# polimi-ispl/deep_prior_interpolation

Measured on AMD Instinct MI355X. Metric: Adam iters/sec on 3D MultiRes-UNet (whole job over n_gpus; per_gpu beside it); recon SNR(dB) vs ref under config.snr_vs_reference, higher is better.
Workload: dtype f32

## Files before the change

### deep_prior_interpolation_amd/_lib.py

```python
import ctypes as C
import os

_HERE = os.path.dirname(os.path.abspath(__file__))
LIB_PATH = os.path.join(_HERE, "libdpi_hip.so")


class DpiError(RuntimeError):
    pass


ABI_VERSION = 406

IO_X_BF16, IO_Y_BF16, IO_DY_BF16, IO_DX_BF16 = 1, 2, 4, 8
STORE_FWD_BF16, STORE_GRAD_BF16 = 1, 2


class ConvDesc(C.Structure):
    _fields_ = [("size", C.c_int), ("Cin", C.c_int), ("Cout", C.c_int), ("D", C.c_int), ("H", C.c_int), ("W", C.c_int),
                ("k", C.c_int), ("kd", C.c_int), ("stride", C.c_int), ("precision", C.c_int), ("io", C.c_int)]

    def __init__(self, Cin=0, Cout=0, D=1, H=1, W=1, k=1, kd=1, stride=1, precision=0, io=0):
        super().__init__(C.sizeof(ConvDesc), int(Cin), int(Cout), int(D), int(H), int(W), int(k), int(kd), int(stride), int(precision), int(io))


# ... 32 lines not shown
    "dpi_bn_bwd_reduce": (_I, [_P, _P, _P, _P, _P, _P, _F, _F, _I, _Z, _P, _P]),
    "dpi_bn_bwd_apply": (_I, [_P, _P, _P, _P, _P, _P, _F, _F, _P, _I, _I, _Z, _P, _P, _P, _P]),
    "dpi_bn_bwd_apply_fork": (_I, [_P, _P, _P, _P, _P, _P, _F, _F, _P, _I, _I, _Z, _P, _P, _P,
                                   _P, _P, _P, _P, _P, _F, _P, _P, _P, _P, _P, _P, _F, _P, _P]),
    "dpi_bn_bwd_apply_dual": (_I, [_P, _I, _I, _Z] + [_P, _P, _P, _P, _P, _F, _P, _P, _P, _P] * 2 + [_I, _I, _P, _P, _P, _F, _P, _P]),
    "dpi_chain_add_stats": (_I, [_P, _P, _P, _P, _I, _Z, _F, _P, _P, _P]),
    "dpi_lrelu_bwd": (_I, [_P, _P, _F, _Z, _P, _P]),
    "dpi_act_fwd": (_I, [_P, _Z, _I, _P, _P]),
    "dpi_act_bwd": (_I, [_P, _P, _Z, _I, _P, _P]),
    "dpi_add": (_I, [_P, _P, _Z, _P, _P]),
    "dpi_channel_sum": (_I, [_P, _I, _Z, _P, _P, _P]),
    "dpi_upsample2x_fwd": (_I, [_P, _P, _I, _I, _I, _I, _I, _I, _I, _I, _P, _P]),
    "dpi_upsample2x_bwd_ws_floats": (_Z, [_I, _I, _I, _I, _I, _I, _I, _I]),
    "dpi_upsample2x_bwd": (_I, [_P, _I, _I, _I, _I, _I, _I, _I, _I, _P, _P, _P]),
    "dpi_crop_copy": (_I, [_P, _I, _I, _I, _I, _I, _I, _I, _I, _I, _I, _P, _P]),
    "dpi_crop_copy_bwd": (_I, [_P, _I, _I, _I, _I, _I, _I, _I, _I, _I, _I, _P, _P]),
    "dpi_attn_gate_fwd": (_I, [_P, _P, _I, _I, _I, _I, _I, _P, _P, _P]),
    "dpi_attn_gate_bwd_ws_floats": (_Z, [_I, _I, _I, _I, _I]),
    "dpi_attn_gate_bwd": (_I, [_P, _P, _P, _I, _I, _I, _I, _I, _P, _P, _P, _P]),
    "dpi_pconv_mask_fwd": (_I, [_P, _P, _I, _I, _Z, _P, _P, _P]),
    "dpi_pconv_norm_fwd": (_I, [_P, _P, _P, _I, _I, _I, _I, _P, _P, _P, _P]),
    "dpi_pconv_norm_bwd_ws_floats": (_Z, [_I, _Z]),
    "dpi_pconv_norm_bwd": (_I, [_P, _P, _I, _Z, _P, _P, _P, _P]),
    "dpi_pconv_mask_bwd": (_I, [_P, _P, _P, _I, _I, _Z, _P, _P, _P]),
    "dpi_maxpool2x2_fwd": (_I, [_P, _I, _I, _I, _P, _P]),
    "dpi_maxpool2x2_bwd": (_I, [_P, _P, _I, _I, _I, _P, _P]),
    "dpi_deconv4x4s2_fwd": (_I, [_P, _P, _P, _I, _I, _I, _I, _P, _P]),
    "dpi_deconv4x4s2_bwd_data": (_I, [_P, _P, _I, _I, _I, _I, _P, _P]),
    "dpi_deconv4x4s2_bwd_weight": (_I, [_P, _P, _I, _I, _I, _I, _P, _P]),
    "dpi_loss_ws_doubles": (_Z, [_Z]),
    "dpi_masked_loss": (_I, [_P, _P, _P, _Z, _I, _F, _P, _P, _P, _P]),
    "dpi_adam_multi": (_I, [_P, _P, _I, _P, C.c_double, C.c_double, C.c_double, _P, _P]),
    "dpi_langevin_multi": (_I, [_P, _P, _I, _P, _I, C.c_double, C.c_double, C.c_double, C.c_double, C.c_double, _U64, _P, _P, _P]),
    "dpi_moments_update": (_I, [_P, _P, _P, _Z, _P, _I, _I, _P, _P]),
    "dpi_loop_control": (_I, [_P, _P, _P, _I, _P, _P, _P, _I, C.c_double, C.c_double, _I, C.c_double, C.c_double, _I, C.c_double, _P]),
    "dpi_copy_if": (_I, [_P, _P, _P, _Z, _P]),
    "dpi_masked_loss_holdout": (_I, [_P, _P, _P, _P, _I, _I, _Z, _I, _F, _P, _P, _P, _P]),
    "dpi_loop_control_holdout": (_I, [_P, _P, _P, _I, _P, _P, _P, _I, C.c_double, C.c_double, _I, C.c_double, C.c_double, _I, C.c_double, _P]),
    "dpi_ema_loss": (_I, [_P, _P, _P, _P, _P, _I, _I, _Z, _I, _F, _P, _P, _P, _P, _P]),
    "dpi_loop_control_ema": (_I, [_P, _P, _I, _P, _P, _I, _P, _P, _P, _I, C.c_double, C.c_double, _I, C.c_double, C.c_double, _I, C.c_double, _P]),
    "dpi_noise_add": (_I, [_P, _Z, _F, _U64, _P, _P, _P]),
    "dpi_fill_normal": (_I, [_P, _Z, _F, _F, _U64, _U64, _P]),
    "dpi_fir_axis0": (_I, [_P, _P, _I, _I, _I, _Z, _P, _P]),
    "dpi_axpy": (_I, [_F, _P, _Z, _P, _P]),
    "dpi_diff_axis": (_I, [_P, _Z, _I, _Z, _I, _F, _I, _P, _P]),
    "dpi_hale2d": (_I, [_P, _P, _P, _P, _Z, _I, _I, _I, _P, _P]),
    "dpi_structure_tensor": (_I, [_P, _Z, _I, _I, _F, _F, _P, _P, _P, _P]),
    "dpi_dips": (_I, [_P, _P, _P, _Z, _P, _P, _P]),
    "dpi_hale_sections": (_I, [_P, _P, _I, _I, _I, _I, _I, _P, _P]),
    "dpi_structure_tensor_sections": (_I, [_P, _I, _I, _I, _I, _F, _F, _F, _P, _P, _P, _P, _P, _P]),
    "dpi_avo_fwd": (_I, [_P, _P, _I, _I, _Z, _P, _P]),
    "dpi_avo_adj": (_I, [_P, _P, _I, _I, _Z, _P, _P]),
    "dpi_trace_sample_fwd": (_I, [_P, _P, _I, _I, _I, _I, _P, _P]),
    "dpi_trace_sample_adj": (_I, [_P, _P, _I, _I, _I, _I, _P, _P]),
    "dpi_max_ws_floats": (_Z, [_Z]),
    "dpi_scaled_max": (_I, [_P, _Z, _F, _P, _P, _P]),
    "dpi_threshold": (_I, [_P, _Z, _P, _P, _P]),
    "dpi_pocs_project": (_I, [_P, _P, _P, _Z, _P, _P]),
    "dpi_overlap_add": (_I, [_P, _I, _I, _I, _I, _I, _I, _P, _I, _I, _I, _P]),
    "dpi_overlap_normalize": (_I, [_P, _I, _I, _I, _I, _I, _I, _I, _I, _I, _F, _P]),
    "dpi_overlap_add_weighted": (_I, [_P, _P, _I, _I, _I, _I, _I, _I, _P, _I, _P, _I, _P, _I, _U, _P, _I, _I, _I, _I, _P]),
    "dpi_overlap_finalize_weighted": (_I, [_P, _I, _I, _I, _I, _F, _P, _P, _P]),
    "dpi_channel_stats_io": (_I, [_P, _P, _I, _Z, _P, _U, _P]),
    "dpi_chain_apply_io": (_I, [_P, _P, _I, _Z, _P, _U, _P]),
    "dpi_chain_add_stats_io": (_I, [_P, _P, _P, _P, _I, _Z, _F, _P, _P, _U, _P]),
    "dpi_bn_bwd_reduce_io": (_I, [_P, _P, _P, _P, _P, _P, _F, _F, _I, _Z, _P, _U, _P]),
    "dpi_bn_bwd_apply_io": (_I, [_P, _P, _P, _P, _P, _P, _F, _F, _P, _I, _I, _Z, _P, _P, _P, _U, _P]),
    "dpi_bn_bwd_apply_fork_io": (_I, [_P, _P, _P, _P, _P, _P, _F, _F, _P, _I, _I, _Z, _P, _P, _P,
                                      _P, _P, _P, _P, _P, _F, _P, _P, _P, _P, _P, _P, _F, _P, _U, _P]),
    "dpi_bn_bwd_apply_dual_io": (_I, [_P, _I, _I, _Z] + [_P, _P, _P, _P, _P, _F, _P, _P, _P, _P] * 2 + [_I, _I, _P, _P, _P, _F, _P, _U, _P]),
    "dpi_upsample2x_fwd_io": (_I, [_P, _P, _I, _I, _I, _I, _I, _I, _I, _I, _P, _U, _P]),
    "dpi_upsample2x_bwd_io": (_I, [_P, _I, _I, _I, _I, _I, _I, _I, _I, _P, _P, _U, _P]),
    "dpi_noise_add_io": (_I, [_P, _Z, _F, _U64, _P, _P, _U, _P]),
    "dpi_noise_add_regen_io": (_I, [_Z, _F, _U64, _U64, _F, _U64, _P, _P, _U, _P]),
    "dpi_set_option": (_I, [C.c_char_p, _I]),
    "dpi_pack_scratch_bytes": (_Z, []),
    "dpi_pack_release": (_I, []),
    "dpi_pack_forget": (_I, [_P]),
    "dpi_pack_slot_count": (_Z, []),
    "dpi_join_bwd_ws_doubles": (_Z, [_I, _Z]),
    "dpi_join_bwd": (_I, [_P, _P, _P, _P, _P, _F, _I, _Z,  _P, _P, _P, _P, _P, _F,  _P, _P, _P, _P, _P, _F,  _P, _P,  _I, _I, _P, _P, _P, _F,
                          _P, _P, _P, _P, _P, _P, _P, _U, _P]),
    "dpi_chain_add_apply": (_I, [_P, _P, _P, _P, _P, _I, _Z, _P, _U, _P]),
}

_lib = None


def load():
    global _lib
    if _lib is not None:
        return _lib
    if not os.path.exists(LIB_PATH):
        raise DpiError("libdpi_hip.so not found at %s — run `python -c 'import __graft_entry__ as g; g.build()'` "
                       "(hipcc --offload-arch=gfx950); there is no CPU fallback" % LIB_PATH)
    import torch
    lib = C.CDLL(LIB_PATH)
    for name, (res, args) in SIGNATURES.items():
        try:
            fn = getattr(lib, name)
        except AttributeError as e:
            raise DpiError("libdpi_hip.so does not export %s (stale build?)" % name) from e
        fn.restype = res
        fn.argtypes = args
    if lib.dpi_version() < ABI_VERSION or lib.dpi_conv_desc_size() != C.sizeof(ConvDesc):
        raise DpiError("libdpi_hip.so is ABI version %d with a %d-byte dpi_conv_desc; this binding needs >= %d and %d bytes (stale build? "
                       "re-run __graft_entry__.build())" % (lib.dpi_version(), lib.dpi_conv_desc_size(), ABI_VERSION, C.sizeof(ConvDesc)))
    lib.set_option = lambda key, value: check(lib.dpi_set_option(key.encode(), int(value)), "dpi_set_option(%s)" % key)
    _lib = lib
    return lib


def check(code, what=""):
    if code != 0:
        msg = load().dpi_last_error()
        raise DpiError("%s failed (%d): %s" % (what, code, msg.decode() if msg else "?"))


def ptr(t):
    return None if t is None else t.data_ptr()


def stream():
    import torch
    return torch.cuda.current_stream().cuda_stream
```

### deep_prior_interpolation_amd/csrc/api.cpp

```cpp
#include <stdarg.h>
#include <string.h>
#include "common.h"

static thread_local char g_err[512] = "";

void dpi_set_error(const char* fmt, ...) {
  va_list ap;
  va_start(ap, fmt);
  vsnprintf(g_err, sizeof(g_err), fmt, ap);
  va_end(ap);
}

int dpi_check_launch(const char* what) {
  const hipError_t e = hipGetLastError();
  if (e != hipSuccess) {
    dpi_set_error("%s: %s", what, hipGetErrorString(e));
    return DPI_E_LAUNCH;
  }
  return DPI_OK;
}

extern "C" const char* dpi_last_error(void) { return g_err; }
extern "C" int dpi_version(void) { return 406; }
extern "C" int dpi_conv_desc_size(void) { return (int)sizeof(dpi_conv_desc); }

extern "C" int dpi_device_info(int device, int* cus, int* lds_bytes, size_t* hbm_bytes, char* name, int name_len) {
  hipDeviceProp_t p;
  const hipError_t e = hipGetDeviceProperties(&p, device);
  if (e != hipSuccess) {
    dpi_set_error("device_info: %s", hipGetErrorString(e));
    return DPI_E_LAUNCH;
  }
  if (cus) *cus = p.multiProcessorCount;
  if (lds_bytes) *lds_bytes = (int)p.sharedMemPerBlock;
  if (hbm_bytes) *hbm_bytes = p.totalGlobalMem;
  if (name && name_len > 0) {
    strncpy(name, p.gcnArchName, name_len - 1);
    name[name_len - 1] = 0;
  }
  return DPI_OK;
}

__global__ void dpi_marker_kernel() {}

extern "C" int dpi_profile_marker(int id, void* stream) {
  DPI_REQUIRE(id >= 1 && id < 65536, "profile_marker: id %d out of range", id);
  dpi_marker_kernel<<<(unsigned)id, 64, 0, (hipStream_t)stream>>>();
  return dpi_check_launch("profile_marker");
}

extern "C" int dpi_set_option(const char* key, int value) {
  DPI_REQUIRE(key != nullptr, "set_option: key is NULL");
  struct Entry { const char* key; int lo, hi; void (*set)(int); };
  static const Entry table[] = {
      {"splitk", 0, 1, dpi_set_splitk},
      {"dual_bwd_data", 0, 1, dpi_set_dual_bwd_data},
      {"bw_pair", 0, 2, dpi_set_bw_pair},
      {"bw_workgroups", 1, 1 << 24, [](int v) { dpi_set_bw_tuning(v, -1); }},
      {"bw_xcd_order", 0, 1, [](int v) { dpi_set_bw_tuning(0, v); }},
      {"mfma_min_cout", 0, 1 << 20, dpi_set_mfma_min_cout},
      {"bwd_weight_mfma_min_cout", 0, 1 << 20, dpi_set_bwd_weight_mfma_min_cout},
      {"fewco_mfma", 0, 1, dpi_set_fewco_mfma},
      {"q4", 0, 2, [](int v) { dpi_set_q4(v, -1); }},
      {"q4_ck", 0, 4, [](int v) { dpi_set_q4(-1, v); }},
      {"q4_debug", 0, 0xFFFF, dpi_set_q4_debug},
      {"bf16_debug", 0, 0x7F, dpi_set_bf16_debug},
  };
  for (const Entry& e : table)
    if (strcmp(key, e.key) == 0) {
      DPI_REQUIRE(value >= e.lo && value <= e.hi && !(strcmp(key, "q4_ck") == 0 && value != 0 && value != 2 && value != 4),
                  "set_option: %s = %d out of range [%d, %d]", key, value, e.lo, e.hi);
      e.set(value);
      return DPI_OK;
    }
  dpi_set_error("set_option: unknown key '%s'", key);
  return DPI_E_ARG;
}
```

### deep_prior_interpolation_amd/csrc/conv_direct.hip

```cpp
#include "conv_kernels.h"

namespace {

struct ConvArgs {
  const float* __restrict__ x;
  const float* __restrict__ chain;
  const float* __restrict__ w;
  const float* __restrict__ bias;
  float* __restrict__ y;
  double* __restrict__ partials;
  int Cin, Cout;
  int D, H, W;
  int Do, Ho, Wo;
  int ntd, nth, ntw;
  long w_out_stride, w_in_stride;
  int accumulate;
  int xb, yb;
};

template <int KD, int S, int CO_B, int OW, int TZ, int TY, int TX, int CI_B, bool FLIP>
__global__ __launch_bounds__(TZ* TY* TX) void conv_direct_kernel(ConvArgs a) {
  constexpr int KS = 3;
  constexpr int NT = TZ * TY * TX;
  constexpr int SD = (KD > 1) ? S : 1;
// ... 447 lines not shown

extern "C" size_t dpi_conv_bwd_data_ws_floats(const dpi_conv_desc* d) {
  return dpi_check_conv_desc(d) == DPI_OK && d->stride == 1 ? conv_plan(d, true, 0).ws_floats : 0;
}

static int conv_run(const dpi_conv_desc* d, const float* x, const float* chain, const float* w, const float* bias,
                    float* y, double* partials, bool flip, int accumulate, float* ws, size_t ws_floats, hipStream_t st) {
  switch (conv_plan(d, flip, accumulate).kernel) {
    case ConvKernel::Bf16S2: return dpi_conv_bf16_s2_run(d, x, chain, w, bias, y, partials, st);
    case ConvKernel::Bf16: return dpi_conv_bf16_run(d, x, chain, w, bias, y, partials, flip, accumulate, st);
    case ConvKernel::Q4: return dpi_conv_q4_run(d, x, chain, w, bias, y, partials, flip, accumulate, st);
    case ConvKernel::Mfma: return dpi_conv_mfma_run(d, x, chain, w, bias, y, partials, flip, accumulate, ws, ws_floats, st);
    case ConvKernel::PwMfma: return dpi_conv_pw_mfma_run(d, x, chain, w, bias, y, partials, flip, accumulate, st);
    case ConvKernel::Fewco: return dpi_conv_fewco_mfma_run(d, x, chain, w, bias, y, partials, st);
    case ConvKernel::Pw: case ConvKernel::Direct: break;
  }
  const int taps = d->kd * d->k * d->k;
  const int cin = flip ? d->Cout : d->Cin, cout = flip ? d->Cin : d->Cout;
  const long w_out = flip ? taps : (long)d->Cin * taps, w_in = flip ? (long)d->Cin * taps : taps;
  const int xb = dpi_io_in(d, flip), yb = dpi_io_out(d, flip);
  const int co_b = pick_co_b(cout);
  if (d->k == 1) {
    PwArgs a{x, chain, w, bias, y, partials, cin, cout, (size_t)d->D * d->H * d->W, w_out, w_in, accumulate, xb, yb};
    dim3 grid((unsigned)cdivz(a.V, kPwVoxPerBlock), cdiv(cout, co_b));
    launch_pw_co(a, co_b, grid, st);
    return dpi_check_launch("conv_pw");
  }
  ConvArgs a{x, chain, w, bias, y, partials, cin, cout, d->D, d->H, d->W, 0, 0, 0, 0, 0, 0, w_out, w_in, accumulate, xb, yb};
  dpi_conv_out_dims(d, &a.Do, &a.Ho, &a.Wo);
  dim3 grid(direct_tiles(d, &a.ntd, &a.nth, &a.ntw), cdiv(cout, co_b));
  if (d->kd == 3) {
    if (d->stride == 1) { if (flip) launch_co<3, 1, true>(a, co_b, grid, st); else launch_co<3, 1, false>(a, co_b, grid, st); }
    else launch_co<3, 2, false>(a, co_b, grid, st);
  } else {
    if (d->stride == 1) { if (flip) launch_co<1, 1, true>(a, co_b, grid, st); else launch_co<1, 1, false>(a, co_b, grid, st); }
    else launch_co<1, 2, false>(a, co_b, grid, st);
  }
  return dpi_check_launch("conv_direct");
}

extern "C" int dpi_conv_fwd_ws(const dpi_conv_desc* d, const float* x, const float* x_chain, const float* w, const float* bias, float* y,
                               double* stat_partials, float* ws, size_t ws_floats, void* stream) {
  if (int e = dpi_check_conv_desc(d)) return e;
  DPI_REQUIRE(x && w && y, "conv_fwd: null tensor");
  DPI_REQUIRE(ws || ws_floats == 0, "conv_fwd: workspace size without a workspace");
  return conv_run(d, x, x_chain, w, bias, y, stat_partials, false, 0, ws, ws_floats, (hipStream_t)stream);
}

extern "C" int dpi_conv_fwd(const dpi_conv_desc* d, const float* x, const float* x_chain, const float* w,
                            const float* bias, float* y, double* stat_partials, void* stream) {
  return dpi_conv_fwd_ws(d, x, x_chain, w, bias, y, stat_partials, nullptr, 0, stream);
}

extern "C" int dpi_conv_bwd_data(const dpi_conv_desc* d, const float* dy, const float* w, float* dx,
                                 int accumulate, void* stream) {
  return dpi_conv_bwd_data_ws(d, dy, w, dx, accumulate, nullptr, 0, stream);
}

static int g_dual = getenv("DPI_NO_DUAL") ? 0 : 1;
extern "C" void dpi_set_dual_bwd_data(int on) { g_dual = on; }
extern "C" int dpi_conv_bwd_data_dual(const dpi_conv_desc* d3, const float* dy3, const float* w3, const dpi_conv_desc* d1, const float* dy1,
                                      const float* w1, float* dx, int accumulate, float* ws, size_t ws_floats, void* stream) {
  if (int e = dpi_check_conv_desc(d3)) return e;
  if (int e = dpi_check_conv_desc(d1)) return e;
  DPI_REQUIRE(dy3 && w3 && dy1 && w1 && dx, "conv_bwd_data_dual: null tensor");
  DPI_REQUIRE(ws || ws_floats == 0, "conv_bwd_data_dual: workspace size without a workspace");
  DPI_REQUIRE(d3->k == 3 && d1->k == 1 && d3->stride == 1 && d1->stride == 1, "conv_bwd_data_dual: needs a 3x3(x3) and a 1x1(x1) stride-1 layer");
  DPI_REQUIRE(d3->Cin == d1->Cin && d3->D == d1->D && d3->H == d1->H && d3->W == d1->W, "conv_bwd_data_dual: the two layers read different tensors");
  hipStream_t st = (hipStream_t)stream;
  DPI_REQUIRE((d3->io & (DPI_IO_DX_BF16 | DPI_IO_X_BF16)) == (d1->io & (DPI_IO_DX_BF16 | DPI_IO_X_BF16)), "conv_bwd_data_dual: the two layers disagree on the storage type of their input");
  const ConvKernel k3 = conv_plan(d3, true, accumulate).kernel;
  if (g_dual && k3 == ConvKernel::Bf16 && dpi_conv_bf16_second_ok(d3, true) && (d3->io & DPI_IO_DY_BF16) == (d1->io & DPI_IO_DY_BF16)) {
    const MfmaSecond sec{dy1, w1, d1->Cout, 1, (long)d1->Cin};
    return dpi_conv_bf16_run(d3, dy3, nullptr, w3, nullptr, dx, nullptr, true, accumulate, st, &sec);
  }
  if (g_dual && k3 == ConvKernel::Mfma && dpi_conv_mfma_second_ok(d3, true, d1->Cout, ws != nullptr)) {
    const MfmaSecond sec{dy1, w1, d1->Cout, 1, (long)d1->Cin};
    return dpi_conv_mfma_run(d3, dy3, nullptr, w3, nullptr, dx, nullptr, true, accumulate, nullptr, 0, st, &sec);
  }
  if (int e = conv_run(d1, dy1, nullptr, w1, nullptr, dx, nullptr, true, accumulate, nullptr, 0, st)) return e;
  return conv_run(d3, dy3, nullptr, w3, nullptr, dx, nullptr, true, 1, ws, ws_floats, st);
}

extern "C" int dpi_conv_bwd_data_ws(const dpi_conv_desc* d, const float* dy, const float* w, float* dx,
                                    int accumulate, float* ws, size_t ws_floats, void* stream) {
  if (int e = dpi_check_conv_desc(d)) return e;
  DPI_REQUIRE(dy && w && dx, "conv_bwd_data: null tensor");
  DPI_REQUIRE(ws || ws_floats == 0, "conv_bwd_data: workspace size without a workspace");
  hipStream_t st = (hipStream_t)stream;
  if (d->stride == 1) return conv_run(d, dy, nullptr, w, nullptr, dx, nullptr, true, accumulate, ws, ws_floats, st);
  if (dpi_conv_bf16_s2_bwd_usable(d) && ((uintptr_t)dy & 7) == 0 && ((uintptr_t)dx & 3) == 0) return dpi_conv_bf16_s2_bwd_run(d, dy, w, dx, accumulate, st);
  if (d->Cin >= g_mfma_min_cout) return dpi_conv_bwd_data_s2_mfma_run(d, dy, w, dx, accumulate, st);
  int Do, Ho, Wo;
  dpi_conv_out_dims(d, &Do, &Ho, &Wo);
  BwdS2Args a{dy, w, dx, d->Cin, d->Cout, d->D, d->H, d->W, Do, Ho, Wo, d->kd, accumulate, (d->io & DPI_IO_DY_BF16) != 0, (d->io & DPI_IO_DX_BF16) != 0};
  const size_t V = (size_t)d->D * d->H * d->W;
  dim3 grid((unsigned)cdivz(V, 256), cdiv(d->Cin, 8));
  conv_bwd_data_s2_kernel<8><<<grid, 256, 0, st>>>(a);
  return dpi_check_launch("conv_bwd_data_s2");
}
```

### deep_prior_interpolation_amd/csrc/conv_kernels.h

```cpp
#pragma once
#include "common.h"

struct MfmaSecond { const float* x2; const float* w2; int C2; long w2_co_stride, w2_c_stride; };
void dpi_conv_out_dims(const dpi_conv_desc* d, int* Do, int* Ho, int* Wo);
int dpi_conv_mfma_stat_blocks(const dpi_conv_desc* d, bool flip);
size_t dpi_conv_mfma_ws_floats(const dpi_conv_desc* d, bool flip);
bool dpi_conv_mfma_second_ok(const dpi_conv_desc* d, bool flip, int C2, bool have_ws);
int dpi_conv_mfma_run(const dpi_conv_desc* d, const float* x, const float* chain, const float* w, const float* bias, float* y,
                      double* partials, bool flip, int accumulate, float* ws, size_t ws_floats, hipStream_t st, const MfmaSecond* sec = nullptr);
int dpi_conv_bwd_data_s2_mfma_run(const dpi_conv_desc* d, const float* dy, const float* w, float* dx, int accumulate, hipStream_t st);
size_t dpi_conv_bwd_weight_mfma_ws_floats(const dpi_conv_desc* d);
bool dpi_conv_bwd_weight_mfma_swapped(const dpi_conv_desc* d, bool chained);
int dpi_conv_bwd_weight_mfma_run(const dpi_conv_desc* d, const float* x, const float* chain, const float* dy, float* dw, float* ws, hipStream_t st);
size_t dpi_conv_bwd_weight_smallco_ws_floats(const dpi_conv_desc* d);
int dpi_conv_bwd_weight_smallco_run(const dpi_conv_desc* d, const float* x, const float* chain, const float* dy, float* dw, float* ws, hipStream_t st);
int dpi_conv_pw_mfma_stat_blocks(const dpi_conv_desc* d);
int dpi_conv_pw_mfma_run(const dpi_conv_desc* d, const float* x, const float* chain, const float* w, const float* bias, float* y,
                         double* partials, bool flip, int accumulate, hipStream_t st);
size_t dpi_conv_pw_bwd_weight_mfma_ws_floats(const dpi_conv_desc* d);
int dpi_conv_pw_bwd_weight_mfma_run(const dpi_conv_desc* d, const float* x, const float* chain, const float* dy, float* dw, float* ws, hipStream_t st);
bool dpi_conv_fewco_usable(const dpi_conv_desc* d);
int dpi_conv_fewco_stat_blocks(const dpi_conv_desc* d);
int dpi_conv_fewco_mfma_run(const dpi_conv_desc* d, const float* x, const float* chain, const float* w, const float* bias, float* y,
                            double* partials, hipStream_t st);
bool dpi_conv_q4_usable(const dpi_conv_desc* d, bool flip);
int dpi_conv_q4_stat_blocks(const dpi_conv_desc* d);
int dpi_conv_q4_run(const dpi_conv_desc* d, const float* x, const float* chain, const float* w, const float* bias, float* y,
                    double* partials, bool flip, int accumulate, hipStream_t st);
bool dpi_bf16_force_all();
bool dpi_conv_bf16_usable(const dpi_conv_desc* d, bool flip);
int dpi_conv_bf16_stat_blocks(const dpi_conv_desc* d);
bool dpi_conv_bf16_second_ok(const dpi_conv_desc* d, bool flip);
int dpi_conv_bf16_run(const dpi_conv_desc* d, const float* x, const float* chain, const float* w, const float* bias, float* y,
                      double* partials, bool flip, int accumulate, hipStream_t st, const MfmaSecond* sec = nullptr);
bool dpi_conv_bf16_s2_usable(const dpi_conv_desc* d);
int dpi_conv_bf16_s2_stat_blocks(const dpi_conv_desc* d);
int dpi_conv_bf16_s2_run(const dpi_conv_desc* d, const float* x, const float* chain, const float* w, const float* bias, float* y, double* partials,
                         hipStream_t st);
bool dpi_conv_bf16_s2_bwd_usable(const dpi_conv_desc* d);
int dpi_conv_bf16_s2_bwd_run(const dpi_conv_desc* d, const float* dy, const float* w, float* dx, int accumulate, hipStream_t st);
bool dpi_conv_bf16_bww_usable(const dpi_conv_desc* d);
size_t dpi_conv_bf16_bww_ws_floats(const dpi_conv_desc* d);
int dpi_conv_bf16_bww_run(const dpi_conv_desc* d, const float* x, const float* chain, const float* dy, float* dw, float* ws, hipStream_t st);
bool dpi_conv_bf16_bww_s2_usable(const dpi_conv_desc* d);
size_t dpi_conv_bf16_bww_s2_ws_floats(const dpi_conv_desc* d);
int dpi_conv_bf16_bww_s2_run(const dpi_conv_desc* d, const float* x, const float* dy, float* dw, float* ws, hipStream_t st);
```

### deep_prior_interpolation_amd/csrc/conv_mfma.hip

```cpp
#include "conv_kernels.h"

namespace {

typedef float f32x4 __attribute__((ext_vector_type(4)));

struct MArgs {
  const float* __restrict__ x;
  const float* __restrict__ chain;
  const float* __restrict__ w;
  const float* __restrict__ bias;
  float* __restrict__ y;
  double* __restrict__ partials;
  int Cin, Cout;
  int D, H, W;
  int ntd, nth, ntw;
  long w_out_stride, w_in_stride;
  int accumulate;
  int split_cps;
  const float* __restrict__ x2;
  const float* __restrict__ w2;
  int C2;
  long w2_co_stride, w2_c_stride;
  int xb, yb;
  int ny;
};

template <int KD, int NR, int NH, int S = 1>
struct Geo {
  static constexpr bool SLICES = (KD == 3 && NR >= 4);
  static constexpr int SD = KD == 3 ? S : 1;
  static constexpr int TZ = SLICES ? 4 : 1;
  static constexpr int TY = SLICES ? NR : 4 * NR;
  static constexpr int TW = 16 * NH;
  static constexpr int ID = (TZ - 1) * SD + KD;
  static constexpr int IH = (TY - 1) * S + 3;
  static constexpr int IW = (TW - 1) * S + 3;
  static constexpr int RS = (IW + 3) & ~3;
  static constexpr int DS0 = IH * RS;
  static constexpr int DS = (S == 1 && (RS % 32) == 4) ? DS0 + ((12 - (DS0 % 32)) + 32) % 32 : DS0;
  static constexpr int CS0 = ID * DS;
  static constexpr int CSM = S == 1 ? 16 : 1;
  static constexpr int CS = CS0 + ((CSM - (CS0 % 32)) + 32) % 32;
  static constexpr int TILE = ID * IH * IW;
  static constexpr int E = (TILE + 255) / 256;
  static constexpr int NROW = (NR - 1) * S + 3;
  static constexpr int NSTEP = KD * NROW;
  static constexpr int NB = 3 * NH;
};

__device__ __forceinline__ int xcd_tile(int bid, int ntiles) {
  const int q = ntiles >> 3, r = ntiles & 7, xcd = bid & 7, i = bid >> 3;
  return (xcd < r ? xcd * (q + 1) : r * (q + 1) + (xcd - r) * q) + i;
}

template <class G>
__device__ __forceinline__ void tile_slots(int tid, int id0, int ih0, int iw0, int D, int H, int W, int (&goff)[G::E], int (&loff)[G::E]) {
#pragma unroll
  for (int e = 0; e < G::E; ++e) {
    const int idx = tid + e * 256;
    const int col = idx % G::IW, row = idx / G::IW;
    const int hy = row % G::IH, dz = row / G::IH;
    const int gd = id0 + dz, gh = ih0 + hy, gw = iw0 + col;
    const bool ok = idx < G::TILE && gd >= 0 && gd < D && gh >= 0 && gh < H && gw >= 0 && gw < W;
    goff[e] = ok ? (gd * H + gh) * W + gw : -1;
    loff[e] = idx < G::TILE ? dz * G::DS + hy * G::RS + col : -1;
  }
}

template <class G>
__device__ __forceinline__ void stage_load(float (&sr)[4][G::E], const float* __restrict__ x, int Cin, size_t V, int c0,
                                           const int (&goff)[G::E], bool xb = false) {
  if (xb) {
#pragma unroll
    for (int c = 0; c < 4; ++c) {
      const int ci = min(c0 + c, Cin - 1);
      const __amdgpu_buffer_rsrc_t r = dpi_buffer_t(dpi_at(x, (size_t)ci * V, true), V, true);
#pragma unroll
      for (int e = 0; e < G::E; ++e) sr[c][e] = dpi_buffer_load_bf16_raw(r, goff[e]);
    }
    return;
  }
#pragma unroll
  for (int c = 0; c < 4; ++c) {
    const int ci = min(c0 + c, Cin - 1);
    const __amdgpu_buffer_rsrc_t r = dpi_buffer(x + (size_t)ci * V, V * sizeof(float));
#pragma unroll
    for (int e = 0; e < G::E; ++e) sr[c][e] = dpi_buffer_load(r, goff[e] * 4);
  }
}

template <class G>
__device__ __forceinline__ void stage_store(float* lds, const float (&sr_in)[4][G::E], const float* __restrict__ chain, int Cin, int c0,
                                            const int (&goff)[G::E], const int (&loff)[G::E], bool xb = false) {
  float sr[4][G::E];
#pragma unroll
  for (int c = 0; c < 4; ++c)
#pragma unroll
    for (int e = 0; e < G::E; ++e) sr[c][e] = sr_in[c][e];
  if (xb) {
#pragma unroll
    for (int c = 0; c < 4; ++c)
#pragma unroll
      for (int e = 0; e < G::E; ++e) sr[c][e] = dpi_widen_raw(sr[c][e]);
  }
  if (chain == nullptr) {
#pragma unroll
    for (int c = 0; c < 4; ++c)
// ... 11 lines not shown
      const float v = goff[e] >= 0 ? apply_chain(t, sr[c][e]) : sr[c][e];
      if ((e + 1) * 256 <= G::TILE || loff[e] >= 0) lds[c * G::CS + loff[e]] = v;
    }
  }
}

template <int KD, int NR, int NH>
struct GeoV2 {
  static constexpr int TY = 4 * NR, TW = 16 * NH;
  static constexpr int ID = KD == 3 ? 3 : 1, IH = (TY - 1) * 2 + 3;
  static constexpr int NQ = TW / 2 + 1;
  static constexpr int PW = 2 * NQ;
  static constexpr int RS = 2 * PW;
  static constexpr int DS = IH * RS;
  static constexpr int CS0 = ID * DS;
  static constexpr int CS = CS0 + ((16 - (CS0 % 32)) + 32) % 32;
  static constexpr int NV4 = ID * IH * NQ;
  static constexpr int E = (NV4 + 255) / 256;
};
template <class GV>
__device__ __forceinline__ void tile_slots_v(int tid, int id0, int ih0, int iw0, int D, int H, int W, int (&goff)[GV::E], int (&loff)[GV::E]) {
#pragma unroll
  for (int e = 0; e < GV::E; ++e) {
    const int idx = tid + e * 256;
    const int q = idx % GV::NQ, row = idx / GV::NQ;
    const int hy = row % GV::IH, dz = row / GV::IH;
    const int gd = id0 + dz, gh = ih0 + hy, gw = iw0 + 4 * q;
    const bool ok = idx < GV::NV4 && gd >= 0 && gd < D && gh >= 0 && gh < H && gw >= 0 && gw + 4 <= W;
    goff[e] = ok ? (gd * H + gh) * W + gw : -4;
    loff[e] = idx < GV::NV4 ? dz * GV::DS + hy * GV::RS + 2 * q : -1;
  }
}
template <class GV>
__device__ __forceinline__ void stage_load_v(f32x4 (&sv)[4][GV::E], const float* __restrict__ x, int Cin, size_t V, int c0, const int (&goff)[GV::E]) {
#pragma unroll
  for (int c = 0; c < 4; ++c) {
    const int ci = min(c0 + c, Cin - 1);
    const __amdgpu_buffer_rsrc_t r = dpi_buffer(x + (size_t)ci * V, V * sizeof(float));
#pragma unroll
    for (int e = 0; e < GV::E; ++e) sv[c][e] = __builtin_bit_cast(f32x4, __builtin_amdgcn_raw_buffer_load_b128(r, goff[e] * 4, 0, 0));
  }
}
template <class GV>
__device__ __forceinline__ void stage_store_v(float* lds, const f32x4 (&sv)[4][GV::E], const float* __restrict__ chain, int Cin, int c0,
                                              const int (&goff)[GV::E], const int (&loff)[GV::E]) {
  typedef float f32x2 __attribute__((ext_vector_type(2)));
  if (chain == nullptr) {
#pragma unroll
    for (int c = 0; c < 4; ++c)
#pragma unroll
      for (int e = 0; e < GV::E; ++e)
        if ((e + 1) * 256 <= GV::NV4 || loff[e] >= 0) {
          float* const p = lds + c * GV::CS + loff[e];
          *reinterpret_cast<f32x2*>(p) = (f32x2){sv[c][e][0], sv[c][e][2]};
          *reinterpret_cast<f32x2*>(p + GV::PW) = (f32x2){sv[c][e][1], sv[c][e][3]};
        }
    return;
  }
#pragma unroll
  for (int c = 0; c < 4; ++c) {
    const Chain t = load_chain(chain, min(c0 + c, Cin - 1));
#pragma unroll
    for (int e = 0; e < GV::E; ++e) {
      const float m = goff[e] >= 0 ? 1.f : 0.f;
      if ((e + 1) * 256 <= GV::NV4 || loff[e] >= 0) {
        float* const p = lds + c * GV::CS + loff[e];
        *reinterpret_cast<f32x2*>(p) = (f32x2){m * apply_chain(t, sv[c][e][0]), m * apply_chain(t, sv[c][e][2])};
        *reinterpret_cast<f32x2*>(p + GV::PW) = (f32x2){m * apply_chain(t, sv[c][e][1]), m * apply_chain(t, sv[c][e][3])};
      }
    }
  }
}

#ifdef DPI_TRACE
__device__ long long g_blk[8192][4];
__device__ long long g_trace[4][64];
#define TR(i) do { if (trc >= 0 && tid == 0) g_trace[trc][i] = clock64(); } while (0)
#define TRC(i) do { if (trc >= 0 && tid == 0 && (i) < 38) g_trace[trc][i] = clock64(); } while (0)
#else
#define TR(i)
#define TRC(i)
#endif
template <int KD, int NR, int NH, bool FLIP, int S = 1, int WPE = 2, bool PERSIST = false, bool TAILPACK = false, bool IOB = false, bool YLOOP = false,
          bool S2V = false>
__global__ __launch_bounds__(256, WPE) void conv_mfma_kernel(MArgs a) {
  static_assert(!YLOOP || (!PERSIST && !TAILPACK), "the channel-tile loop is built for the one-tile-per-workgroup variants without a packed tail");
  static_assert(!S2V || (S == 2 && !FLIP && !PERSIST && !TAILPACK && !IOB && NR < 4), "vectorised stride-2 staging: forward, fp32 tensors, row-split tiles");
  using GV = GeoV2<KD, NR < 4 ? NR : 2, NH>;
  if constexpr (!IOB) { a.xb = 0; a.yb = 0; }
  using G = Geo<KD, NR, NH, S>;
  constexpr int TAPS = KD * 9;
  constexpr int PD = (KD - 1) / 2;
  constexpr int NT = NR * NH;
  __shared__ __attribute__((aligned(16))) float lds[4 * (S2V ? GV::CS : G::CS)];
  __shared__ double red[4][16][2];

  const int tid = threadIdx.x, lane = tid & 63, wid = tid >> 6;
  const int lk = lane >> 4, lj = lane & 15;
  const int ntiles = a.ntd * a.nth * a.ntw;
  int vt0 = blockIdx.x, ytile = blockIdx.y;
  if constexpr (!PERSIST) {
    if (a.ny > 0) {
      const int q8 = ntiles >> 3, r8 = ntiles & 7, xcd = blockIdx.x & 7, j = blockIdx.x >> 3;
      const int i = YLOOP ? j : j / a.ny;
      ytile = YLOOP ? 0 : j - i * a.ny;
      if (i >= q8 + (xcd < r8 ? 1 : 0)) return;
      vt0 = i * 8 + xcd;
    }
  }
  int n0 = ytile * 16;
  const size_t V = (size_t)a.D * a.H * a.W;
  const int Do = (a.D + 2 * PD - KD) / G::SD + 1, Ho = (a.H - 1) / S + 1, Wo = (a.W - 1) / S + 1;
  const size_t Vo = (size_t)Do * Ho * Wo;
#ifdef DPI_TRACE
  const int trc = blockIdx.y != 0 ? -1 : blockIdx.x == 0 ? 0 : blockIdx.x == 1 ? 1 : blockIdx.x == 30 ? 2 : blockIdx.x == 50 ? 3 : -1;
  TR(0);
  if (tid == 0 && blockIdx.y == 0 && blockIdx.x < 8192) {
    g_blk[blockIdx.x][0] = wall_clock64();
    g_blk[blockIdx.x][2] = __builtin_amdgcn_s_getreg(63492);
    g_blk[blockIdx.x][3] = __builtin_amdgcn_s_getreg(63508);
  }
#endif
  auto tile_origin = [&](int vt, int& tile_id, int& od0, int& oh0, int& ow0) {
    tile_id = xcd_tile(vt, ntiles);
    int bt = tile_id;
    const int tw_i = bt % a.ntw; bt /= a.ntw;
    const int th_i = bt % a.nth; bt /= a.nth;
    od0 = bt * G::TZ; oh0 = th_i * G::TY; ow0 = tw_i * G::TW;
  };

  const int wz = G::SLICES ? wid : 0, wh = G::SLICES ? 0 : wid * NR;
  const int lbase = S2V ? lk * GV::CS + wh * 2 * GV::RS + lj : lk * G::CS + wz * G::SD * G::DS + wh * S * G::RS + lj * S;

  int co_w = n0 + lj;
  auto w_ptr = [&](int c0, bool& ok) {
    const int ci = c0 + lk;
    ok = co_w < a.Cout && ci < a.Cin;
    return a.w + (ok ? co_w : 0) * a.w_out_stride + (ok ? ci : 0) * a.w_in_stride;
  };
  auto load_w_raw = [&](float (&wn)[9], int c0, int kd) {
    bool ok;
    const float* __restrict__ wp = w_ptr(c0, ok);
#pragma unroll
    for (int t = 0; t < 9; ++t) wn[t] = wp[FLIP ? (TAPS - 1 - (kd * 9 + t)) : kd * 9 + t];
  };
  auto commit_w = [&](float (&wr)[TAPS], const float (&wn)[9], int c0, int kd) {
    const bool ok = co_w < a.Cout && c0 + lk < a.Cin;
#pragma unroll
    for (int t = 0; t < 9; ++t) wr[kd * 9 + t] = ok ? wn[t] : 0.f;
  };

  const int c_lo = a.split_cps ? (int)blockIdx.z * a.split_cps : 0;
  float* __restrict__ const ybase = a.y + (size_t)blockIdx.z * a.Cout * Vo;
  constexpr int EE = S2V ? GV::E : G::E;
  int goff[EE], loff[EE];
  float wr[TAPS], wn[9], sr[S2V ? 1 : 4][S2V ? 1 : G::E];
  f32x4 sv[S2V ? 4 : 1][S2V ? GV::E : 1];
  auto slots = [&](int od, int oh, int ow) {
    if constexpr (S2V) tile_slots_v<GV>(tid, od * G::SD - PD, oh * 2 - 1, ow * 2 - 4, a.D, a.H, a.W, goff, loff);
    else tile_slots<G>(tid, od * G::SD - PD, oh * S - 1, ow * S - 1, a.D, a.H, a.W, goff, loff);
  };
  auto sload = [&](int c0) {
    if constexpr (S2V) stage_load_v<GV>(sv, a.x, a.Cin, V, c0, goff);
    else stage_load<G>(sr, a.x, a.Cin, V, c0, goff, a.xb);
  };
  auto sstore = [&](int c0) {
    if constexpr (S2V) stage_store_v<GV>(lds, sv, a.chain, a.Cin, c0, goff, loff);
    else stage_store<G>(lds, sr, a.chain, a.Cin, c0, goff, loff, a.xb);
// ... 128 lines not shown
        for (int i = 0; i < G::NB; ++i) bc[i] = bn[i];
        if constexpr (!YLOOP) { if (ir == G::NROW - 1) commit_w(wr, wn, cn, kd); }
      }
      if (tail_next) commit_tail_w();
      TRC(5 + (c0 / 4) * 4);
    }
    if constexpr (TAILPACK) {
      if (tail && cin_main == 0) { load_tail_w(); commit_tail_w(); }
      if (tail) {
        __syncthreads();
        sstore(cin_main);
        __syncthreads();
        if (has_next) {
          slots(od_n, oh_n, ow_n);
          sload(0);
        }
#pragma unroll
        for (int hr = 0; hr < NR; ++hr) {
          float tb[NH][NTG];
#pragma unroll
          for (int h = 0; h < NH; ++h)
#pragma unroll
            for (int g = 0; g < NTG; ++g) tb[h][g] = lds[lbase + ttoff[g] + hr * G::RS + h * 16];
#pragma unroll
          for (int g = 0; g < NTG; ++g)
#pragma unroll
            for (int h = 0; h < NH; ++h)
              acc[hr * NH + h] = __builtin_amdgcn_mfma_f32_16x16x4f32(wt[g], tb[h][g], acc[hr * NH + h], 0, 0, 0);
        }
      }
    }
    if constexpr (YLOOP) {
      if (yt + 1 < nyt) {
        const int con = (yt + 1) * 16 + lj, ci = c_lo + lk;
        const bool okn = con < a.Cout && ci < a.Cin;
        const float* __restrict__ wp = a.w + (okn ? con : 0) * a.w_out_stride + (okn ? ci : 0) * a.w_in_stride;
#pragma unroll
        for (int t = 0; t < TAPS; ++t) wr[t] = wp[FLIP ? (TAPS - 1 - t) : t];
      }
    }
    if constexpr (FLIP && !PERSIST) if (a.x2 != nullptr) {
      const __amdgpu_buffer_rsrc_t r2 = dpi_buffer_t(a.x2, (size_t)a.C2 * Vo, a.xb);
      int voff[NT];
#pragma unroll
      for (int t = 0; t < NT; ++t) {
        const int od = od0 + wz, oh = oh0 + wh + t / NH, ow = ow0 + (t % NH) * 16 + lj;
        voff[t] = (od < Do && oh < Ho && ow < Wo) ? (od * Ho + oh) * Wo + ow : -1;
      }
      const int nk2 = (a.C2 + 3) >> 2;
      auto load2 = [&](float (&b)[NT], float& wv, int kc) {
        const int c = kc * 4 + lk;
        const bool ok = c < a.C2 && co_w < a.Cout;
        const float wraw = a.w2[(ok ? co_w : 0) * a.w2_co_stride + (ok ? c : 0) * a.w2_c_stride];
        wv = ok ? wraw : 0.f;
        const int cbase = c * (int)Vo;
#pragma unroll
        for (int t = 0; t < NT; ++t)
          b[t] = a.xb ? dpi_buffer_load_bf16(r2, voff[t] >= 0 ? cbase + voff[t] : -1) : dpi_buffer_load(r2, voff[t] >= 0 ? (cbase + voff[t]) * 4 : -4);
      };
      float b0[NT], b1[NT], w0v, w1v;
      load2(b0, w0v, 0);
      for (int kc = 0; kc < nk2; kc += 2) {
        if (kc + 1 < nk2) load2(b1, w1v, kc + 1);
#pragma unroll
        for (int t = 0; t < NT; ++t) acc[t] = __builtin_amdgcn_mfma_f32_16x16x4f32(w0v, b0[t], acc[t], 0, 0, 0);
        if (kc + 1 < nk2) {
          if (kc + 2 < nk2) load2(b0, w0v, kc + 2);
#pragma unroll
          for (int t = 0; t < NT; ++t) acc[t] = __builtin_amdgcn_mfma_f32_16x16x4f32(w1v, b1[t], acc[t], 0, 0, 0);
        }
      }
    }
    TR(40);

    const bool interior = od0 + G::TZ <= Do && oh0 + G::TY <= Ho && ow0 + G::TW <= Wo && n0 + 16 <= a.Cout;
    const int vbase = ((od0 + wz) * Ho + oh0 + wh) * Wo + ow0 + lj;
#pragma unroll
    for (int r = 0; r < 4; ++r) {
      const int co = n0 + 4 * lk + r;
      const bool cok = co < a.Cout;
      const float bv = (a.bias && cok) ? a.bias[co] : 0.f;
      float* __restrict__ yc = dpi_at(ybase, (size_t)(cok ? co : 0) * Vo + vbase, a.yb);
      double s = 0.0, q = 0.0;
      if (a.yb) {
        const bool pairs = !(Wo & 1) && !(Vo & 1) && !((uintptr_t)ybase & 3);
#pragma unroll
        for (int t = 0; t < NT; ++t) {
          const int od = od0 + wz, oh = oh0 + wh + t / NH, ow = ow0 + (t % NH) * 16 + lj;
          const bool ok = interior || (cok && od < Do && oh < Ho && ow < Wo);
          const float v = dpi_round_bf16(acc[t][r] + bv);
          dpi_st_bf16_row(yc, (t / NH) * Wo + (t % NH) * 16, v, ok, pairs, lj);
          if (ok) { s += v; q += (double)v * v; }
        }
      } else if (interior) {
#pragma unroll
        for (int t = 0; t < NT; ++t) {
          const float v = acc[t][r] + bv;
          yc[(t / NH) * Wo + (t % NH) * 16] = v;
          if (a.partials) { s += v; q += (double)v * v; }
        }
      } else {
#pragma unroll
        for (int t = 0; t < NT; ++t) {
          const int od = od0 + wz, oh = oh0 + wh + t / NH, ow = ow0 + (t % NH) * 16 + lj;
          if (cok && od < Do && oh < Ho && ow < Wo) {
            const float v = acc[t][r] + bv;
            yc[(t / NH) * Wo + (t % NH) * 16] = v;
            s += v;
            q += (double)v * v;
          }
        }
      }
      if (a.partials) {
#pragma unroll
        for (int o = 8; o > 0; o >>= 1) { s += __shfl_xor(s, o, 64); q += __shfl_xor(q, o, 64); }
        if (lj == 0) { red[wid][4 * lk + r][0] = s; red[wid][4 * lk + r][1] = q; }
      }
    }
    if (a.partials) {
      __syncthreads();
      if (tid < 32) {
        const int c = tid >> 1, which = tid & 1;
        const double rsum = red[0][c][which] + red[1][c][which] + red[2][c][which] + red[3][c][which];
        if (n0 + c < a.Cout) a.partials[((size_t)tile_id * a.Cout + n0 + c) * 2 + which] = rsum;
      }
    }
    }
    TR(41);
    if (!has_next) break;
    vt = vt_next; tile_id = tile_n; od0 = od_n; oh0 = oh_n; ow0 = ow_n;
  }
#ifdef DPI_TRACE
  if (tid == 0 && blockIdx.y == 0 && blockIdx.x < 8192) g_blk[blockIdx.x][1] = wall_clock64();
#endif
}

struct BwMArgs {
  const float* __restrict__ x;
  const float* __restrict__ chain;
  const float* __restrict__ dy;
  float* __restrict__ ws;
  int Cin, Cout;
  int D, H, W;
  int ntd, nth, ntw, ntiles, tiles_per_chunk;
  int swap;
  int y0;
  int ngroups, nchunks;
  int xb, dyb;
};

template <int KD, int S, int NR, int NH, int NG = 1>
struct BwLds {
  using G = Geo<KD, NR, NH, S>;
  static constexpr int NTQ0 = (4 * KD * 9 + 15) / 16;
  static constexpr int LDSF = NG * (4 * G::CS > 4 * NTQ0 * 256 ? 4 * G::CS : 4 * NTQ0 * 256);
  static constexpr int DYRS = 4 * (4 * NH) + 4;
};

template <int KD, int S, int NR, int NH, int TC, int NG = 1, bool IOB = false>
__device__ __forceinline__ void conv_bwd_weight_mfma_body(const BwMArgs& a_in, float* __restrict__ lds, float* __restrict__ dyl_all, int first_group = -1) {
  BwMArgs a = a_in;
  if constexpr (!IOB) { a.xb = 0; a.dyb = 0; }
  static_assert(NG == 1 || TC == 0, "the column-trimmed tail is a single group");
#ifdef DPI_TRACE
  const int trc = (blockIdx.y == 0 && blockIdx.z == 0 && blockIdx.x < 4) ? (int)blockIdx.x : -1;
  int trn = 0;
#define TRW() do { if (trc >= 0 && threadIdx.x == 0 && trn < 64) g_trace[trc][trn++] = clock64(); } while (0)
// ... 447 lines not shown
      for (int t = 0; t < TAPS; ++t) wr[t] = ok ? wn[t] : 0.f;
    }
    __syncthreads();
#pragma unroll
    for (int c = 0; c < 4; ++c)
#pragma unroll
      for (int e = 0; e < E; ++e)
        if ((e + 1) * 256 <= TILE || loff[e] >= 0) lds[c * CS + loff[e]] = a.dyb ? dpi_widen_raw(sr[c][e]) : sr[c][e];
    __syncthreads();
    if (c0 + 4 < a.Cout) fetch(c0 + 4);
#pragma unroll
    for (int sd = 0; sd < ID; ++sd)
#pragma unroll
      for (int ir = 0; ir < 3; ++ir)
#pragma unroll
        for (int sw = 0; sw < 2; ++sw) {
          const float b = lds[lbase + (sd * IH + ir) * RS + sw];
#pragma unroll
          for (int sh = 0; sh < 2; ++sh) {
            const int row = ir - sh;
            if (row < 0 || row > 1) continue;
#pragma unroll
            for (int cls = 0; cls < NCLS; ++cls) {
              const int pw = cls & 1, ph = (cls >> 1) & 1, pd = KD == 3 ? (cls >> 2) & 1 : 0;
              if ((sw && !pw) || (sh && !ph) || (sd && !pd)) continue;
              const int kw = pw ? (sw ? 0 : 2) : 1, kh = ph ? (sh ? 0 : 2) : 1, kd = KD == 3 ? (pd ? (sd ? 0 : 2) : 1) : 0;
              acc[cls][row] = __builtin_amdgcn_mfma_f32_16x16x4f32(wr[(kd * 3 + kh) * 3 + kw], b, acc[cls][row], 0, 0, 0);
            }
          }
        }
  }
  typedef float f32x2 __attribute__((ext_vector_type(2)));
  const bool vec2 = !a.dxb && ((a.W | (int)(V & 1)) & 1) == 0 && (((uintptr_t)a.dx) & 7) == 0;
  if (vec2) {
#pragma unroll
    for (int cp = 0; cp < NCLS / 2; ++cp) {
      const int ph = cp & 1, pd = KD == 3 ? (cp >> 1) & 1 : 0;
#pragma unroll
      for (int row = 0; row < 2; ++row) {
        const int id = KD == 3 ? 2 * md0 + pd : md0, ih = 2 * (mh0 + wid * 2 + row) + ph, iw = 2 * (mw0 + lj);
        if (id < a.D && ih < a.H && iw < a.W) {
          f32x2 old[4];
#pragma unroll
          for (int r = 0; r < 4; ++r) {
            const int ci = n0 + 4 * lk + r;
            const size_t o = (size_t)min(ci, a.Cin - 1) * V + ((size_t)id * a.H + ih) * a.W + iw;
            old[r] = a.accumulate ? *reinterpret_cast<const f32x2*>(a.dx + o) : (f32x2){0.f, 0.f};
          }
#pragma unroll
          for (int r = 0; r < 4; ++r) {
            const int ci = n0 + 4 * lk + r;
            if (ci < a.Cin) {
              const size_t o = (size_t)ci * V + ((size_t)id * a.H + ih) * a.W + iw;
              const f32x2 v = a.accumulate ? (f32x2){old[r][0] + acc[2 * cp][row][r], old[r][1] + acc[2 * cp + 1][row][r]}
                                           : (f32x2){acc[2 * cp][row][r], acc[2 * cp + 1][row][r]};
              *reinterpret_cast<f32x2*>(a.dx + o) = v;
            }
          }
        }
      }
    }
    return;
  }
#pragma unroll
  for (int cls = 0; cls < NCLS; ++cls) {
    const int pw = cls & 1, ph = (cls >> 1) & 1, pd = KD == 3 ? (cls >> 2) & 1 : 0;
#pragma unroll
    for (int row = 0; row < 2; ++row) {
      const int id = KD == 3 ? 2 * md0 + pd : md0, ih = 2 * (mh0 + wid * 2 + row) + ph, iw = 2 * (mw0 + lj) + pw;
      if (id < a.D && ih < a.H && iw < a.W) {
#pragma unroll
        for (int r = 0; r < 4; ++r) {
          const int ci = n0 + 4 * lk + r;
          if (ci < a.Cin) {
            const size_t o = (size_t)ci * V + ((size_t)id * a.H + ih) * a.W + iw;
            dpi_st(a.dx, o, a.accumulate ? dpi_ld(a.dx, o, a.dxb) + acc[cls][row][r] : acc[cls][row][r], a.dxb);
          }
        }
      }
    }
  }
}

__global__ __launch_bounds__(256) void splitk_reduce_kernel(const float* __restrict__ ws, int nsplit, const float* __restrict__ bias,
                                                            float* __restrict__ y, int accumulate, double* __restrict__ partials,
                                                            int Cout, size_t Vo, size_t per, bool yb) {
  const int lane = threadIdx.x & 63, co = blockIdx.y * 4 + (threadIdx.x >> 6);
  if (co >= Cout) return;
  const size_t lo = (size_t)blockIdx.x * per, hi = lo + per < Vo ? lo + per : Vo;
  const float bv = bias ? bias[co] : 0.f;
  double sum = 0.0, sq = 0.0;
  for (size_t v = lo + lane; v < hi; v += 64) {
    float t = ws[(size_t)co * Vo + v];
    for (int sp = 1; sp < nsplit; ++sp) t += ws[((size_t)sp * Cout + co) * Vo + v];
    t += bv;
    if (accumulate) t += dpi_ld(y, (size_t)co * Vo + v, yb);
    t = dpi_stored(t, yb);
    dpi_st(y, (size_t)co * Vo + v, t, yb);
    sum += t; sq += (double)t * t;
  }
  if (partials) {
#pragma unroll
    for (int o = 32; o > 0; o >>= 1) { sum += __shfl_xor(sum, o, 64); sq += __shfl_xor(sq, o, 64); }
    if (lane == 0) { partials[((size_t)blockIdx.x * Cout + co) * 2] = sum; partials[((size_t)blockIdx.x * Cout + co) * 2 + 1] = sq; }
  }
}

}

static void dpi_mfma_variant(const dpi_conv_desc* d, int cout, int* nr, int* nh) {
  int Do, Ho, Wo;
  dpi_conv_out_dims(d, &Do, &Ho, &Wo);
  const int tz = d->kd == 3 ? 4 : 1, ty = d->kd == 3 ? 8 : 32;
  const long nb = (long)cdiv(Do, tz) * cdiv(Ho, ty) * cdiv(Wo, 32) * cdiv(cout, 16);
  if (nb >= 512 && d->stride == 1) { *nr = 8; *nh = 2; }
  else { *nr = 2; *nh = Wo > 16 ? 2 : 1; }
}

static bool dpi_mfma_half_tile(const dpi_conv_desc* d, bool flip) {
  const int cin = flip ? d->Cout : d->Cin, cout = flip ? d->Cin : d->Cout;
  int nr, nh;
  dpi_mfma_variant(d, cout, &nr, &nh);
  if (nr != 8 || d->kd != 3) return false;
  if (cin == 1) return true;
  if (cin <= 8) return false;
  return flip || ((cin & 3) == 1);
}

static int dpi_mfma_tiles(const dpi_conv_desc* d, int nr, int nh, int* ntd, int* nth, int* ntw) {
  int Do, Ho, Wo;
  dpi_conv_out_dims(d, &Do, &Ho, &Wo);
  const bool slices = d->kd == 3 && nr >= 4;
  const int tz = slices ? 4 : 1, ty = slices ? nr : 4 * nr;
  *ntd = cdiv(Do, tz); *nth = cdiv(Ho, ty); *ntw = cdiv(Wo, 16 * nh);
  return *ntd * *nth * *ntw;
}

struct MfmaTiling { int nr, nh, ntd, nth, ntw, ntiles; };
static MfmaTiling mfma_tiling(const dpi_conv_desc* d, bool flip) {
  MfmaTiling t{};
  dpi_mfma_variant(d, flip ? d->Cin : d->Cout, &t.nr, &t.nh);
  if (dpi_mfma_half_tile(d, flip)) t.nr = 4;
  t.ntiles = dpi_mfma_tiles(d, t.nr, t.nh, &t.ntd, &t.nth, &t.ntw);
  return t;
}
int dpi_conv_mfma_stat_blocks(const dpi_conv_desc* d, bool flip) { return mfma_tiling(d, flip).ntiles; }

template <int KD, bool FLIP, bool IOB = false>
static void launch_variant(const MArgs& a_in, int nr, int nh, int stride, dim3 grid_in, hipStream_t st) {
  if constexpr (!IOB) {
    if (a_in.xb || a_in.yb) { launch_variant<KD, FLIP, true>(a_in, nr, nh, stride, grid_in, st); return; }
  }
  const bool persistent = stride == 1 && nr == 8 && a_in.Cin > 8;
  MArgs a = a_in;
  dim3 grid = grid_in;
  if (!persistent && grid_in.y > 1) {
    a.ny = (int)grid_in.y;
    grid = dim3(8 * ((grid_in.x + 7) / 8) * grid_in.y, 1, grid_in.z);
  }
  if (stride == 2) {
    if constexpr (!FLIP) {
      if constexpr (!IOB) {
        static const bool s2v = getenv("DPI_NO_S2V") == nullptr;
        if (s2v && a.W % 4 == 0 && (((size_t)a.D * a.H * a.W) & 3) == 0 && ((uintptr_t)a.x & 15) == 0) {
          if (nh == 2) conv_mfma_kernel<KD, 2, 2, false, 2, 2, false, false, false, false, true><<<grid, 256, 0, st>>>(a);
          else conv_mfma_kernel<KD, 2, 1, false, 2, 2, false, false, false, false, true><<<grid, 256, 0, st>>>(a);
          return;
        }
      }
      if (nh == 2) conv_mfma_kernel<KD, 2, 2, false, 2, 2, false, false, IOB><<<grid, 256, 0, st>>>(a);
      else conv_mfma_kernel<KD, 2, 1, false, 2, 2, false, false, IOB><<<grid, 256, 0, st>>>(a);
    }
    return;
  }
  const bool tailpack = (a.Cin & 3) == 1 && (a.Cin > 4 || a.Cin == 1);
  if (nr == 4) {
    if constexpr (KD == 3) {
      if (tailpack) conv_mfma_kernel<KD, 4, 2, FLIP, 1, 3, false, true, IOB><<<grid, 256, 0, st>>>(a);
      else conv_mfma_kernel<KD, 4, 2, FLIP, 1, 3, false, false, IOB><<<grid, 256, 0, st>>>(a);
    }
    return;
  }
  if (nr == 8) {
    static const bool persist = getenv("DPI_NO_PERSIST") == nullptr;
    dim3 pg = grid;
    static const bool yloop = getenv("DPI_YLOOP") != nullptr && getenv("DPI_YLOOP")[0] == '1';
    if constexpr (KD == 3 && FLIP && !IOB) {
      if (yloop && a.Cin <= 4 && a.ny > 1 && a.split_cps == 0 && grid_in.z == 1) {
        conv_mfma_kernel<KD, 8, 2, FLIP, 1, 2, false, false, IOB, true><<<dim3(8 * ((grid_in.x + 7) / 8), 1, 1), 256, 0, st>>>(a);
        return;
      }
    }
    if (a.Cin <= 8) conv_mfma_kernel<KD, 8, 2, FLIP, 1, 3, false, false, IOB><<<grid, 256, 0, st>>>(a);
    else {
      if (persist && grid.x > 512) pg.x = 512;
      if (tailpack) conv_mfma_kernel<KD, 8, 2, FLIP, 1, 2, true, true, IOB><<<pg, 256, 0, st>>>(a);
      else conv_mfma_kernel<KD, 8, 2, FLIP, 1, 2, true, false, IOB><<<pg, 256, 0, st>>>(a);
    }
  }
  else if (nh == 2) conv_mfma_kernel<KD, 2, 2, FLIP, 1, 2, false, false, IOB><<<grid, 256, 0, st>>>(a);
  else conv_mfma_kernel<KD, 2, 1, FLIP, 1, 2, false, false, IOB><<<grid, 256, 0, st>>>(a);
}

#ifdef DPI_TRACE
extern "C" int dpi_debug_read_blocks(long long* out) { return (int)hipMemcpyFromSymbol(out, HIP_SYMBOL(g_blk), sizeof(long long) * 8192 * 4); }
extern "C" int dpi_debug_read_trace(long long* out) { return (int)hipMemcpyFromSymbol(out, HIP_SYMBOL(g_trace), sizeof(long long) * 4 * 64); }
#endif
static int g_splitk = getenv("DPI_SPLITK") ? atoi(getenv("DPI_SPLITK")) : 1;
extern "C" void dpi_set_splitk(int on) { g_splitk = on; }
static int dpi_mfma_splitk(const dpi_conv_desc* d, bool flip) {
  if (!g_splitk || d->k != 3) return 1;
  const int cin = flip ? d->Cout : d->Cin, cout = flip ? d->Cin : d->Cout;
  int nr, nh, a, b, c;
  dpi_mfma_variant(d, cout, &nr, &nh);
  if (nr != 2 || dpi_mfma_half_tile(d, flip)) return 1;
  const long wgs = (long)dpi_mfma_tiles(d, nr, nh, &a, &b, &c) * cdiv(cout, 16);
  const int chunks = cdiv(cin, 4);
  if (wgs > 512 || (wgs > 256 && chunks < 24)) return 1;
  long ns = 1536 / wgs;
  if (ns > chunks / 8) ns = chunks / 8;
  if (ns > 8) ns = 8;
  return ns < 2 ? 1 : (int)ns;
}
size_t dpi_conv_mfma_ws_floats(const dpi_conv_desc* d, bool flip) {
  const int ns = dpi_mfma_splitk(d, flip);
  if (ns < 2) return 0;
  int Do, Ho, Wo;
  dpi_conv_out_dims(d, &Do, &Ho, &Wo);
  return (size_t)ns * (flip ? d->Cin : d->Cout) * Do * Ho * Wo;
}

bool dpi_conv_mfma_second_ok(const dpi_conv_desc* d, bool flip, int C2, bool have_ws) {
  int Do, Ho, Wo;
  dpi_conv_out_dims(d, &Do, &Ho, &Wo);
  if (!flip || d->stride != 1 || C2 < 1 || ((size_t)C2 + 4) * Do * Ho * Wo * sizeof(float) >= ((size_t)1 << 31)) return false;
  int nr, nh;
  dpi_mfma_variant(d, d->Cin, &nr, &nh);
  if (nr == 8 && !dpi_mfma_half_tile(d, flip) && d->Cout > 8) return false;
  return !(have_ws && dpi_mfma_splitk(d, flip) > 1);
}

int dpi_conv_mfma_run(const dpi_conv_desc* d, const float* x, const float* chain, const float* w, const float* bias, float* y,
                      double* partials, bool flip, int accumulate, float* ws, size_t ws_floats, hipStream_t st, const MfmaSecond* sec) {
  const int taps = d->kd * 9;
  const int cin = flip ? d->Cout : d->Cin, cout = flip ? d->Cin : d->Cout;
  const long w_out = flip ? taps : (long)d->Cin * taps, w_in = flip ? (long)d->Cin * taps : taps;
  MArgs a{x, chain, w, bias, y, partials, cin, cout, d->D, d->H, d->W, 0, 0, 0, w_out, w_in, accumulate, 0, nullptr, nullptr, 0, 0, 0,
          dpi_io_in(d, flip), dpi_io_out(d, flip)};
  const MfmaTiling t = mfma_tiling(d, flip);
  const int nr = t.nr, nh = t.nh, ntiles = t.ntiles;
  a.ntd = t.ntd; a.nth = t.nth; a.ntw = t.ntw;
  dim3 grid(ntiles, cdiv(cout, 16));
  if (sec) { a.x2 = sec->x2; a.w2 = sec->w2; a.C2 = sec->C2; a.w2_co_stride = sec->w2_co_stride; a.w2_c_stride = sec->w2_c_stride; }
  const int nsplit = (ws && !sec) ? dpi_mfma_splitk(d, flip) : 1;
  if (nsplit > 1) {
    int Do, Ho, Wo;
    dpi_conv_out_dims(d, &Do, &Ho, &Wo);
    const size_t Vo = (size_t)Do * Ho * Wo;
    DPI_REQUIRE(ws_floats >= (size_t)nsplit * cout * Vo, "conv (split): workspace of %zu floats, need %zu", ws_floats, (size_t)nsplit * cout * Vo);
    a.split_cps = 4 * cdiv(cdiv(cin, 4), nsplit);
    a.y = ws; a.bias = nullptr; a.partials = nullptr; a.accumulate = 0; a.yb = 0;
    grid.z = cdiv(cin, a.split_cps);
    const int nz = (int)grid.z;
    if (d->kd == 3) { if (flip) launch_variant<3, true>(a, nr, nh, d->stride, grid, st); else launch_variant<3, false>(a, nr, nh, d->stride, grid, st); }
    else { if (flip) launch_variant<1, true>(a, nr, nh, d->stride, grid, st); else launch_variant<1, false>(a, nr, nh, d->stride, grid, st); }
    if (int e = dpi_check_launch("conv_mfma (split)")) return e;
    splitk_reduce_kernel<<<dim3(ntiles, cdiv(cout, 4)), 256, 0, st>>>(ws, nz, bias, y, accumulate, partials, cout, Vo, cdivz(Vo, (size_t)ntiles),
                                                                      dpi_io_out(d, flip));
    return dpi_check_launch("splitk_reduce");
  }
  if (d->kd == 3) { if (flip) launch_variant<3, true>(a, nr, nh, d->stride, grid, st); else launch_variant<3, false>(a, nr, nh, d->stride, grid, st); }
  else { if (flip) launch_variant<1, true>(a, nr, nh, d->stride, grid, st); else launch_variant<1, false>(a, nr, nh, d->stride, grid, st); }
  return dpi_check_launch("conv_mfma");
}

static bool mfma_bw_swap_better(const dpi_conv_desc* d) {
  if (d->stride != 1) return false;
  auto util = [](int rows, int staged) { return (double)rows / (16.0 * cdiv(rows, 16)) * staged / (4.0 * cdiv(staged, 4)); };
  return util(d->Cin, d->Cout) > 1.15 * util(d->Cout, d->Cin);
}

static int g_bw_want = getenv("DPI_BW_WANT") ? atoi(getenv("DPI_BW_WANT")) : 2304;
static int g_bw_xcd_order = getenv("DPI_BW_XCD_ORDER") ? atoi(getenv("DPI_BW_XCD_ORDER")) : 0;
extern "C" void dpi_set_bw_tuning(int want_workgroups, int xcd_order) {
  if (want_workgroups > 0) g_bw_want = want_workgroups;
  if (xcd_order >= 0) g_bw_xcd_order = xcd_order;
}
static size_t bw_extra_lds() { static const size_t v = getenv("DPI_BW_EXTRA_LDS") ? (size_t)atoi(getenv("DPI_BW_EXTRA_LDS")) * 1024 : 0; return v; }
struct MfmaBwPlan { int nchunks, tiles_per_chunk, ntiles, ntd, nth, ntw, nr, nh, npairs, nfull, ny; };
static int g_bw_pair = getenv("DPI_BW_PAIR") ? atoi(getenv("DPI_BW_PAIR")) : 2;
extern "C" void dpi_set_bw_pair(int mode) { if (mode >= 0 && mode <= 2) g_bw_pair = mode; }
static MfmaBwPlan mfma_bw_plan(const dpi_conv_desc* d, bool swap = false) {
  MfmaBwPlan p{};
  {
    const int staged = swap ? d->Cout : d->Cin, groups = cdiv(staged, 4);
    const bool s1k3 = d->stride == 1 && d->kd == 3;
    const int tailg = (s1k3 && (staged & 3) == 1) ? 1 : 0;
    p.nfull = groups - tailg;
    p.npairs = (g_bw_pair && s1k3 && !g_bw_xcd_order && p.nfull >= 2 && d->io == 0) ? p.nfull / 2 : 0;
    if (g_bw_pair == 2) {
      int a_, b_, c_;
      if (p.nfull < 4 || dpi_mfma_tiles(d, 8, 2, &a_, &b_, &c_) < 1024) p.npairs = 0;
    }
    p.ny = p.npairs ? p.npairs + (p.nfull & 1) + tailg : groups;
  }
  if (d->stride == 1) { p.nr = 8; p.nh = 2; }
  else { int Do, Ho, Wo; dpi_conv_out_dims(d, &Do, &Ho, &Wo); p.nr = 2; p.nh = Wo > 16 ? 2 : 1; }
  p.ntiles = dpi_mfma_tiles(d, p.nr, p.nh, &p.ntd, &p.nth, &p.ntw);
  const size_t per = (size_t)d->Cout * d->Cin * d->kd * 9;
  const size_t max_chunks_mem = per ? ((size_t)32 << 20) / per : 1;
  const size_t blocks_other = (size_t)p.ny * (swap ? cdiv(d->Cin, 16) : cdiv(d->Cout, 16));
  size_t want = (size_t)g_bw_want / blocks_other;
  if (want < 1) want = 1;
  if (want > (size_t)p.ntiles) want = p.ntiles;
  if (want > max_chunks_mem) want = max_chunks_mem;
  if (want < 1) want = 1;
  if (g_bw_xcd_order && want > 8) want = want / 8 * 8;
  p.tiles_per_chunk = (int)cdivz(p.ntiles, want);
  p.nchunks = cdiv(p.ntiles, p.tiles_per_chunk);
  return p;
}

size_t dpi_conv_bwd_weight_mfma_ws_floats(const dpi_conv_desc* d) {
  const int n0 = mfma_bw_plan(d, false).nchunks, n1 = mfma_bw_swap_better(d) ? mfma_bw_plan(d, true).nchunks : 0;
  return (size_t)(n0 > n1 ? n0 : n1) * d->Cout * d->Cin * d->kd * 9;
}
bool dpi_conv_bwd_weight_mfma_swapped(const dpi_conv_desc* d, bool chained) { return !chained && mfma_bw_swap_better(d); }

static int bf16_row_class(const void* base, int row_len, size_t channel_elems) {
  return ((row_len & 1) == 0 && (channel_elems & 1) == 0 && ((uintptr_t)base & 3) == 0) ? 1 : 2;
}

int dpi_conv_bwd_weight_mfma_run(const dpi_conv_desc* d, const float* x, const float* chain, const float* dy, float* dw, float* ws,
                                 hipStream_t st) {
  const bool swap = dpi_conv_bwd_weight_mfma_swapped(d, chain != nullptr);
  const MfmaBwPlan p = mfma_bw_plan(d, swap);
  BwMArgs a{x, chain, dy, ws, d->Cin, d->Cout, d->D, d->H, d->W, p.ntd, p.nth, p.ntw, p.ntiles, p.tiles_per_chunk, 0, 0, 0, p.nchunks,
            (d->io & DPI_IO_X_BF16) != 0, (d->io & DPI_IO_DY_BF16) != 0};
  dim3 grid(p.nchunks, cdiv(d->Cin, 4), cdiv(d->Cout, 16));
  if (swap) {
    a.x = dy; a.chain = nullptr; a.dy = x; a.Cin = d->Cout; a.Cout = d->Cin; a.swap = 1;
    a.xb = (d->io & DPI_IO_DY_BF16) != 0; a.dyb = (d->io & DPI_IO_X_BF16) != 0;
    grid = dim3(p.nchunks, cdiv(d->Cout, 4), cdiv(d->Cin, 16));
  }
  if (a.dyb) {
    int Do_, Ho_, Wo_;
    dpi_conv_out_dims(d, &Do_, &Ho_, &Wo_);
    a.dyb = swap ? bf16_row_class(a.dy, d->W, (size_t)d->D * d->H * d->W) : bf16_row_class(a.dy, Wo_, (size_t)Do_ * Ho_ * Wo_);
  }
  auto xcd_grid = [&](dim3 g) {
    if (!g_bw_xcd_order) { a.ngroups = 0; return g; }
    a.ngroups = (int)g.y;
// ... 97 lines not shown
```

### deep_prior_interpolation_amd/csrc/conv_q4_mfma.hip

```cpp
#include "conv_kernels.h"

namespace {

typedef float f32x4 __attribute__((ext_vector_type(4)));

struct QArgs {
  const float* __restrict__ x;
  const float* __restrict__ chain;
  const float* __restrict__ w;
  const float* __restrict__ bias;
  float* __restrict__ y;
  double* __restrict__ partials;
  int Cin, Cout;
  int D, H, W;
  int ntd, nth, ntw;
  long w_out_stride, w_in_stride;
  int accumulate;
  int dbg;
};

template <int R>
struct QGeo {
  static constexpr int TZ = 4, TY = R, TW = 64;
  static constexpr int ID = TZ + 2, IH = R + 2;
  static constexpr int RS = 72;
  static constexpr int DS = IH * RS, CS = ID * DS;
  static constexpr int NV4 = ID * IH * 18;
  static constexpr int E = (NV4 + 255) / 256;
};

__device__ __forceinline__ int q4_xcd_tile(int bid, int ntiles) {
  const int q = ntiles >> 3, r = ntiles & 7, xcd = bid & 7, i = bid >> 3;
  return (xcd < r ? xcd * (q + 1) : r * (q + 1) + (xcd - r) * q) + i;
}

template <int R, int NB, int CK, bool FLIP, bool AL>
__global__ __launch_bounds__(256, 2) void conv_q4_mfma_kernel(QArgs a) {
  using G = QGeo<R>;
  constexpr int TAPS = 27;
  constexpr int NWT = CK * TAPS * NB * 4;
  constexpr int WE = (NWT + 255) / 256;
  __shared__ __attribute__((aligned(16))) float lds[CK * G::CS];
  __shared__ float wl[NWT];
  __shared__ double red[4][4 * NB][2];

  const int tid = threadIdx.x, lane = tid & 63, wid = tid >> 6;
  const int ntiles = a.ntd * a.nth * a.ntw;
  const int tile_id = q4_xcd_tile(blockIdx.x, ntiles);
  int bt = tile_id;
  const int tw_i = bt % a.ntw; bt /= a.ntw;
  const int th_i = bt % a.nth; bt /= a.nth;
  const int od0 = bt * G::TZ, oh0 = th_i * G::TY, ow0 = tw_i * G::TW;
  const size_t V = (size_t)a.D * a.H * a.W;

  int goff[G::E], loff[G::E];
#pragma unroll
  for (int e = 0; e < G::E; ++e) {
    const int idx = tid + e * 256;
    const int q = idx % 18, row = idx / 18;
    const int hy = row % G::IH, dz = row / G::IH;
    const int gd = od0 - 1 + dz, gh = oh0 - 1 + hy, gw = ow0 - 4 + 4 * q;
    const bool ok = idx < G::NV4 && gd >= 0 && gd < a.D && gh >= 0 && gh < a.H && gw >= 0 && gw + 4 <= a.W;
    goff[e] = ok ? (gd * a.H + gh) * a.W + gw : -4;
    loff[e] = idx < G::NV4 ? dz * G::DS + hy * G::RS + 4 * q : -1;
  }
  auto stage_load = [&](f32x4 (&sr)[CK][G::E], int c0) {
#pragma unroll
    for (int c = 0; c < CK; ++c) {
      const int ci = min(c0 + c, a.Cin - 1);
      const __amdgpu_buffer_rsrc_t r = dpi_buffer(a.x + (size_t)ci * V, V * sizeof(float));
#pragma unroll
      for (int e = 0; e < G::E; ++e) {
        if constexpr (AL) sr[c][e] = __builtin_bit_cast(f32x4, __builtin_amdgcn_raw_buffer_load_b128(r, goff[e] * 4, 0, 0));
        else {
#pragma unroll
          for (int k = 0; k < 4; ++k) sr[c][e][k] = dpi_buffer_load(r, goff[e] < 0 ? -4 : (goff[e] + k) * 4);
        }
      }
    }
  };
  auto stage_store = [&](const f32x4 (&sr)[CK][G::E], int c0) {
    if (a.chain == nullptr) {
#pragma unroll
      for (int c = 0; c < CK; ++c)
#pragma unroll
        for (int e = 0; e < G::E; ++e)
          if ((e + 1) * 256 <= G::NV4 || loff[e] >= 0) *reinterpret_cast<f32x4*>(lds + c * G::CS + loff[e]) = sr[c][e];
      return;
    }
#pragma unroll
    for (int c = 0; c < CK; ++c) {
      const Chain t = load_chain(a.chain, min(c0 + c, a.Cin - 1));
#pragma unroll
      for (int e = 0; e < G::E; ++e) {
        const float m = goff[e] >= 0 ? 1.f : 0.f;
        f32x4 v;
#pragma unroll
        for (int k = 0; k < 4; ++k) v[k] = m * apply_chain(t, sr[c][e][k]);
        if ((e + 1) * 256 <= G::NV4 || loff[e] >= 0) *reinterpret_cast<f32x4*>(lds + c * G::CS + loff[e]) = v;
      }
    }
  };
  auto wt_index = [&](int t, int c0, bool& ok) {
    const int i = t & 3, s = (t >> 2) % NB, ct = (t >> 2) / NB, tap = ct % TAPS, c = ct / TAPS;
    const int co = 4 * s + i, ci = c0 + c;
    ok = t < NWT && co < a.Cout && ci < a.Cin;
    return (ok ? co : 0) * a.w_out_stride + (ok ? ci : 0) * a.w_in_stride + (FLIP ? TAPS - 1 - tap : tap);
  };
  auto load_wt = [&](float (&wreg)[WE], int c0) {
#pragma unroll
    for (int k = 0; k < WE; ++k) {
      bool ok;
      wreg[k] = a.w[wt_index(tid + k * 256, c0, ok)];
    }
  };
  auto store_wt = [&](const float (&wreg)[WE], int c0) {
#pragma unroll
    for (int k = 0; k < WE; ++k) {
      bool ok;
      wt_index(tid + k * 256, c0, ok);
// ... 1 lines not shown
    }
  };

  const int Do = a.D, Ho = a.H, Wo = a.W;
  const int od = od0 + wid, ow = ow0 + lane;
  f32x4 acc[R][NB];
#pragma unroll
  for (int hr = 0; hr < R; ++hr)
#pragma unroll
    for (int s = 0; s < NB; ++s) acc[hr][s] = (f32x4){0.f, 0.f, 0.f, 0.f};

  f32x4 sr[CK][G::E];
  float wreg[WE];
  load_wt(wreg, 0);
  stage_load(sr, 0);

  const int xbase = wid * G::DS + 4 + lane;
  constexpr int NSTEP = CK * 3 * G::IH;

  for (int c0 = 0; c0 < a.Cin; c0 += CK) {
    if (!(a.dbg & 32)) __syncthreads();
    if (!(a.dbg & 2) || c0 == 0) stage_store(sr, c0);
    store_wt(wreg, c0);
    if (!(a.dbg & 32)) __syncthreads();
    if (a.dbg & 4) {
      if (c0 + CK < a.Cin) { load_wt(wreg, c0 + CK); stage_load(sr, c0 + CK); }
      continue;
    }
    float wr[CK][TAPS][NB];
#pragma unroll
    for (int c = 0; c < CK; ++c)
#pragma unroll
      for (int t = 0; t < TAPS; ++t)
#pragma unroll
        for (int s = 0; s < NB; ++s) wr[c][t][s] = wl[((c * TAPS + t) * NB + s) * 4 + (lane & 3)];

    auto load_x = [&](float (&xv)[3], int step) {
      const int c = step / (3 * G::IH), kd = (step / G::IH) % 3, ir = step % G::IH;
      const int o = xbase + c * G::CS + kd * G::DS + ir * G::RS;
#pragma unroll
      for (int kw = 0; kw < 3; ++kw) xv[kw] = lds[o + kw - 1];
    };
    float xv[3], xn[3];
    load_x(xv, 0);
    __builtin_amdgcn_sched_barrier(0);
    if (c0 + CK < a.Cin) {
      load_wt(wreg, c0 + CK);
      if (!(a.dbg & 1)) stage_load(sr, c0 + CK);
    }
    __builtin_amdgcn_sched_barrier(0);
#pragma unroll
    for (int step = 0; step < NSTEP; ++step) {
      const int c = step / (3 * G::IH), kd = (step / G::IH) % 3, ir = step % G::IH;
      if (step + 1 < NSTEP) load_x(xn, step + 1);
      __builtin_amdgcn_sched_barrier(0);
#pragma unroll
      for (int kw = 0; kw < 3; ++kw) {
#pragma unroll
        for (int kh = 0; kh < 3; ++kh) {
          const int hr = ir - kh;
          if (hr >= 0 && hr < R) {
#pragma unroll
            for (int s = 0; s < NB; ++s)
              acc[hr][s] = __builtin_amdgcn_mfma_f32_4x4x1f32(wr[c][(kd * 3 + kh) * 3 + kw][s], xv[kw], acc[hr][s], 0, 0, 0);
          }
        }
      }
      __builtin_amdgcn_sched_barrier(0);
#pragma unroll
      for (int kw = 0; kw < 3; ++kw) xv[kw] = xn[kw];
    }
  }

  const bool col_ok = od < Do && ow < Wo;
#pragma unroll
  for (int s = 0; s < NB; ++s)
#pragma unroll
    for (int i = 0; i < 4; ++i) {
      const int co = 4 * s + i;
      const bool cok = co < a.Cout;
      const float bv = (a.bias && cok) ? a.bias[co] : 0.f;
      float* __restrict__ yc = a.y + (size_t)(cok ? co : 0) * V + ((size_t)(od < Do ? od : 0) * Ho + oh0) * Wo + ow;
      double sm = 0.0, sq = 0.0;
      float old[R];
      if (a.accumulate) {
#pragma unroll
        for (int hr = 0; hr < R; ++hr) old[hr] = (cok && col_ok && oh0 + hr < Ho) ? yc[hr * Wo] : 0.f;
      } else {
#pragma unroll
        for (int hr = 0; hr < R; ++hr) old[hr] = 0.f;
      }
#pragma unroll
      for (int hr = 0; hr < R; ++hr) {
        if (cok && col_ok && oh0 + hr < Ho) {
          const float v = acc[hr][s][i] + bv + old[hr];
          if (!(a.dbg & 8)) yc[hr * Wo] = v;
          sm += v;
          sq += (double)v * v;
        }
      }
      if (a.partials && cok) {
        sm = wave_sum(sm);
        sq = wave_sum(sq);
        if (lane == 0) { red[wid][co][0] = sm; red[wid][co][1] = sq; }
      }
    }
  if (a.partials) {
    __syncthreads();
    if (tid < 2 * a.Cout) {
      const int c = tid >> 1, which = tid & 1;
      a.partials[((size_t)tile_id * a.Cout + c) * 2 + which] = red[0][c][which] + red[1][c][which] + red[2][c][which] + red[3][c][which];
    }
  }
}

template <int R>
struct QiGeo {
  static constexpr int TZ = 4, TY = R, TW = 64;
  static constexpr int ID = TZ + 2, IH = R + 2;
  static constexpr int NP = 72;
  static constexpr int RS = NP * 4, DS = IH * RS, TILE = ID * DS;
  static constexpr int NSLOT = ID * IH * 18;
  static constexpr int E = (NSLOT + 255) / 256;
};
__device__ __forceinline__ int qi_pos(int col) {
  const int g = col >> 2, j = col & 3;
  return (4 * g + (j ^ ((g >> 1) & 3))) * 4;
}

template <int R, int NB, bool FLIP, bool AL, bool KHP = false>
__global__ __launch_bounds__(256, 2) void conv_q4i_mfma_kernel(QArgs a) {
  static_assert(!KHP || (NB == 1 && !FLIP), "kh-packed rows: one output channel, forward only");
  using G = QiGeo<R>;
  constexpr int TAPS = 27;
  constexpr int NWT = KHP ? 9 * 16 : TAPS * NB * 16;
  constexpr int WE = (NWT + 255) / 256;
  __shared__ __attribute__((aligned(16))) float lds[G::TILE];
  __shared__ __attribute__((aligned(16))) float wl[NWT];
  __shared__ double red[4][4 * NB][2];

  const int tid = threadIdx.x, lane = tid & 63, wid = tid >> 6;
  const int ntiles = a.ntd * a.nth * a.ntw;
  const int tile_id = q4_xcd_tile(blockIdx.x, ntiles);
  int bt = tile_id;
  const int tw_i = bt % a.ntw; bt /= a.ntw;
  const int th_i = bt % a.nth; bt /= a.nth;
  const int od0 = bt * G::TZ, oh0 = th_i * G::TY, ow0 = tw_i * G::TW;
  const size_t V = (size_t)a.D * a.H * a.W;

  int goff[G::E], loff[G::E];
#pragma unroll
  for (int e = 0; e < G::E; ++e) {
    const int idx = tid + e * 256;
    const int q = idx % 18, row = idx / 18;
    const int hy = row % G::IH, dz = row / G::IH;
    const int gd = od0 - 1 + dz, gh = oh0 - 1 + hy, gw = ow0 - 4 + 4 * q;
    const bool ok = idx < G::NSLOT && gd >= 0 && gd < a.D && gh >= 0 && gh < a.H && gw >= 0 && gw + 4 <= a.W;
    goff[e] = ok ? (gd * a.H + gh) * a.W + gw : -4;
    loff[e] = idx < G::NSLOT ? dz * G::DS + hy * G::RS + 16 * q : -1;
  }
  const int swz = ((tid % 18) >> 1) & 3;
  auto stage_load = [&](f32x4 (&sr)[G::E][4], int c0) {
#pragma unroll
    for (int c = 0; c < 4; ++c) {
      const int ci = min(c0 + c, a.Cin - 1);
      const __amdgpu_buffer_rsrc_t r = dpi_buffer(a.x + (size_t)ci * V, V * sizeof(float));
#pragma unroll
      for (int e = 0; e < G::E; ++e) {
        if constexpr (AL) sr[e][c] = __builtin_bit_cast(f32x4, __builtin_amdgcn_raw_buffer_load_b128(r, goff[e] * 4, 0, 0));
        else {
#pragma unroll
          for (int k = 0; k < 4; ++k) sr[e][c][k] = dpi_buffer_load(r, goff[e] < 0 ? -4 : (goff[e] + k) * 4);
        }
      }
    }
  };
  auto stage_store = [&](const f32x4 (&sr)[G::E][4], int c0) {
    if (a.chain == nullptr) {
#pragma unroll
      for (int e = 0; e < G::E; ++e) {
        const int x = (((tid + e * 256) % 18) >> 1) & 3;
// ... 153 lines not shown
      float old[R];
      if (a.accumulate) {
#pragma unroll
        for (int hr = 0; hr < R; ++hr) old[hr] = (cok && col_ok && oh0 + hr < Ho) ? yc[hr * Wo] : 0.f;
      } else {
#pragma unroll
        for (int hr = 0; hr < R; ++hr) old[hr] = 0.f;
      }
#pragma unroll
      for (int hr = 0; hr < R; ++hr) {
        if (cok && col_ok && oh0 + hr < Ho) {
          const float v = acc[hr][s][i] + bv + old[hr];
          if (!(a.dbg & 8)) yc[hr * Wo] = v;
          sm += v;
          sq += (double)v * v;
        }
      }
      if (a.partials && cok) {
        sm = wave_sum(sm);
        sq = wave_sum(sq);
        if (lane == 0) { red[wid][co][0] = sm; red[wid][co][1] = sq; }
      }
    }
  if (a.partials) {
    __syncthreads();
    if (tid < 2 * a.Cout) {
      const int c = tid >> 1, which = tid & 1;
      a.partials[((size_t)tile_id * a.Cout + c) * 2 + which] = red[0][c][which] + red[1][c][which] + red[2][c][which] + red[3][c][which];
    }
  }
}

static int g_q4 = 1;
static int g_q4_ck = 0;
static int g_q4_dbg = 0;
static int g_q4_khp = getenv("DPI_NO_KHP") ? 0 : 1;

}

extern "C" void dpi_set_q4_debug(int flags) { g_q4_dbg = flags; }
extern "C" void dpi_set_q4(int on, int ck) {
  if (on >= 0) g_q4 = on;
  if (ck == 0 || ck == 2 || ck == 4) g_q4_ck = ck;
}

bool dpi_conv_q4_usable(const dpi_conv_desc* d, bool flip) {
  if (!g_q4 || d->k != 3 || d->kd != 3 || d->stride != 1) return false;
  if (dpi_io_in(d, flip) || dpi_io_out(d, flip)) return false;
  const int cout = flip ? d->Cin : d->Cout;
  if (cout > 8 || (d->W & 3)) return false;
  if (g_q4 == 2) return true;
  if (d->W < 48) return false;
  const long tiles = (long)cdiv(d->D, 4) * cdiv(d->H, 8) * cdiv(d->W, 64);
  return tiles >= 192;
}

static int q4_tiles(const dpi_conv_desc* d, int* ntd, int* nth, int* ntw) {
  *ntd = cdiv(d->D, 4); *nth = cdiv(d->H, 8); *ntw = cdiv(d->W, 64);
  return *ntd * *nth * *ntw;
}
int dpi_conv_q4_stat_blocks(const dpi_conv_desc* d) { int a, b, c; return q4_tiles(d, &a, &b, &c); }

template <int NB, bool FLIP>
static void q4_launch(const QArgs& a, int ntiles, bool aligned, hipStream_t st) {
  const size_t extra = (size_t)((g_q4_dbg >> 8) & 255) * 1024;
  if constexpr (NB == 1) {
    if constexpr (!FLIP) {
      if (a.Cout == 1 && g_q4_khp && (g_q4_ck == 4 || g_q4_ck == 0)) {
        if (aligned) conv_q4i_mfma_kernel<8, 1, false, true, true><<<ntiles, 256, extra, st>>>(a);
        else conv_q4i_mfma_kernel<8, 1, false, false, true><<<ntiles, 256, extra, st>>>(a);
        return;
      }
    }
    if (g_q4_ck == 4 || (g_q4_ck == 0 && a.Cin >= 16)) {
      if (aligned) conv_q4i_mfma_kernel<8, NB, FLIP, true><<<ntiles, 256, extra, st>>>(a);
      else conv_q4i_mfma_kernel<8, NB, FLIP, false><<<ntiles, 256, extra, st>>>(a);
      return;
    }
  }
  if (aligned) conv_q4_mfma_kernel<8, NB, 2, FLIP, true><<<ntiles, 256, extra, st>>>(a);
  else conv_q4_mfma_kernel<8, NB, 2, FLIP, false><<<ntiles, 256, extra, st>>>(a);
}

int dpi_conv_q4_run(const dpi_conv_desc* d, const float* x, const float* chain, const float* w, const float* bias, float* y,
                    double* partials, bool flip, int accumulate, hipStream_t st) {
  const int cin = flip ? d->Cout : d->Cin, cout = flip ? d->Cin : d->Cout;
  const long w_out = flip ? 27 : (long)d->Cin * 27, w_in = flip ? (long)d->Cin * 27 : 27;
  QArgs a{x, chain, w, bias, y, partials, cin, cout, d->D, d->H, d->W, 0, 0, 0, w_out, w_in, accumulate, g_q4_dbg};
  const int ntiles = q4_tiles(d, &a.ntd, &a.nth, &a.ntw);
  const bool aligned = ((uintptr_t)x & 15) == 0;
  if (cout <= 4) { if (flip) q4_launch<1, true>(a, ntiles, aligned, st); else q4_launch<1, false>(a, ntiles, aligned, st); }
  else { if (flip) q4_launch<2, true>(a, ntiles, aligned, st); else q4_launch<2, false>(a, ntiles, aligned, st); }
  return dpi_check_launch("conv_q4_mfma");
}
```

### deep_prior_interpolation_amd/csrc/dpi_hip_internal.h

```cpp
#pragma once
#define DPI_INTERNAL __attribute__((visibility("hidden")))
extern "C" {
DPI_INTERNAL void dpi_set_bw_tuning(int want_workgroups, int xcd_order);
DPI_INTERNAL void dpi_set_bf16_debug(int flags);
DPI_INTERNAL void dpi_set_splitk(int on);
DPI_INTERNAL void dpi_set_dual_bwd_data(int on);
DPI_INTERNAL void dpi_set_bw_pair(int mode);
DPI_INTERNAL void dpi_set_mfma_min_cout(int n);
DPI_INTERNAL void dpi_set_bwd_weight_mfma_min_cout(int n);
DPI_INTERNAL void dpi_set_fewco_mfma(int on);
DPI_INTERNAL void dpi_set_q4(int on, int ck);
DPI_INTERNAL void dpi_set_q4_debug(int flags);
}
```

### deep_prior_interpolation_amd/csrc/elementwise.hip

```cpp
#include "common.h"
#include <stdlib.h>

namespace {

constexpr int kStatSpan = 16384;
constexpr int kMaxStatBlocks = 2048;

__host__ __device__ inline size_t stat_span(size_t V, int nblk) {
  size_t s = (V + nblk - 1) / nblk;
  return (s + 3) & ~(size_t)3;
}

typedef float ew_f32x4 __attribute__((ext_vector_type(4)));
constexpr size_t kNtMinFloats = (size_t)32 << 20;
__device__ __forceinline__ float4 ld4(const float* p, bool nt) {
  if (nt) { const ew_f32x4 v = __builtin_nontemporal_load(reinterpret_cast<const ew_f32x4*>(p)); return make_float4(v[0], v[1], v[2], v[3]); }
  return *reinterpret_cast<const float4*>(p);
}
__device__ __forceinline__ void st4(float* p, float4 v, bool nt) {
  if (nt) __builtin_nontemporal_store((ew_f32x4){v.x, v.y, v.z, v.w}, reinterpret_cast<ew_f32x4*>(p));
  else *reinterpret_cast<float4*>(p) = v;
}

template <bool xb = false>
__global__ __launch_bounds__(256) void channel_stats_kernel(const float* __restrict__ x, const float* __restrict__ chain,
                                                            int C, size_t V, int nblk, double* __restrict__ partials) {
  const bool nt = (size_t)gridDim.y * V >= kNtMinFloats;
  const int c = blockIdx.y, b = blockIdx.x;
  const size_t span = stat_span(V, nblk);
  const size_t beg = (size_t)b * span, end = beg + span < V ? beg + span : V;
  const float* __restrict__ xc = dpi_at(x, (size_t)c * V, xb);
  const Chain t = load_chain(chain, c);
  double s = 0.0, q = 0.0;
  const bool vec = (V & 3) == 0;
  for (size_t i = beg + (size_t)threadIdx.x * 4; i < end; i += 1024) {
    float v[4];
    if (vec) {
      const float4 f = dpi_ld4(xc, i, xb, nt);
      v[0] = f.x; v[1] = f.y; v[2] = f.z; v[3] = f.w;
    } else {
#pragma unroll
      for (int k = 0; k < 4; ++k) v[k] = i + k < end ? dpi_ld(xc, i + k, xb) : 0.f;
    }
    float ls = 0.f;
    double lq = 0.0;
#pragma unroll
    for (int k = 0; k < 4; ++k)
      if (i + k < end) {
        const float y = apply_chain(t, v[k]);
        ls += y;
        lq += (double)y * y;
      }
    s += ls; q += lq;
  }
  __shared__ double sh[8];
  const double S = block_sum(s, sh);
  const double Q = block_sum(q, sh + 4);
  if (threadIdx.x == 0) {
    partials[((size_t)b * C + c) * 2 + 0] = S;
    partials[((size_t)b * C + c) * 2 + 1] = Q;
  }
}

__global__ __launch_bounds__(256) void bn_finalize_kernel(const double* __restrict__ partials, int nblk, int C, double count,
                                                         const float* __restrict__ gamma, const float* __restrict__ beta,
                                                         float eps, float momentum, float slope, int act_first,
                                                         const float* __restrict__ in_chain, float* running_mean, float* running_var, int64_t* nbt,
                                                         float* __restrict__ mean_invstd, float* __restrict__ chain_out) {
  const int c = blockIdx.x, lane = threadIdx.x;
  double s = 0.0, q = 0.0;
  {
    double s1 = 0.0, q1 = 0.0;
    int b = lane;
    for (; b + 256 < nblk; b += 512) {
      const double2 u = *reinterpret_cast<const double2*>(partials + ((size_t)b * C + c) * 2);
      const double2 v = *reinterpret_cast<const double2*>(partials + ((size_t)(b + 256) * C + c) * 2);
      s += u.x; q += u.y; s1 += v.x; q1 += v.y;
    }
    if (b < nblk) {
      const double2 u = *reinterpret_cast<const double2*>(partials + ((size_t)b * C + c) * 2);
      s += u.x; q += u.y;
    }
    s += s1; q += q1;
  }
  __shared__ double sh[8];
  s = block_sum(s, sh);
  q = block_sum(q, sh + 4);
  if (lane == 0) {
    const double mean = s / count;
    double var = q / count - mean * mean;
    if (var < 0.0) var = 0.0;
    const float invstd = (float)(1.0 / sqrt(var + (double)eps));
    const float meanf = (float)mean;
    if (mean_invstd) { mean_invstd[c] = meanf; mean_invstd[C + c] = invstd; }
    if (running_mean) running_mean[c] = (1.f - momentum) * running_mean[c] + momentum * meanf;
    if (running_var) {
      const double unb = count > 1.0 ? var * (count / (count - 1.0)) : var;
      running_var[c] = (1.f - momentum) * running_var[c] + momentum * (float)unb;
    }
    if (nbt && c == 0) *nbt += 1;
    if (chain_out) {
      const float g = gamma ? gamma[c] : 1.f, bt = beta ? beta[c] : 0.f;
      const float a = g * invstd;
      float* o = chain_out + (size_t)c * DPI_CHAIN_STRIDE;
      if (in_chain) {
        const float* ic = in_chain + (size_t)c * DPI_CHAIN_STRIDE;
        o[0] = ic[0]; o[1] = ic[1]; o[2] = ic[2]; o[3] = a * ic[3]; o[4] = fmaf(a, ic[4], bt - meanf * a);
      } else if (act_first) { o[0] = 1.f; o[1] = 0.f; o[2] = slope; o[3] = a; o[4] = bt - meanf * a; }
      else { o[0] = a; o[1] = bt - meanf * a; o[2] = slope; o[3] = 1.f; o[4] = 0.f; }
    }
  }
}

template <bool xb = false, bool yb = false>
__global__ __launch_bounds__(256) void chain_apply_kernel(const float* __restrict__ x, const float* __restrict__ chain, size_t V,
                                                          float* __restrict__ y) {
  const bool nt = (size_t)gridDim.y * V >= kNtMinFloats;
  const int c = blockIdx.y;
  const Chain t = load_chain(chain, c);
  const float* __restrict__ xc = dpi_at(x, (size_t)c * V, xb);
  float* __restrict__ yc = dpi_at(y, (size_t)c * V, yb);
  const bool vec = (V & 3) == 0;
  for (size_t i = ((size_t)blockIdx.x * 256 + threadIdx.x) * 4; i < V; i += (size_t)gridDim.x * 1024) {
    if (vec) {
      float4 f = dpi_ld4(xc, i, xb, nt);
      f.x = apply_chain(t, f.x); f.y = apply_chain(t, f.y); f.z = apply_chain(t, f.z); f.w = apply_chain(t, f.w);
      dpi_st4(yc, i, f, yb, nt);
    } else {
      for (int k = 0; k < 4 && i + k < V; ++k) dpi_st(yc, i + k, apply_chain(t, dpi_ld(xc, i + k, xb)), yb);
    }
  }
}

struct BnBwd {
  float mean, invstd, a, pb, pre, post;
  bool chained;
  Chain in;
};
__device__ __forceinline__ BnBwd bn_bwd_consts(const float* __restrict__ mean_invstd, const float* __restrict__ gamma,
                                               const float* __restrict__ beta, const float* __restrict__ in_chain, float pre,
                                               float post, int C, int c) {
  BnBwd k;
  k.chained = in_chain != nullptr;
  k.in = load_chain(in_chain, c);
  k.mean = mean_invstd[c]; k.invstd = mean_invstd[C + c];
  k.a = (gamma ? gamma[c] : 1.f) * k.invstd;
  k.pb = (beta ? beta[c] : 0.f) - k.mean * k.a;
  k.pre = pre; k.post = post;
  return k;
}
__device__ __forceinline__ void bn_bwd_elem(const BnBwd& k, float x, float dy, float& xhat, float& g) {
  if (k.chained) x = apply_chain(k.in, x);
  const float u = x > 0.f ? x : x * k.pre;
  xhat = (u - k.mean) * k.invstd;
  const float yv = fmaf(k.a, u, k.pb);
  g = (k.post == 1.f || yv > 0.f) ? dy : dy * k.post;
}

template <bool fb = false, bool gb = false>
__global__ __launch_bounds__(256) void bn_bwd_reduce_kernel(const float* __restrict__ dy, const float* __restrict__ x,
                                                            const float* __restrict__ mean_invstd, const float* __restrict__ gamma,
                                                            const float* __restrict__ beta, const float* __restrict__ in_chain,
                                                            float pre, float post, int C, size_t V, int nblk,
                                                            double* __restrict__ partials) {
  const bool nt = (size_t)gridDim.y * V >= kNtMinFloats;
  const int c = blockIdx.y, b = blockIdx.x;
  const size_t span = stat_span(V, nblk);
  const size_t beg = (size_t)b * span, end = beg + span < V ? beg + span : V;
  const BnBwd k = bn_bwd_consts(mean_invstd, gamma, beta, in_chain, pre, post, C, c);
  const float* __restrict__ xc = dpi_at(x, (size_t)c * V, fb);
  const float* __restrict__ gc = dpi_at(dy, (size_t)c * V, gb);
  double s = 0.0, q = 0.0;
  const bool vec = (V & 3) == 0;
  for (size_t i = beg + (size_t)threadIdx.x * 4; i < end; i += 1024) {
    float xv[4], gv[4];
    if (vec) {
      const float4 f = dpi_ld4(xc, i, fb, nt);
      const float4 g = dpi_ld4(gc, i, gb, nt);
      xv[0] = f.x; xv[1] = f.y; xv[2] = f.z; xv[3] = f.w;
      gv[0] = g.x; gv[1] = g.y; gv[2] = g.z; gv[3] = g.w;
    } else {
#pragma unroll
      for (int j = 0; j < 4; ++j) { xv[j] = i + j < end ? dpi_ld(xc, i + j, fb) : 0.f; gv[j] = i + j < end ? dpi_ld(gc, i + j, gb) : 0.f; }
    }
    float ls = 0.f, lq = 0.f;
#pragma unroll
    for (int j = 0; j < 4; ++j)
      if (i + j < end) {
        float xh, g;
        bn_bwd_elem(k, xv[j], gv[j], xh, g);
        ls += g; lq = fmaf(g, xh, lq);
      }
    s += ls; q += lq;
  }
  __shared__ double sh[8];
  const double S = block_sum(s, sh);
  const double Q = block_sum(q, sh + 4);
  if (threadIdx.x == 0) {
    partials[((size_t)b * C + c) * 2 + 0] = S;
    partials[((size_t)b * C + c) * 2 + 1] = Q;
  }
}

template <bool fb = false, bool gb = false>
__global__ __launch_bounds__(256) void bn_bwd_apply_kernel(const float* __restrict__ dy, const float* __restrict__ x,
                                                           const float* __restrict__ mean_invstd, const float* __restrict__ gamma,
                                                           const float* __restrict__ beta, const float* __restrict__ in_chain,
                                                           float pre, float post, const double* __restrict__ partials, int nblk, int C, size_t V,
                                                           float* __restrict__ dx, float* __restrict__ dgamma,
                                                           float* __restrict__ dbeta) {
  const bool nt = (size_t)gridDim.y * V >= kNtMinFloats;
  const int c = blockIdx.y;
  __shared__ double tot[2];
  if (threadIdx.x < 64) {
    double s = 0.0, q = 0.0;
    for (int b = threadIdx.x; b < nblk; b += 64) {
      s += partials[((size_t)b * C + c) * 2 + 0];
      q += partials[((size_t)b * C + c) * 2 + 1];
    }
    s = wave_sum(s);
    q = wave_sum(q);
    if (threadIdx.x == 0) { tot[0] = s; tot[1] = q; }
  }
  __syncthreads();
  const BnBwd k = bn_bwd_consts(mean_invstd, gamma, beta, in_chain, pre, post, C, c);
  const float k1 = (float)(tot[0] / (double)V), k2 = (float)(tot[1] / (double)V);
  if (blockIdx.x == 0 && threadIdx.x == 0) {
    if (dgamma) dgamma[c] = (float)tot[1];
    if (dbeta) dbeta[c] = (float)tot[0];
  }
  const float* __restrict__ xc = dpi_at(x, (size_t)c * V, fb);
  const float* __restrict__ gc = dpi_at(dy, (size_t)c * V, gb);
  float* __restrict__ oc = dpi_at(dx, (size_t)c * V, gb);
  const bool vec = (V & 3) == 0;
  auto one = [&](float xv, float gv) {
    float xh, g;
    bn_bwd_elem(k, xv, gv, xh, g);
    const float du = k.a * (g - k1 - xh * k2);
    return (k.pre == 1.f || xv > 0.f) ? du : du * k.pre;
// ... 816 lines not shown

#define DPI_LAUNCH_FG(io, KERNEL, GRID, ST, ...)                                          \
  do {                                                                                    \
    if (DPI_FB(io)) {                                                                     \
      if (DPI_GB(io)) KERNEL<true, true><<<GRID, 256, 0, ST>>>(__VA_ARGS__);              \
      else KERNEL<true, false><<<GRID, 256, 0, ST>>>(__VA_ARGS__);                        \
    } else {                                                                              \
      if (DPI_GB(io)) KERNEL<false, true><<<GRID, 256, 0, ST>>>(__VA_ARGS__);             \
      else KERNEL<false, false><<<GRID, 256, 0, ST>>>(__VA_ARGS__);                       \
    }                                                                                     \
  } while (0)
#define DPI_FB(io) (((io) & DPI_STORE_FWD_BF16) != 0)
#define DPI_GB(io) (((io) & DPI_STORE_GRAD_BF16) != 0)
#define DPI_REQUIRE_IO(io, what) DPI_REQUIRE(((io) & ~3u) == 0, what ": unknown storage-type bits in io = %u", (unsigned)(io))

extern "C" int dpi_channel_stats_io(const float* x, const float* chain, int C, size_t V, double* partials, unsigned io, void* stream) {
  DPI_REQUIRE(x && partials && C > 0 && V > 0, "channel_stats: bad argument");
  DPI_REQUIRE_IO(io, "channel_stats");
  const int nblk = dpi_stat_blocks(C, V);
  if (DPI_FB(io)) channel_stats_kernel<true><<<dim3(nblk, C), 256, 0, (hipStream_t)stream>>>(x, chain, C, V, nblk, partials);
  else channel_stats_kernel<false><<<dim3(nblk, C), 256, 0, (hipStream_t)stream>>>(x, chain, C, V, nblk, partials);
  return dpi_check_launch("channel_stats");
}
extern "C" int dpi_channel_stats(const float* x, const float* chain, int C, size_t V, double* partials, void* stream) {
  return dpi_channel_stats_io(x, chain, C, V, partials, 0, stream);
}

extern "C" int dpi_bn_finalize(const double* partials, int nblk, int C, size_t count, const float* gamma, const float* beta,
                               float eps, float momentum, float slope, int act_first, const float* in_chain, float* running_mean,
                               float* running_var, int64_t* num_batches_tracked, float* mean_invstd, float* chain_out,
                               void* stream) {
  DPI_REQUIRE(partials && nblk > 0 && C > 0 && count > 0, "bn_finalize: bad argument");
  DPI_REQUIRE(!in_chain || (slope == 1.f && !act_first), "bn_finalize: a composed input chain excludes a fused activation");
  bn_finalize_kernel<<<C, 256, 0, (hipStream_t)stream>>>(partials, nblk, C, (double)count, gamma, beta, eps, momentum, slope, act_first,
                                                        in_chain, running_mean, running_var, num_batches_tracked, mean_invstd, chain_out);
  return dpi_check_launch("bn_finalize");
}

extern "C" int dpi_chain_apply_io(const float* x, const float* chain, int C, size_t V, float* y, unsigned io, void* stream) {
  DPI_REQUIRE(x && y && C > 0 && V > 0, "chain_apply: bad argument");
  DPI_REQUIRE_IO(io, "chain_apply");
  if (DPI_FB(io)) chain_apply_kernel<true, true><<<dim3(ew_blocks(cdivz(V, 4)), C), 256, 0, (hipStream_t)stream>>>(x, chain, V, y);
  else chain_apply_kernel<false, false><<<dim3(ew_blocks(cdivz(V, 4)), C), 256, 0, (hipStream_t)stream>>>(x, chain, V, y);
  return dpi_check_launch("chain_apply");
}
extern "C" int dpi_chain_apply(const float* x, const float* chain, int C, size_t V, float* y, void* stream) {
  return dpi_chain_apply_io(x, chain, C, V, y, 0, stream);
}

extern "C" int dpi_bn_bwd_reduce(const float* dy, const float* x, const float* mean_invstd, const float* gamma, const float* beta,
                                 const float* in_chain, float pre_slope, float post_slope, int C, size_t V, double* partials,
                                 void* stream) {
  return dpi_bn_bwd_reduce_io(dy, x, mean_invstd, gamma, beta, in_chain, pre_slope, post_slope, C, V, partials, 0, stream);
}
extern "C" int dpi_bn_bwd_reduce_io(const float* dy, const float* x, const float* mean_invstd, const float* gamma, const float* beta,
                                    const float* in_chain, float pre_slope, float post_slope, int C, size_t V, double* partials,
                                    unsigned io, void* stream) {
  DPI_REQUIRE(dy && x && mean_invstd && partials && C > 0 && V > 0, "bn_bwd_reduce: bad argument");
  DPI_REQUIRE_IO(io, "bn_bwd_reduce");
  DPI_REQUIRE(!in_chain || pre_slope == 1.f, "bn_bwd_reduce: in_chain excludes pre_slope");
  const int nblk = dpi_stat_blocks(C, V);
  DPI_LAUNCH_FG(io, bn_bwd_reduce_kernel, dim3(nblk, C), (hipStream_t)stream, dy, x, mean_invstd, gamma, beta, in_chain, pre_slope, post_slope, C, V,
                nblk, partials);
  return dpi_check_launch("bn_bwd_reduce");
}

extern "C" int dpi_bn_bwd_apply(const float* dy, const float* x, const float* mean_invstd, const float* gamma, const float* beta,
                                const float* in_chain, float pre_slope, float post_slope, const double* partials, int nblk, int C,
                                size_t V, float* dx, float* dgamma, float* dbeta, void* stream) {
  return dpi_bn_bwd_apply_io(dy, x, mean_invstd, gamma, beta, in_chain, pre_slope, post_slope, partials, nblk, C, V, dx, dgamma, dbeta, 0, stream);
}
extern "C" int dpi_bn_bwd_apply_io(const float* dy, const float* x, const float* mean_invstd, const float* gamma, const float* beta,
                                   const float* in_chain, float pre_slope, float post_slope, const double* partials, int nblk, int C,
                                   size_t V, float* dx, float* dgamma, float* dbeta, unsigned io, void* stream) {
  DPI_REQUIRE(dy && x && mean_invstd && partials && dx && C > 0 && V > 0 && nblk > 0, "bn_bwd_apply: bad argument");
  DPI_REQUIRE_IO(io, "bn_bwd_apply");
  DPI_REQUIRE(!in_chain || pre_slope == 1.f, "bn_bwd_apply: in_chain excludes pre_slope");
  unsigned gx = ew_blocks(cdivz(V, 4 * 8));
  DPI_LAUNCH_FG(io, bn_bwd_apply_kernel, dim3(gx, C), (hipStream_t)stream, dy, x, mean_invstd, gamma, beta, in_chain, pre_slope, post_slope, partials, nblk,
                C, V, dx, dgamma, dbeta);
  return dpi_check_launch("bn_bwd_apply");
}

extern "C" int dpi_bn_bwd_apply_fork(const float* dy, const float* x, const float* mean_invstd, const float* gamma, const float* beta,
                                     const float* in_chain, float pre_slope, float post_slope, const double* partials, int nblk, int C,
                                     size_t V, float* dx, float* dgamma, float* dbeta, const float* xa, const float* mi_a,
                                     const float* gamma_a, const float* beta_a, const float* chain_a, float post_a, double* partials_a,
                                     const float* xb, const float* mi_b, const float* gamma_b, const float* beta_b, const float* chain_b,
                                     float post_b, double* partials_b, void* stream) {
  return dpi_bn_bwd_apply_fork_io(dy, x, mean_invstd, gamma, beta, in_chain, pre_slope, post_slope, partials, nblk, C, V, dx, dgamma, dbeta,
                                  xa, mi_a, gamma_a, beta_a, chain_a, post_a, partials_a, xb, mi_b, gamma_b, beta_b, chain_b, post_b, partials_b, 0,
                                  stream);
}
extern "C" int dpi_bn_bwd_apply_fork_io(const float* dy, const float* x, const float* mean_invstd, const float* gamma, const float* beta,
                                        const float* in_chain, float pre_slope, float post_slope, const double* partials, int nblk, int C,
                                        size_t V, float* dx, float* dgamma, float* dbeta, const float* xa, const float* mi_a,
                                        const float* gamma_a, const float* beta_a, const float* chain_a, float post_a, double* partials_a,
                                        const float* xb, const float* mi_b, const float* gamma_b, const float* beta_b, const float* chain_b,
                                        float post_b, double* partials_b, unsigned io, void* stream) {
  DPI_REQUIRE(dy && x && mean_invstd && partials && dx && C > 0 && V > 0 && nblk > 0, "bn_bwd_apply_fork: bad argument");
  DPI_REQUIRE_IO(io, "bn_bwd_apply_fork");
  DPI_REQUIRE(!in_chain || pre_slope == 1.f, "bn_bwd_apply_fork: in_chain excludes pre_slope");
  DPI_REQUIRE((!xa || (mi_a && partials_a)) && (!xb || (mi_b && partials_b)), "bn_bwd_apply_fork: incomplete follow-up BatchNorm");
  const int nb = dpi_stat_blocks(C, V);
  const BnFork fa{xa, mi_a, gamma_a, beta_a, chain_a, post_a, partials_a}, fb{xb, mi_b, gamma_b, beta_b, chain_b, post_b, partials_b};
  DPI_LAUNCH_FG(io, bn_bwd_apply_fork_kernel, dim3(nb, C), (hipStream_t)stream, dy, x, mean_invstd, gamma, beta, in_chain, pre_slope, post_slope,
                partials, nblk, C, V, nb, dx, dgamma, dbeta, fa, fb);
  return dpi_check_launch("bn_bwd_apply_fork");
}

extern "C" int dpi_bn_bwd_apply_dual(const float* dy, int nblk, int C, size_t V, const float* xa, const float* mi_a, const float* gamma_a,
                                     const float* beta_a, const float* chain_a, float post_a, const double* partials_a, float* dxa,
                                     float* dgamma_a, float* dbeta_a, const float* xb, const float* mi_b, const float* gamma_b,
                                     const float* beta_b, const float* chain_b, float post_b, const double* partials_b, float* dxb,
                                     float* dgamma_b, float* dbeta_b, int f_lo, int f_hi, const float* f_mi, const float* f_gamma,
                                     const float* f_beta, float f_post, double* f_partials, void* stream) {
  return dpi_bn_bwd_apply_dual_io(dy, nblk, C, V, xa, mi_a, gamma_a, beta_a, chain_a, post_a, partials_a, dxa, dgamma_a, dbeta_a, xb, mi_b, gamma_b,
                                  beta_b, chain_b, post_b, partials_b, dxb, dgamma_b, dbeta_b, f_lo, f_hi, f_mi, f_gamma, f_beta, f_post, f_partials, 0,
                                  stream);
}
extern "C" int dpi_bn_bwd_apply_dual_io(const float* dy, int nblk, int C, size_t V, const float* xa, const float* mi_a, const float* gamma_a,
                                        const float* beta_a, const float* chain_a, float post_a, const double* partials_a, float* dxa,
                                        float* dgamma_a, float* dbeta_a, const float* xb, const float* mi_b, const float* gamma_b,
                                        const float* beta_b, const float* chain_b, float post_b, const double* partials_b, float* dxb,
                                        float* dgamma_b, float* dbeta_b, int f_lo, int f_hi, const float* f_mi, const float* f_gamma,
                                        const float* f_beta, float f_post, double* f_partials, unsigned io, void* stream) {
  DPI_REQUIRE(dy && xa && xb && mi_a && mi_b && partials_a && partials_b && dxa && dxb && C > 0 && V > 0 && nblk > 0,
              "bn_bwd_apply_dual: bad argument");
  DPI_REQUIRE_IO(io, "bn_bwd_apply_dual");
  DPI_REQUIRE(!f_partials || (f_mi && f_lo >= 0 && f_hi <= C && f_lo < f_hi), "bn_bwd_apply_dual: bad fork range");
  const int nb = dpi_stat_blocks(C, V);
  const BnSide A{xa, mi_a, gamma_a, beta_a, chain_a, post_a, partials_a, dxa, dgamma_a, dbeta_a};
  const BnSide B{xb, mi_b, gamma_b, beta_b, chain_b, post_b, partials_b, dxb, dgamma_b, dbeta_b};
  DPI_LAUNCH_FG(io, bn_bwd_apply_dual_kernel, dim3(nb, C), (hipStream_t)stream, dy, A, B, nblk, C, V, nb, f_lo, f_hi, f_mi, f_gamma, f_beta, f_post,
                f_partials);
  return dpi_check_launch("bn_bwd_apply_dual");
}

static int join_blocks(int C, size_t V) { return dpi_stat_blocks(C, V); }
extern "C" size_t dpi_join_bwd_ws_doubles(int C, size_t V) { return (size_t)join_blocks(C, V) * (size_t)C * kJoinSums; }
extern "C" int dpi_join_bwd(const float* dy, const float* t, const float* mi, const float* gamma, const float* beta, float pre, int C, size_t V,
                            const float* xa, const float* mi_a, const float* gamma_a, const float* beta_a, const float* chain_a, float post_a,
                            const float* xb, const float* mi_b, const float* gamma_b, const float* beta_b, const float* chain_b, float post_b,
                            const float* fwd_chain_a, const float* fwd_chain_b,
                            int f_lo, int f_hi, const float* f_mi, const float* f_gamma, const float* f_beta, float f_post,
                            double* ws, float* coef, float* dxa, float* dxb, float* dxf, float* dgb, float* dgb_f, unsigned io, void* stream) {
  DPI_REQUIRE(dy && mi && xa && xb && mi_a && mi_b && ws && coef && dxa && dxb && dgb && C > 0 && V > 0, "join_bwd: bad argument");
  DPI_REQUIRE_IO(io, "join_bwd");
  DPI_REQUIRE(t || (fwd_chain_a && fwd_chain_b), "join_bwd: without t the two forward chains that form it are needed");
  DPI_REQUIRE(f_lo >= 0 && f_hi <= C && f_lo <= f_hi, "join_bwd: bad fork range");
  DPI_REQUIRE(f_lo == f_hi || (f_mi && dxf && dgb_f), "join_bwd: the fork range needs its BatchNorm's statistics and outputs");
  const int nblk = join_blocks(C, V);
  const JoinSide A{xa, mi_a, gamma_a, beta_a, chain_a, post_a, fwd_chain_a}, B{xb, mi_b, gamma_b, beta_b, chain_b, post_b, fwd_chain_b};
  const JoinFork F{f_lo, f_hi, f_mi, f_gamma, f_beta, f_post};
  hipStream_t st = (hipStream_t)stream;
  DPI_LAUNCH_FG(io, join_bwd_sums_kernel, dim3(nblk, C), st, dy, t, mi, gamma, beta, pre, A, B, F, C, V, nblk, ws);
  join_bwd_coef_kernel<<<C, 64, 0, st>>>(ws, nblk, C, (double)V, mi_b, gamma_b, f_lo, f_hi, coef, dgb, dgb_f);
  DPI_LAUNCH_FG(io, join_bwd_apply_kernel, dim3(ew_blocks(cdivz(V, 4 * 8)), C), st, dy, t, mi, gamma, beta, pre, A, B, F, coef, C, V, dxa, dxb, dxf);
  return dpi_check_launch("join_bwd");
}

extern "C" int dpi_chain_add_stats(const float* a, const float* chain_a, const float* b, const float* chain_b, int C, size_t V,
                                   float slope, float* t, double* partials, void* stream) {
  return dpi_chain_add_stats_io(a, chain_a, b, chain_b, C, V, slope, t, partials, 0, stream);
}
extern "C" int dpi_chain_add_stats_io(const float* a, const float* chain_a, const float* b, const float* chain_b, int C, size_t V,
// ... 165 lines not shown
```

### deep_prior_interpolation_amd/ops.py

```python
import ctypes as C
import os
import threading

import torch

from . import _lib
from ._lib import ConvDesc, check, ptr, stream
from .schedule import Schedule

BN_EPS = 1e-5
BN_MOMENTUM = 0.1


def _req(t, name, act=False):
    if not t.is_cuda:
        raise _lib.DpiError("%s must live on the GPU: the HIP path has no CPU fallback" % name)
    if t.dtype != torch.float32 and not (act and t.dtype == torch.bfloat16):
        raise _lib.DpiError("%s must be float32%s (got %s)" % (name, " or bfloat16" if act else "", t.dtype))
    return t.contiguous()


STORAGE_BF16 = os.environ.get("DPI_STORAGE", "fp32") == "bf16"
_tls = threading.local()

# ... 88 lines not shown
        raise _lib.DpiError("conv: weight expects %d input channels, tensor has %d" % (w.shape[1], Cin))
    io = ((_lib.IO_X_BF16 | _lib.IO_DX_BF16) if _bf(x) else 0) | ((_lib.IO_Y_BF16 | _lib.IO_DY_BF16) if ydt == torch.bfloat16 else 0)
    return ConvDesc(Cin, w.shape[0], D, H, W, k, kd, int(stride), precision(), io)


def desc_out_dims(d):
    sd = d.stride if d.kd > 1 else 1
    return conv_out(d.D, d.kd, sd), conv_out(d.H, d.k, d.stride), conv_out(d.W, d.k, d.stride)


class KernelTimer:

    def __init__(self, match):
        self.match = match
        self.events = []

    def durations(self):
        return [a.elapsed_time(b) for _, a, b in self.events]

    def by_key(self):
        out = {}
        for key, a, b in self.events:
            out.setdefault(key, []).append(a.elapsed_time(b))
        return out


_timer = None


def set_timer(t):
    global _timer
    _timer = t


_PROFILE_TAGS = os.environ.get("DPI_PROFILE_TAGS")
_tag_ids = {}


def _tag_id(kind, d):
    key = "%s %d->%d k%d%s s%d @%dx%dx%d" % (kind, d.Cin, d.Cout, d.k, " (2-D)" if d.D == 1 else "", d.stride, d.D, d.H, d.W)
    i = _tag_ids.get(key)
    if i is None:
        i = len(_tag_ids) + 2
        _tag_ids[key] = i
    return i


if _PROFILE_TAGS:
    import atexit
    import json

    def _dump_tags():
        with open(_PROFILE_TAGS, "w") as fp:
            json.dump({str(i): k for k, i in _tag_ids.items()}, fp, indent=0)
    atexit.register(_dump_tags)


def _timed(kind, d, launch):
    if _PROFILE_TAGS:
        L = _lib.load()
        L.dpi_profile_marker(_tag_id(kind, d), stream())
        launch()
        L.dpi_profile_marker(1, stream())
        return
    key = _timer.match(kind, d) if _timer is not None else None
    if key:
        e0, e1 = torch.cuda.Event(enable_timing=True), torch.cuda.Event(enable_timing=True)
        e0.record()
        launch()
        e1.record()
        _timer.events.append((key, e0, e1))
    else:
        launch()


_ws_cache = {}


def _ws_floats(kind, d):
    key = (kind, d.Cin, d.Cout, d.D, d.H, d.W, d.k, d.kd, d.stride, d.precision, d.io)
    n = _ws_cache.get(key)
    if n is None:
        L = _lib.load()
        n = {"fwd": L.dpi_conv_fwd_ws_floats, "bwd_data": L.dpi_conv_bwd_data_ws_floats}[kind](C.byref(d))
        _ws_cache[key] = n
    return n


def reset_ws_cache():
    _ws_cache.clear()


def _conv_ws(n, like):
    return torch.empty(n, dtype=torch.float32, device=like.device) if n else None


def raw_conv_fwd(d, x, chain, w, bias, y, partials=None):
    L = _lib.load()
    n = _ws_floats("fwd", d)
    ws = _conv_ws(n, x)
    _timed("conv_fwd", d, lambda: check(L.dpi_conv_fwd_ws(C.byref(d), ptr(x), ptr(chain), ptr(w), ptr(bias), ptr(y),
                                                          ptr(partials), ptr(ws), n, stream()), "dpi_conv_fwd"))


def raw_conv_bwd_data(d, dy, w, dx, accumulate=False):
    L = _lib.load()
    n = _ws_floats("bwd_data", d)
    ws = _conv_ws(n, dy)
    _timed("conv_bwd_data", d, lambda: check(L.dpi_conv_bwd_data_ws(C.byref(d), ptr(dy), ptr(w), ptr(dx), int(accumulate),
                                                                    ptr(ws), n, stream()), "dpi_conv_bwd_data"))


def raw_conv_bwd_data_dual(d3, dy3, w3, d1, dy1, w1, dx, accumulate=False):
    L = _lib.load()
    n = _ws_floats("bwd_data", d3)
    ws = _conv_ws(n, dy3)

    def launch():
        check(L.dpi_conv_bwd_data_dual(C.byref(d3), ptr(dy3), ptr(w3), C.byref(d1), ptr(dy1), ptr(w1), ptr(dx), int(accumulate),
                                       ptr(ws), n, stream()), "dpi_conv_bwd_data_dual")
    _timed("conv_bwd_data", d3, launch)


sched = Schedule()
set_weight_grad_overlap = sched.set_overlap
begin_iteration = sched.begin
abort_iteration = sched.abort
finish_backward = sched.finish


def conv_bwd_weight_async(d, x, chain, dy, dw):
    if not sched.overlap or (torch.cuda.is_current_stream_capturing() and not sched.overlap_in_graph):
        return raw_conv_bwd_weight(d, x, chain, dy, dw)
    side = sched.side_stream()
    side.wait_stream(torch.cuda.current_stream())
    with torch.cuda.stream(side):
        raw_conv_bwd_weight(d, x, chain, dy, dw)
    sched.keep(x, chain, dy, dw)


def raw_conv_bwd_weight(d, x, chain, dy, dw):
    L = _lib.load()
    n = L.dpi_conv_bwd_weight_ws_floats(C.byref(d))
    ws = torch.empty(n, dtype=torch.float32, device=x.device)
    _timed("conv_bwd_weight", d, lambda: check(L.dpi_conv_bwd_weight(C.byref(d), ptr(x), ptr(chain), ptr(dy), ptr(dw),
                                                                     ptr(ws), n, stream()), "dpi_conv_bwd_weight"))


def raw_channel_sum(x, C_, V, out):
    L = _lib.load()
    nblk = L.dpi_stat_blocks(C_, V)
    ws = torch.empty(nblk * C_ * 2, dtype=torch.float64, device=x.device)
    check(L.dpi_channel_sum(ptr(x), C_, V, ptr(ws), ptr(out), stream()), "dpi_channel_sum")


def raw_bn_stats_finalize(x, chain_in, C_, V, gamma, beta, slope, running_mean, running_var, nbt, mean_invstd, chain_out,
                          eps=BN_EPS, momentum=BN_MOMENTUM, act_first=0, compose=False):
    L = _lib.load()
    nblk = L.dpi_stat_blocks(C_, V)
    part = torch.empty(nblk * C_ * 2, dtype=torch.float64, device=x.device)
    check(L.dpi_channel_stats_io(ptr(x), ptr(chain_in), C_, V, ptr(part), _io(x), stream()), "dpi_channel_stats")
    check(L.dpi_bn_finalize(ptr(part), nblk, C_, V, ptr(gamma), ptr(beta), eps, momentum, slope, act_first,
                            ptr(chain_in) if compose else None, ptr(running_mean), ptr(running_var), ptr(nbt), ptr(mean_invstd),
                            ptr(chain_out), stream()), "dpi_bn_finalize")


def raw_bn_finalize(part, nblk, C_, count, gamma, beta, slope, running_mean, running_var, nbt, mean_invstd, chain_out,
# ... 40 lines not shown
        Do, Ho, Wo = desc_out_dims(d)
        y = torch.empty(_like_spatial(x, d.Cout, Do, Ho, Wo), dtype=torch.float32, device=x.device)
        raw_conv_fwd(d, x, None, w, b, y)
        ctx.save_for_backward(x, w)
        ctx.d = d
        ctx.has_bias = b is not None
        return y

    @staticmethod
    def backward(ctx, dy):
        x, w = ctx.saved_tensors
        d = ctx.d
        dy = _req(dy, "conv grad")
        dx = dw = db = None
        if ctx.needs_input_grad[1]:
            dw = torch.empty_like(w)
            conv_bwd_weight_async(d, x, None, dy, dw)
        if ctx.needs_input_grad[0]:
            dx = torch.empty_like(x)
            raw_conv_bwd_data(d, dy, w, dx)
        if ctx.has_bias and ctx.needs_input_grad[2]:
            db = torch.empty(d.Cout, dtype=torch.float32, device=x.device)
            raw_channel_sum(dy, d.Cout, dy.numel() // d.Cout, db)
        sched.join_side()
        return dx, dw, db, None


def _bn_backward(dy, x, mi, gamma, beta, pre_slope, post_slope, in_chain=None, dx=None):
    L = _lib.load()
    C_ = x.shape[1]
    V = x.numel() // C_
    nblk = L.dpi_stat_blocks(C_, V)
    part = torch.empty(nblk * C_ * 2, dtype=torch.float64, device=x.device)
    io = _io(x, dy)
    check(L.dpi_bn_bwd_reduce_io(ptr(dy), ptr(x), ptr(mi), ptr(gamma), ptr(beta), ptr(in_chain), pre_slope, post_slope, C_, V,
                                 ptr(part), io, stream()), "dpi_bn_bwd_reduce")
    if dx is None:
        dx = torch.empty_like(dy)
    _same_type(dy, dx, "bn_backward")
    dgamma = torch.empty_like(gamma)
    dbeta = torch.empty_like(gamma)
    check(L.dpi_bn_bwd_apply_io(ptr(dy), ptr(x), ptr(mi), ptr(gamma), ptr(beta), ptr(in_chain), pre_slope, post_slope, ptr(part), nblk,
                                C_, V, ptr(dx), ptr(dgamma), ptr(dbeta), io, stream()), "dpi_bn_bwd_apply")
    return dx, dgamma, dbeta


def _bn_backward_fork(dy, x, mi, gamma, beta, pre_slope, post_slope, forks):
    L = _lib.load()
    C_ = x.shape[1]
    V = x.numel() // C_
    nblk = L.dpi_stat_blocks(C_, V)
    part = torch.empty(nblk * C_ * 2, dtype=torch.float64, device=x.device)
    io = _io(x, dy)
    check(L.dpi_bn_bwd_reduce_io(ptr(dy), ptr(x), ptr(mi), ptr(gamma), ptr(beta), None, pre_slope, post_slope, C_, V, ptr(part),
                                 io, stream()), "dpi_bn_bwd_reduce")
    dx = torch.empty_like(dy)
    dgamma, dbeta = torch.empty_like(gamma), torch.empty_like(gamma)
    fparts = [torch.empty(nblk * C_ * 2, dtype=torch.float64, device=x.device) for _ in forks]
    fa = []
    for k in range(2):
        if k < len(forks):
            xk, mik, gk, ek, chk, postk = forks[k]
            _same_type(x, xk, "bn_backward_fork")
            fa += [ptr(xk), ptr(mik), ptr(gk), ptr(ek), ptr(chk), postk, ptr(fparts[k])]
        else:
            fa += [None, None, None, None, None, 1.0, None]
    check(L.dpi_bn_bwd_apply_fork_io(ptr(dy), ptr(x), ptr(mi), ptr(gamma), ptr(beta), None, pre_slope, post_slope, ptr(part), nblk, C_, V,
                                     ptr(dx), ptr(dgamma), ptr(dbeta), *fa, io, stream()), "dpi_bn_bwd_apply_fork")
    return dx, dgamma, dbeta, [(nblk, fp) for fp in fparts]


def _bn_backward_apply(dy, x, mi, gamma, beta, pre_slope, post_slope, red, in_chain=None, dx=None):
    L = _lib.load()
    C_ = x.shape[1]
    V = x.numel() // C_
    nblk, part = red
    if dx is None:
        dx = torch.empty_like(dy)
    _same_type(dy, dx, "bn_backward_apply")
    dgamma, dbeta = torch.empty_like(gamma), torch.empty_like(gamma)
    check(L.dpi_bn_bwd_apply_io(ptr(dy), ptr(x), ptr(mi), ptr(gamma), ptr(beta), ptr(in_chain), pre_slope, post_slope, ptr(part), nblk,
                                C_, V, ptr(dx), ptr(dgamma), ptr(dbeta), _io(x, dy), stream()), "dpi_bn_bwd_apply")
    return dx, dgamma, dbeta


def _bn_backward_apply_dual(dy, side_a, side_b, fork=None):
    L = _lib.load()
    xa, mia, ga, ea, cha, posta, (nblk, parta) = side_a
    xb, mib, gb, eb, chb, postb, (nblk_b, partb) = side_b
    assert nblk == nblk_b
    C_ = xa.shape[1]
    V = xa.numel() // C_
    _same_type(xa, xb, "bn_backward_apply_dual")
    dxa, dxb = torch.empty_like(dy), torch.empty_like(dy)
    dga, dea, dgb, deb = (torch.empty_like(g) for g in (ga, ga, gb, gb))
    red_f = None
    fargs = [0, 0, None, None, None, 1.0, None]
    if fork is not None:
        lo, hi, mif, gf, ef, postf = fork
        nb = L.dpi_stat_blocks(C_, V)
        pf = torch.empty(nb * (hi - lo) * 2, dtype=torch.float64, device=xa.device)
        fargs = [lo, hi, ptr(mif), ptr(gf), ptr(ef), postf, ptr(pf)]
        red_f = (nb, pf)
    check(L.dpi_bn_bwd_apply_dual_io(ptr(dy), nblk, C_, V,
                                     ptr(xa), ptr(mia), ptr(ga), ptr(ea), ptr(cha), posta, ptr(parta), ptr(dxa), ptr(dga), ptr(dea),
                                     ptr(xb), ptr(mib), ptr(gb), ptr(eb), ptr(chb), postb, ptr(partb), ptr(dxb), ptr(dgb), ptr(deb),
                                     *fargs, _io(xa, dy), stream()), "dpi_bn_bwd_apply_dual")
    return (dxa, dga, dea), (dxb, dgb, deb), red_f


JOIN_BWD_FUSED = os.environ.get("DPI_JOIN_BWD", "1") == "1"


def _join_backward(dy, t, mi, gamma, beta, pre_slope, side_a, side_b, fork=None, fwd_chains=None):
    L = _lib.load()
    xa, mia, ga, ea, cha, posta = side_a
    xb, mib, gb, eb, chb, postb = side_b
    C_ = dy.shape[1]
    V = dy.numel() // C_
    dev = dy.device
    fwa, fwb = fwd_chains if fwd_chains is not None else (None, None)
    ws = torch.empty(L.dpi_join_bwd_ws_doubles(C_, V), dtype=torch.float64, device=dev)
    coef = torch.empty(C_ * 8, dtype=torch.float32, device=dev)
    dgb = torch.empty((6, C_), dtype=torch.float32, device=dev)
    dxa, dxb = torch.empty_like(dy), torch.empty_like(dy)
    if fork is not None:
        lo, hi, mif, gf, ef, postf, dxf = fork
        dgbf = torch.empty((2, hi - lo), dtype=torch.float32, device=dev)
        fa = [lo, hi, ptr(mif), ptr(gf), ptr(ef), postf]
    else:
        dxf = dgbf = None
        fa = [0, 0, None, None, None, 1.0]
    check(L.dpi_join_bwd(ptr(dy), ptr(t), ptr(mi), ptr(gamma), ptr(beta), pre_slope, C_, V,
                         ptr(xa), ptr(mia), ptr(ga), ptr(ea), ptr(cha), posta, ptr(xb), ptr(mib), ptr(gb), ptr(eb), ptr(chb), postb,
                         ptr(fwa), ptr(fwb), *fa, ptr(ws), ptr(coef), ptr(dxa), ptr(dxb), ptr(dxf), ptr(dgb), ptr(dgbf), _io(xa, dy), stream()),
          "dpi_join_bwd")
    f = None if dgbf is None else (dgbf[0], dgbf[1])
    return (dxa, dgb[2], dgb[3]), (dxb, dgb[4], dgb[5]), (dgb[0], dgb[1]), f


def _join_fused_ok(*tensors):
    return JOIN_BWD_FUSED and (all(x.dtype == torch.float32 for x in tensors) or all(x.dtype == torch.bfloat16 for x in tensors))


def _join_forward(a, ch_a, b, ch_b, C_, V, slope, bn, gamma, beta, mi_out, y, keep_t, t=None, ch_out=None):
    L = _lib.load()
    dev = a.device
    if keep_t and t is None:
        t = torch.empty_like(a)
    nblk = L.dpi_stat_blocks(C_, V)
    part = torch.empty(nblk * C_ * 2, dtype=torch.float64, device=dev)
    check(L.dpi_chain_add_stats_io(ptr(a), ptr(ch_a), ptr(b), ptr(ch_b), C_, V, slope, ptr(t), ptr(part), _io(a), stream()),
          "dpi_chain_add_stats")
    if ch_out is None:
        ch_out = torch.empty(C_ * 5, dtype=torch.float32, device=dev)
    raw_bn_finalize(part, nblk, C_, V, gamma, beta, slope, bn.running_mean, bn.running_var, bn.num_batches_tracked, mi_out, ch_out,
                    act_first=1)
    if keep_t:
        raw_chain_apply(t, ch_out, C_, V, y)
    else:
        check(L.dpi_chain_add_apply(ptr(a), ptr(ch_a), ptr(b), ptr(ch_b), ptr(ch_out), C_, V, ptr(y), _io(a), stream()), "dpi_chain_add_apply")
    return t


def _pre_chain(C_, pre_slope, device):
    return None if pre_slope == 1.0 else slope_chain(C_, pre_slope, device)
# ... 124 lines not shown

    @staticmethod
    def forward(ctx, x, blk, slope, *p):
        x = _req(x, "block input", act=True)
        (w1, b1, g1, e1, w2, b2, g2, e2, w3, b3, g3, e3, ws, bs, gs, es, gA, eA, gB, eB) = p
        L = _lib.load()
        dev = x.device
        f32 = dict(dtype=torch.float32, device=dev)
        adt = act_dtype()
        c1, c2, c3 = w1.shape[0], w2.shape[0], w3.shape[0]
        Ct = c1 + c2 + c3
        bn1_, bn2_, bn3_, bns_ = (m._parts()[1] for m in (blk.conv3x3, blk.conv5x5, blk.conv7x7, blk.shortcut))
        d1 = make_desc(x, w1, 1, adt)
        Do, Ho, Wo = desc_out_dims(d1)
        V = Do * Ho * Wo
        R = torch.empty(_like_spatial(x, Ct, Do, Ho, Wo), dtype=adt, device=dev)
        CH = torch.empty(Ct * 5, **f32)
        r1, r2, r3 = R[:, :c1], R[:, c1:c1 + c2], R[:, c1 + c2:]
        ch1, ch2, ch3 = CH[:c1 * 5], CH[c1 * 5:(c1 + c2) * 5], CH[(c1 + c2) * 5:]
        mi1, mi2, mi3 = (torch.empty(2 * c, **f32) for c in (c1, c2, c3))
        miA, miS, miB = (torch.empty(2 * Ct, **f32) for _ in range(3))
        dsc = make_desc(x, ws, 1, adt)
        S = torch.empty_like(R)
        chSA = torch.empty((2, Ct * 5), **f32)
        chS, chA = chSA[0], chSA[1]
        side_shortcut = sched.branch_shortcut if sched.branch_on() else 0

        def shortcut_on_branch():
            with sched.branch("short", x, S, miS, chS):
                _cba_raw(dsc, x, None, ws, bs, bns_, slope, S, miS, chS)
        if side_shortcut == 1:
            shortcut_on_branch()
        _cba_raw(d1, x, None, w1, b1, bn1_, slope, r1, mi1, ch1)
        if side_shortcut == 2:
            shortcut_on_branch()
        d2 = make_desc(r1, w2, 1, adt)
        _cba_raw(d2, r1, ch1, w2, b2, bn2_, slope, r2, mi2, ch2)
        d3 = make_desc(r2, w3, 1, adt)
        _cba_raw(d3, r2, ch2, w3, b3, bn3_, slope, r3, mi3, ch3)
        A = blk.bn1
        raw_bn_stats_finalize(R, CH, Ct, V, gA, eA, 1.0, A.running_mean, A.running_var, A.num_batches_tracked, miA, chA,
                              compose=True)
        if side_shortcut:
            sched.join_branch("short")
        else:
            _cba_raw(dsc, x, None, ws, bs, bns_, slope, S, miS, chS)
        y = torch.empty_like(R)
        tless = _join_fused_ok(R, S)
        t = _join_forward(S, chS, R, chA, Ct, V, slope, blk.bn2, gB, eB, miB, y, keep_t=not tless)
        if tless:
            t = chSA
        ctx.tless = tless
        _save_with_params(ctx, (x, R, S, t, CH, mi1, mi2, mi3, miA, miS, miB), p)
        ctx.descs = (d1, d2, d3, dsc)
        ctx.slope = float(slope)
        ctx.split = (c1, c2, c3)
        return y

    @staticmethod
    def backward(ctx, dy):
        dy = _req(dy, "block grad", act=True)
        (x, R, S, t, CH, mi1, mi2, mi3, miA, miS, miB), p = _saved_with_params(ctx, 11)
        (w1, b1, g1, e1, w2, b2, g2, e2, w3, b3, g3, e3, ws, bs, gs, es, gA, eA, gB, eB) = p
        d1, d2, d3, dsc = ctx.descs
        slope = ctx.slope
        c1, c2, c3 = ctx.split
        s1, s2, s3 = slice(0, c1), slice(c1, c1 + c2), slice(c1 + c2, c1 + c2 + c3)
        ch1, ch2 = CH[:c1 * 5], CH[c1 * 5:(c1 + c2) * 5]
        dR = torch.empty_like(R)
        if ctx.tless or _join_fused_ok(dy, t, S, R):
            (dS, dgs, des), (dcat, dgA, deA), (dgB, deB), (dg3, de3) = _join_backward(
                dy, None if ctx.tless else t, miB, gB, eB, slope, (S, miS, gs, es, None, slope), (R, miA, gA, eA, CH, 1.0),
                fork=(c1 + c2, c1 + c2 + c3, mi3, g3, e3, slope, dR[:, s3]), fwd_chains=(t[0], t[1]) if ctx.tless else None)
        else:
            dt, dgB, deB, (redS, redA) = _bn_backward_fork(dy, t, miB, gB, eB, slope, 1.0,
                                                           [(S, miS, gs, es, None, slope), (R, miA, gA, eA, CH, 1.0)])
            (dS, dgs, des), (dcat, dgA, deA), red3 = _bn_backward_apply_dual(
                dt, (S, miS, gs, es, None, slope, redS), (R, miA, gA, eA, CH, 1.0, redA), fork=(c1 + c2, c1 + c2 + c3, mi3, g3, e3, slope))
            del dt
            _, dg3, de3 = _bn_backward_apply(dcat[:, s3], R[:, s3], mi3, g3, e3, 1.0, slope, red3, dx=dR[:, s3])
        dws = torch.empty_like(ws)
        dw3 = torch.empty_like(w3)
        conv_bwd_weight_async(d3, R[:, s2], ch2, dR[:, s3], dw3)
        raw_conv_bwd_data(d3, dR[:, s3], w3, dcat[:, s2], accumulate=True)
        _, dg2, de2 = _bn_backward(dcat[:, s2], R[:, s2], mi2, g2, e2, 1.0, slope, dx=dR[:, s2])
        dw2 = torch.empty_like(w2)
        conv_bwd_weight_async(d2, R[:, s1], ch1, dR[:, s2], dw2)
        raw_conv_bwd_data(d2, dR[:, s2], w2, dcat[:, s1], accumulate=True)
        _, dg1, de1 = _bn_backward(dcat[:, s1], R[:, s1], mi1, g1, e1, 1.0, slope, dx=dR[:, s1])
        dw1 = torch.empty_like(w1)
        conv_bwd_weight_async(d1, x, None, dR[:, s1], dw1)
        conv_bwd_weight_async(dsc, x, None, dS, dws)
        dx = None
        if ctx.needs_input_grad[0]:
            dx = torch.empty_like(x)
            raw_conv_bwd_data_dual(d1, dR[:, s1], w1, dsc, dS, ws, dx)
        sched.join_side()
        z = _zeros_like_or_none
        return (dx, None, None, dw1, z(b1, dR[:, s1]), dg1, de1, dw2, z(b2, dR[:, s2]), dg2, de2, dw3, z(b3, dR[:, s3]), dg3, de3,
                dws, z(bs, dS), dgs, des, dgA, deA, dgB, deB)


def _respath_bn_backward(dy, t, miB, gB, eB, slope, r3, mi3, g3, e3, r1, mi1, g1, e1, tless=False):
    if tless or _join_fused_ok(dy, t, r3, r1):
        a, b, top, _ = _join_backward(dy, None if tless else t, miB, gB, eB, slope, (r3, mi3, g3, e3, None, slope), (r1, mi1, g1, e1, None, slope),
                                      fwd_chains=(t[1], t[0]) if tless else None)
        return a, b, top
    dt, dgB, deB, (red3, red1) = _bn_backward_fork(dy, t, miB, gB, eB, slope, 1.0,
                                                   [(r3, mi3, g3, e3, None, slope), (r1, mi1, g1, e1, None, slope)])
    a, b, _ = _bn_backward_apply_dual(dt, (r3, mi3, g3, e3, None, slope, red3), (r1, mi1, g1, e1, None, slope, red1))
    return a, b, (dgB, deB)


def _respath_alloc(x, p, y=None):
    w3, w1 = p[0], p[4]
    f32 = dict(dtype=torch.float32, device=x.device)
    adt = act_dtype()
    Cs = w3.shape[0]
    d3, d1 = make_desc(x, w3, 1, adt), make_desc(x, w1, 1, adt)
    dims = desc_out_dims(d3)
    T = dict(adt=adt, Cs=Cs, d3=d3, d1=d1, dims=dims)
    T["r3"] = torch.empty(_like_spatial(x, Cs, *dims), dtype=adt, device=x.device)
    T["r1"] = torch.empty_like(T["r3"])
    if y is not None and (y.shape != T["r3"].shape or y.dtype != adt):
        raise _lib.DpiError("respath: the output slice is %s %s, the node writes %s %s" % (tuple(y.shape), y.dtype, tuple(T["r3"].shape), adt))
    T["y"] = torch.empty_like(T["r3"]) if y is None else y
    T["tless"] = _join_fused_ok(T["r3"])
    T["mi3"], T["mi1"], T["miB"] = (torch.empty(2 * Cs, **f32) for _ in range(3))
    T["ch13"] = torch.empty((2, 5 * Cs), **f32)
    T["ch1"], T["ch3"], T["chB"] = T["ch13"][0], T["ch13"][1], torch.empty(5 * Cs, **f32)
    T["t"] = None if T["tless"] else torch.empty_like(T["r3"])
    T["keep"] = T["ch13"] if T["tless"] else T["t"]
    return T


def _respath_launch(x, rp, slope, p, T):
    (w3, b3, g3, e3, w1, b1, g1, e1, gB, eB) = p
    Do, Ho, Wo = T["dims"]
    bn3_, bn1_ = rp.conv3x3._parts()[1], rp.conv1x1._parts()[1]
    _cba_raw(T["d3"], x, None, w3, b3, bn3_, slope, T["r3"], T["mi3"], T["ch3"])
    _cba_raw(T["d1"], x, None, w1, b1, bn1_, slope, T["r1"], T["mi1"], T["ch1"])
    _join_forward(T["r1"], T["ch1"], T["r3"], T["ch3"], T["Cs"], Do * Ho * Wo, slope, rp.bn, gB, eB, T["miB"], T["y"], keep_t=not T["tless"],
                  t=T["t"], ch_out=T["chB"])


def _respath_save(ctx, x, T, p, slope):
    _save_with_params(ctx, (x, T["r3"], T["r1"], T["keep"], T["mi3"], T["mi1"], T["miB"]), p)
    ctx.descs = (T["d3"], T["d1"])
    ctx.slope = float(slope)
    ctx.tless = T["tless"]


def _respath_backward(ctx, dy):
    (x, r3, r1, t, mi3, mi1, miB), (w3, b3, g3, e3, w1, b1, g1, e1, gB, eB) = _saved_with_params(ctx, 7)
    d3, d1 = ctx.descs
    (dr3, dg3, de3), (dr1, dg1, de1), (dgB, deB) = _respath_bn_backward(dy, t, miB, gB, eB, ctx.slope, r3, mi3, g3, e3, r1, mi1, g1, e1, ctx.tless)
    dw3, dw1 = torch.empty_like(w3), torch.empty_like(w1)
    conv_bwd_weight_async(d3, x, None, dr3, dw3)
    conv_bwd_weight_async(d1, x, None, dr1, dw1)
    dx = None
    if ctx.needs_input_grad[0]:
        dx = torch.empty_like(x)
        raw_conv_bwd_data_dual(d3, dr3, w3, d1, dr1, w1, dx)
    z = _zeros_like_or_none
    return dx, (dw3, z(b3, dr3), dg3, de3, dw1, z(b1, dr1), dg1, de1, dgB, deB)


class ResPath3dFn(torch.autograd.Function):

    @staticmethod
    def forward(ctx, x, rp, slope, *p):
        x = _req(x, "respath input", act=True)
# ... 577 lines not shown
```

### include/dpi_hip.h

```cpp
#ifndef DPI_HIP_H
#define DPI_HIP_H

#include <stddef.h>
#include <stdint.h>

#ifdef __cplusplus
extern "C" {
#endif

#define DPI_OK 0
#define DPI_E_ARG (-1)
#define DPI_E_LAUNCH (-2)
#define DPI_E_WORKSPACE (-3)

#define DPI_CHAIN_STRIDE 5

const char* dpi_last_error(void);
int dpi_version(void);
int dpi_device_info(int device, int* cus, int* lds_bytes, size_t* hbm_bytes, char* name, int name_len);
int dpi_profile_marker(int id, void* stream);
int dpi_set_option(const char* key, int value);

typedef struct {
  int size;
  int Cin, Cout;
  int D, H, W;
  int k, kd;
  int stride;
  int precision;
  int io;
} dpi_conv_desc;
#define DPI_IO_X_BF16 1
#define DPI_IO_Y_BF16 2
#define DPI_IO_DY_BF16 4
#define DPI_IO_DX_BF16 8
int dpi_conv_desc_size(void);

int dpi_conv_fwd_stat_blocks(const dpi_conv_desc* d);
int dpi_conv_fwd(const dpi_conv_desc* d, const float* x, const float* x_chain, const float* w,
                 const float* bias, float* y, double* stat_partials, void* stream);
int dpi_conv_bwd_data(const dpi_conv_desc* d, const float* dy, const float* w, float* dx,
                      int accumulate, void* stream);
size_t dpi_conv_fwd_ws_floats(const dpi_conv_desc* d);
size_t dpi_conv_bwd_data_ws_floats(const dpi_conv_desc* d);
int dpi_conv_fwd_ws(const dpi_conv_desc* d, const float* x, const float* x_chain, const float* w,
                    const float* bias, float* y, double* stat_partials, float* ws, size_t ws_floats, void* stream);
int dpi_conv_bwd_data_ws(const dpi_conv_desc* d, const float* dy, const float* w, float* dx,
                         int accumulate, float* ws, size_t ws_floats, void* stream);
int dpi_conv_bwd_data_dual(const dpi_conv_desc* d3, const float* dy3, const float* w3,
                           const dpi_conv_desc* d1, const float* dy1, const float* w1,
                           float* dx, int accumulate, float* ws, size_t ws_floats, void* stream);
size_t dpi_conv_bwd_weight_ws_floats(const dpi_conv_desc* d);
int dpi_conv_bwd_weight(const dpi_conv_desc* d, const float* x, const float* x_chain, const float* dy,
                        float* dw, float* ws, size_t ws_floats, void* stream);


int dpi_stat_blocks(int C, size_t V);
int dpi_channel_stats(const float* x, const float* chain, int C, size_t V, double* partials, void* stream);
int dpi_bn_finalize(const double* partials, int nblk, int C, size_t count, const float* gamma,
                    const float* beta, float eps, float momentum, float slope, int act_first,
                    const float* in_chain, float* running_mean, float* running_var, int64_t* num_batches_tracked,
                    float* mean_invstd, float* chain_out, void* stream);
int dpi_chain_apply(const float* x, const float* chain, int C, size_t V, float* y, void* stream);
int dpi_bn_bwd_reduce(const float* dy, const float* x, const float* mean_invstd, const float* gamma,
                      const float* beta, const float* in_chain, float pre_slope, float post_slope, int C,
                      size_t V, double* partials, void* stream);
int dpi_bn_bwd_apply(const float* dy, const float* x, const float* mean_invstd, const float* gamma,
                     const float* beta, const float* in_chain, float pre_slope, float post_slope,
                     const double* partials, int nblk, int C, size_t V, float* dx, float* dgamma,
                     float* dbeta, void* stream);
int dpi_bn_bwd_apply_fork(const float* dy, const float* x, const float* mean_invstd, const float* gamma,
                          const float* beta, const float* in_chain, float pre_slope, float post_slope,
                          const double* partials, int nblk, int C, size_t V, float* dx, float* dgamma,
                          float* dbeta, const float* xa, const float* mi_a, const float* gamma_a,
                          const float* beta_a, const float* chain_a, float post_a, double* partials_a,
                          const float* xb, const float* mi_b, const float* gamma_b, const float* beta_b,
                          const float* chain_b, float post_b, double* partials_b, void* stream);
int dpi_bn_bwd_apply_dual(const float* dy, int nblk, int C, size_t V, const float* xa, const float* mi_a,
                          const float* gamma_a, const float* beta_a, const float* chain_a, float post_a,
                          const double* partials_a, float* dxa, float* dgamma_a, float* dbeta_a, const float* xb,
                          const float* mi_b, const float* gamma_b, const float* beta_b, const float* chain_b,
                          float post_b, const double* partials_b, float* dxb, float* dgamma_b, float* dbeta_b,
                          int f_lo, int f_hi, const float* f_mi, const float* f_gamma, const float* f_beta,
                          float f_post, double* f_partials, void* stream);
int dpi_chain_add_stats(const float* a, const float* chain_a, const float* b, const float* chain_b, int C,
                        size_t V, float slope, float* t, double* partials, void* stream);
int dpi_lrelu_bwd(const float* dy, const float* x, float slope, size_t n, float* dx, void* stream);
#define DPI_ACT_ELU 1
#define DPI_ACT_TANH 2
#define DPI_ACT_SIGMOID 3
int dpi_act_fwd(const float* x, size_t n, int kind, float* y, void* stream);
int dpi_act_bwd(const float* dy, const float* y, size_t n, int kind, float* dx, void* stream);
int dpi_add(const float* a, const float* b, size_t n, float* y, void* stream);
int dpi_channel_sum(const float* x, int C, size_t V, double* ws, float* out, void* stream);

#define DPI_STORE_FWD_BF16 1u
#define DPI_STORE_GRAD_BF16 2u
int dpi_channel_stats_io(const float* x , const float* chain, int C, size_t V, double* partials, unsigned io, void* stream);
int dpi_chain_apply_io(const float* x , const float* chain, int C, size_t V, float* y , unsigned io, void* stream);
int dpi_chain_add_stats_io(const float* a , const float* chain_a, const float* b , const float* chain_b, int C, size_t V,
                           float slope, float* t , double* partials, unsigned io, void* stream);
int dpi_bn_bwd_reduce_io(const float* dy , const float* x , const float* mean_invstd, const float* gamma, const float* beta,
                         const float* in_chain, float pre_slope, float post_slope, int C, size_t V, double* partials, unsigned io,
                         void* stream);
int dpi_bn_bwd_apply_io(const float* dy , const float* x , const float* mean_invstd, const float* gamma, const float* beta,
                        const float* in_chain, float pre_slope, float post_slope, const double* partials, int nblk, int C, size_t V,
                        float* dx , float* dgamma, float* dbeta, unsigned io, void* stream);
int dpi_bn_bwd_apply_fork_io(const float* dy , const float* x , const float* mean_invstd, const float* gamma, const float* beta,
                             const float* in_chain, float pre_slope, float post_slope, const double* partials, int nblk, int C,
                             size_t V, float* dx , float* dgamma, float* dbeta, const float* xa , const float* mi_a,
                             const float* gamma_a, const float* beta_a, const float* chain_a, float post_a, double* partials_a,
                             const float* xb , const float* mi_b, const float* gamma_b, const float* beta_b, const float* chain_b,
                             float post_b, double* partials_b, unsigned io, void* stream);
int dpi_bn_bwd_apply_dual_io(const float* dy , int nblk, int C, size_t V, const float* xa , const float* mi_a,
                             const float* gamma_a, const float* beta_a, const float* chain_a, float post_a,
                             const double* partials_a, float* dxa , float* dgamma_a, float* dbeta_a, const float* xb ,
                             const float* mi_b, const float* gamma_b, const float* beta_b, const float* chain_b,
                             float post_b, const double* partials_b, float* dxb , float* dgamma_b, float* dbeta_b,
                             int f_lo, int f_hi, const float* f_mi, const float* f_gamma, const float* f_beta,
                             float f_post, double* f_partials, unsigned io, void* stream);
int dpi_upsample2x_fwd_io(const float* x , const float* chain, int C, int D, int H, int W, int Do, int Ho, int Wo, int linear,
                          float* y , unsigned io, void* stream);
int dpi_upsample2x_bwd_io(const float* dy , int C, int D, int H, int W, int Do, int Ho, int Wo, int linear, float* dx ,
                          float* ws, unsigned io, void* stream);
int dpi_noise_add_io(const float* z, size_t n, float std, uint64_t seed, const uint64_t* step_ptr, float* out , unsigned io,
                     void* stream);

int dpi_upsample2x_fwd(const float* x, const float* chain, int C, int D, int H, int W, int Do, int Ho,
                       int Wo, int linear, float* y, void* stream);
size_t dpi_upsample2x_bwd_ws_floats(int C, int D, int H, int W, int Do, int Ho, int Wo, int linear);
int dpi_upsample2x_bwd(const float* dy, int C, int D, int H, int W, int Do, int Ho, int Wo, int linear,
                       float* dx, float* ws, void* stream);
int dpi_crop_copy(const float* x, int C, int D, int H, int W, int od, int oh, int ow, int Do, int Ho,
                  int Wo, float* y, void* stream);
int dpi_crop_copy_bwd(const float* dy, int C, int D, int H, int W, int od, int oh, int ow, int Do,
                      int Ho, int Wo, float* dx, void* stream);

int dpi_attn_gate_fwd(const float* x, const float* q, int C, int D, int H, int W, int scale_d, float* s_out, float* y, void* stream);
size_t dpi_attn_gate_bwd_ws_floats(int C, int D, int H, int W, int scale_d);
int dpi_attn_gate_bwd(const float* dy, const float* x, const float* s, int C, int D, int H, int W, int scale_d, float* dx, float* dq,
                      float* ws, void* stream);

int dpi_pconv_mask_fwd(const float* x, const float* m, int Cin, int Cm, size_t V, float* xm, float* msum, void* stream);
int dpi_pconv_norm_fwd(const float* c, const float* msum, const float* bias, int Cout, int D, int H, int W, float* y, float* new_mask,
                       float* S, void* stream);
size_t dpi_pconv_norm_bwd_ws_floats(int Cout, size_t V);
int dpi_pconv_norm_bwd(const float* dy, const float* S, int Cout, size_t V, float* dc, float* dbias, float* ws, void* stream);
int dpi_pconv_mask_bwd(const float* dxm, const float* x, const float* m, int Cin, int Cm, size_t V, float* dx, float* dm, void* stream);

int dpi_maxpool2x2_fwd(const float* x, int C, int H, int W, float* y, void* stream);
int dpi_maxpool2x2_bwd(const float* dy, const float* x, int C, int H, int W, float* dx, void* stream);
int dpi_deconv4x4s2_fwd(const float* x, const float* w, const float* bias, int Cin, int Cout, int H, int W,
                        float* y, void* stream);
// ... 99 lines not shown
```

Measured before the change: 34.08.

## Fuse BatchNorm-backward reduction into backward-data conv epilogue for MultiRes chain

The backward-data convolution epilogue (MFMA, Q4 and split-K reduce paths) now reads the saved BN input and computes the per-channel BatchNorm-backward partial sums while it stores dx. This replaces the separate reduction pass that re-read dcat and x. A small fold kernel shrinks the per-tile partials before the existing bn_bwd_apply runs. The cost is extra epilogue register pressure and x loads inside the conv kernels, plus more template variants and a new partials buffer allocation per call.

```diff
diff --git a/deep_prior_interpolation_amd/_lib.py b/deep_prior_interpolation_amd/_lib.py
--- a/deep_prior_interpolation_amd/_lib.py
+++ b/deep_prior_interpolation_amd/_lib.py
@@ -138,6 +138,11 @@
     "dpi_join_bwd": (_I, [_P, _P, _P, _P, _P, _F, _I, _Z,  _P, _P, _P, _P, _P, _F,  _P, _P, _P, _P, _P, _F,  _P, _P,  _I, _I, _P, _P, _P, _F,
                           _P, _P, _P, _P, _P, _P, _P, _U, _P]),
     "dpi_chain_add_apply": (_I, [_P, _P, _P, _P, _P, _I, _Z, _P, _U, _P]),
+    "dpi_conv_bwd_data_bnred_supported": (_I, [_DESC]),
+    "dpi_conv_bwd_data_bnred_blocks": (_I, [_DESC]),
+    "dpi_conv_bwd_data_bnred": (_I, [_DESC, _P, _P, _P, _I, _P, _Z, _P, _P, _P, _P, _P, _F, _F, _P, _P]),
+    "dpi_bn_bwd_fold_rows": (_I, [_I]),
+    "dpi_bn_bwd_fold": (_I, [_P, _I, _I, _P, _P]),
 }
 
 _lib = None
diff --git a/deep_prior_interpolation_amd/csrc/api.cpp b/deep_prior_interpolation_amd/csrc/api.cpp
--- a/deep_prior_interpolation_amd/csrc/api.cpp
+++ b/deep_prior_interpolation_amd/csrc/api.cpp
@@ -55,6 +55,7 @@
   static const Entry table[] = {
       {"splitk", 0, 1, dpi_set_splitk},
       {"dual_bwd_data", 0, 1, dpi_set_dual_bwd_data},
+      {"bwd_data_bnred", 0, 1, dpi_set_bwd_data_bnred},
       {"bw_pair", 0, 2, dpi_set_bw_pair},
       {"bw_workgroups", 1, 1 << 24, [](int v) { dpi_set_bw_tuning(v, -1); }},
       {"bw_xcd_order", 0, 1, [](int v) { dpi_set_bw_tuning(0, v); }},
diff --git a/deep_prior_interpolation_amd/csrc/bn_bwd.h b/deep_prior_interpolation_amd/csrc/bn_bwd.h
--- /dev/null
+++ b/deep_prior_interpolation_amd/csrc/bn_bwd.h
@@ -0,0 +1,36 @@
+#pragma once
+#include "common.h"
+
+struct BnBwd {
+  float mean, invstd, a, pb, pre, post;
+  bool chained;
+  Chain in;
+};
+__device__ __forceinline__ BnBwd bn_bwd_consts(const float* __restrict__ mean_invstd, const float* __restrict__ gamma,
+                                               const float* __restrict__ beta, const float* __restrict__ in_chain, float pre,
+                                               float post, int C, int c) {
+  BnBwd k;
+  k.chained = in_chain != nullptr;
+  k.in = load_chain(in_chain, c);
+  k.mean = mean_invstd[c]; k.invstd = mean_invstd[C + c];
+  k.a = (gamma ? gamma[c] : 1.f) * k.invstd;
+  k.pb = (beta ? beta[c] : 0.f) - k.mean * k.a;
+  k.pre = pre; k.post = post;
+  return k;
+}
+__device__ __forceinline__ void bn_bwd_elem(const BnBwd& k, float x, float dy, float& xhat, float& g) {
+  if (k.chained) x = apply_chain(k.in, x);
+  const float u = x > 0.f ? x : x * k.pre;
+  xhat = (u - k.mean) * k.invstd;
+  const float yv = fmaf(k.a, u, k.pb);
+  g = (k.post == 1.f || yv > 0.f) ? dy : dy * k.post;
+}
+
+struct BnRedArgs {
+  const float* __restrict__ x;
+  const float* __restrict__ mean_invstd;
+  const float* __restrict__ gamma;
+  const float* __restrict__ beta;
+  const float* __restrict__ in_chain;
+  float pre, post;
+};
diff --git a/deep_prior_interpolation_amd/csrc/conv_direct.hip b/deep_prior_interpolation_amd/csrc/conv_direct.hip
--- a/deep_prior_interpolation_amd/csrc/conv_direct.hip
+++ b/deep_prior_interpolation_amd/csrc/conv_direct.hip
@@ -553,6 +553,38 @@
   return conv_run(d3, dy3, nullptr, w3, nullptr, dx, nullptr, true, 1, ws, ws_floats, st);
 }
 
+static int g_bnred = getenv("DPI_NO_BNRED") ? 0 : 1;
+extern "C" void dpi_set_bwd_data_bnred(int on) { g_bnred = on; }
+static bool bnred_plan(const dpi_conv_desc* d, ConvPlan* plan) {
+  if (d->stride != 1) return false;
+  *plan = conv_plan(d, true, 0);
+  if (plan->kernel == ConvKernel::Q4) return dpi_conv_q4_bnred_ok(d);
+  if (plan->kernel == ConvKernel::Mfma) return dpi_conv_mfma_bnred_ok(d);
+  return false;
+}
+extern "C" int dpi_conv_bwd_data_bnred_supported(const dpi_conv_desc* d) {
+  ConvPlan plan;
+  return g_bnred && dpi_check_conv_desc(d) == DPI_OK && bnred_plan(d, &plan) ? 1 : 0;
+}
+extern "C" int dpi_conv_bwd_data_bnred_blocks(const dpi_conv_desc* d) {
+  ConvPlan plan;
+  return dpi_check_conv_desc(d) == DPI_OK && bnred_plan(d, &plan) ? plan.stat_blocks : 0;
+}
+extern "C" int dpi_conv_bwd_data_bnred(const dpi_conv_desc* d, const float* dy, const float* w, float* dx, int accumulate, float* ws,
+                                       size_t ws_floats, const float* x, const float* mean_invstd, const float* gamma, const float* beta,
+                                       const float* in_chain, float pre_slope, float post_slope, double* partials, void* stream) {
+  if (int e = dpi_check_conv_desc(d)) return e;
+  DPI_REQUIRE(dy && w && dx && x && mean_invstd && partials, "conv_bwd_data_bnred: null tensor");
+  DPI_REQUIRE(ws || ws_floats == 0, "conv_bwd_data_bnred: workspace size without a workspace");
+  DPI_REQUIRE(!in_chain || pre_slope == 1.f, "conv_bwd_data_bnred: in_chain excludes pre_slope");
+  ConvPlan plan;
+  DPI_REQUIRE(bnred_plan(d, &plan), "conv_bwd_data_bnred: not supported for this launch (dpi_conv_bwd_data_bnred_supported)");
+  const BnRedArgs bn{x, mean_invstd, gamma, beta, in_chain, pre_slope, post_slope};
+  hipStream_t st = (hipStream_t)stream;
+  if (plan.kernel == ConvKernel::Q4) return dpi_conv_q4_run(d, dy, nullptr, w, nullptr, dx, partials, true, accumulate, st, &bn);
+  return dpi_conv_mfma_run(d, dy, nullptr, w, nullptr, dx, partials, true, accumulate, ws, ws_floats, st, nullptr, &bn);
+}
+
 extern "C" int dpi_conv_bwd_data_ws(const dpi_conv_desc* d, const float* dy, const float* w, float* dx,
                                     int accumulate, float* ws, size_t ws_floats, void* stream) {
   if (int e = dpi_check_conv_desc(d)) return e;
diff --git a/deep_prior_interpolation_amd/csrc/conv_kernels.h b/deep_prior_interpolation_amd/csrc/conv_kernels.h
--- a/deep_prior_interpolation_amd/csrc/conv_kernels.h
+++ b/deep_prior_interpolation_amd/csrc/conv_kernels.h
@@ -1,5 +1,6 @@
 #pragma once
 #include "common.h"
+#include "bn_bwd.h"
 
 struct MfmaSecond { const float* x2; const float* w2; int C2; long w2_co_stride, w2_c_stride; };
 void dpi_conv_out_dims(const dpi_conv_desc* d, int* Do, int* Ho, int* Wo);
@@ -7,7 +8,9 @@
 size_t dpi_conv_mfma_ws_floats(const dpi_conv_desc* d, bool flip);
 bool dpi_conv_mfma_second_ok(const dpi_conv_desc* d, bool flip, int C2, bool have_ws);
 int dpi_conv_mfma_run(const dpi_conv_desc* d, const float* x, const float* chain, const float* w, const float* bias, float* y,
-                      double* partials, bool flip, int accumulate, float* ws, size_t ws_floats, hipStream_t st, const MfmaSecond* sec = nullptr);
+                      double* partials, bool flip, int accumulate, float* ws, size_t ws_floats, hipStream_t st, const MfmaSecond* sec = nullptr,
+                      const BnRedArgs* bn = nullptr);
+bool dpi_conv_mfma_bnred_ok(const dpi_conv_desc* d);
 int dpi_conv_bwd_data_s2_mfma_run(const dpi_conv_desc* d, const float* dy, const float* w, float* dx, int accumulate, hipStream_t st);
 size_t dpi_conv_bwd_weight_mfma_ws_floats(const dpi_conv_desc* d);
 bool dpi_conv_bwd_weight_mfma_swapped(const dpi_conv_desc* d, bool chained);
@@ -26,7 +29,8 @@
 bool dpi_conv_q4_usable(const dpi_conv_desc* d, bool flip);
 int dpi_conv_q4_stat_blocks(const dpi_conv_desc* d);
 int dpi_conv_q4_run(const dpi_conv_desc* d, const float* x, const float* chain, const float* w, const float* bias, float* y,
-                    double* partials, bool flip, int accumulate, hipStream_t st);
+                    double* partials, bool flip, int accumulate, hipStream_t st, const BnRedArgs* bn = nullptr);
+bool dpi_conv_q4_bnred_ok(const dpi_conv_desc* d);
 bool dpi_bf16_force_all();
 bool dpi_conv_bf16_usable(const dpi_conv_desc* d, bool flip);
 int dpi_conv_bf16_stat_blocks(const dpi_conv_desc* d);
diff --git a/deep_prior_interpolation_amd/csrc/conv_mfma.hip b/deep_prior_interpolation_amd/csrc/conv_mfma.hip
--- a/deep_prior_interpolation_amd/csrc/conv_mfma.hip
+++ b/deep_prior_interpolation_amd/csrc/conv_mfma.hip
@@ -23,6 +23,7 @@
   long w2_co_stride, w2_c_stride;
   int xb, yb;
   int ny;
+  BnRedArgs bn;
 };
 
 template <int KD, int NR, int NH, int S = 1>
@@ -200,8 +201,9 @@
 #define TRC(i)
 #endif
 template <int KD, int NR, int NH, bool FLIP, int S = 1, int WPE = 2, bool PERSIST = false, bool TAILPACK = false, bool IOB = false, bool YLOOP = false,
-          bool S2V = false>
+          bool S2V = false, bool BNR = false>
 __global__ __launch_bounds__(256, WPE) void conv_mfma_kernel(MArgs a) {
+  static_assert(!BNR || (FLIP && !IOB && !YLOOP && S == 1), "BatchNorm-backward partials: backward-data launches on fp32 tensors");
   static_assert(!YLOOP || (!PERSIST && !TAILPACK), "the channel-tile loop is built for the one-tile-per-workgroup variants without a packed tail");
   static_assert(!S2V || (S == 2 && !FLIP && !PERSIST && !TAILPACK && !IOB && NR < 4), "vectorised stride-2 staging: forward, fp32 tensors, row-split tiles");
   using GV = GeoV2<KD, NR < 4 ? NR : 2, NH>;
@@ -496,7 +498,29 @@
       const float bv = (a.bias && cok) ? a.bias[co] : 0.f;
       float* __restrict__ yc = dpi_at(ybase, (size_t)(cok ? co : 0) * Vo + vbase, a.yb);
       double s = 0.0, q = 0.0;
-      if (a.yb) {
+      if constexpr (BNR) {
+        const BnBwd k = bn_bwd_consts(a.bn.mean_invstd, a.bn.gamma, a.bn.beta, a.bn.in_chain, a.bn.pre, a.bn.post, a.Cout, cok ? co : 0);
+        const float* __restrict__ xc = a.bn.x + (size_t)(cok ? co : 0) * Vo + vbase;
+        float xr[NT];
+        bool okt[NT];
+#pragma unroll
+        for (int t = 0; t < NT; ++t) {
+          const int od = od0 + wz, oh = oh0 + wh + t / NH, ow = ow0 + (t % NH) * 16 + lj;
+          okt[t] = interior || (cok && od < Do && oh < Ho && ow < Wo);
+          xr[t] = okt[t] ? xc[(t / NH) * Wo + (t % NH) * 16] : 0.f;
+        }
+#pragma unroll
+        for (int t = 0; t < NT; ++t) {
+          if (okt[t]) {
+            const float v = acc[t][r] + bv;
+            yc[(t / NH) * Wo + (t % NH) * 16] = v;
+            float xh, g;
+            bn_bwd_elem(k, xr[t], v, xh, g);
+            s += (double)g;
+            q += (double)(g * xh);
+          }
+        }
+      } else if (a.yb) {
         const bool pairs = !(Wo & 1) && !(Vo & 1) && !((uintptr_t)ybase & 3);
 #pragma unroll
         for (int t = 0; t < NT; ++t) {
@@ -1110,14 +1134,17 @@
   }
 }
 
+template <bool BNR = false>
 __global__ __launch_bounds__(256) void splitk_reduce_kernel(const float* __restrict__ ws, int nsplit, const float* __restrict__ bias,
                                                             float* __restrict__ y, int accumulate, double* __restrict__ partials,
-                                                            int Cout, size_t Vo, size_t per, bool yb) {
+                                                            int Cout, size_t Vo, size_t per, bool yb, BnRedArgs bn) {
   const int lane = threadIdx.x & 63, co = blockIdx.y * 4 + (threadIdx.x >> 6);
   if (co >= Cout) return;
   const size_t lo = (size_t)blockIdx.x * per, hi = lo + per < Vo ? lo + per : Vo;
   const float bv = bias ? bias[co] : 0.f;
   double sum = 0.0, sq = 0.0;
+  BnBwd k;
+  if constexpr (BNR) k = bn_bwd_consts(bn.mean_invstd, bn.gamma, bn.beta, bn.in_chain, bn.pre, bn.post, Cout, co);
   for (size_t v = lo + lane; v < hi; v += 64) {
     float t = ws[(size_t)co * Vo + v];
     for (int sp = 1; sp < nsplit; ++sp) t += ws[((size_t)sp * Cout + co) * Vo + v];
@@ -1125,7 +1152,11 @@
     if (accumulate) t += dpi_ld(y, (size_t)co * Vo + v, yb);
     t = dpi_stored(t, yb);
     dpi_st(y, (size_t)co * Vo + v, t, yb);
-    sum += t; sq += (double)t * t;
+    if constexpr (BNR) {
+      float xh, g;
+      bn_bwd_elem(k, bn.x[(size_t)co * Vo + v], t, xh, g);
+      sum += (double)g; sq += (double)(g * xh);
+    } else { sum += t; sq += (double)t * t; }
   }
   if (partials) {
 #pragma unroll
@@ -1228,6 +1259,23 @@
   }
   else if (nh == 2) conv_mfma_kernel<KD, 2, 2, FLIP, 1, 2, false, false, IOB><<<grid, 256, 0, st>>>(a);
   else conv_mfma_kernel<KD, 2, 1, FLIP, 1, 2, false, false, IOB><<<grid, 256, 0, st>>>(a);
+}
+
+static void launch_variant_bnred(const MArgs& a_in, int nr, int nh, dim3 grid_in, hipStream_t st) {
+  MArgs a = a_in;
+  dim3 grid = grid_in;
+  if (grid_in.y > 1) {
+    a.ny = (int)grid_in.y;
+    grid = dim3(8 * ((grid_in.x + 7) / 8) * grid_in.y, 1, 1);
+  }
+  const bool tailpack = (a.Cin & 3) == 1 && (a.Cin > 4 || a.Cin == 1);
+  if (nr == 4) {
+    if (tailpack) conv_mfma_kernel<3, 4, 2, true, 1, 3, false, true, false, false, false, true><<<grid, 256, 0, st>>>(a);
+    else conv_mfma_kernel<3, 4, 2, true, 1, 3, false, false, false, false, false, true><<<grid, 256, 0, st>>>(a);
+  }
+  else if (nr == 8) conv_mfma_kernel<3, 8, 2, true, 1, 3, false, false, false, false, false, true><<<grid, 256, 0, st>>>(a);
+  else if (nh == 2) conv_mfma_kernel<3, 2, 2, true, 1, 2, false, false, false, false, false, true><<<grid, 256, 0, st>>>(a);
+  else conv_mfma_kernel<3, 2, 1, true, 1, 2, false, false, false, false, false, true><<<grid, 256, 0, st>>>(a);
 }
 
 #ifdef DPI_TRACE
@@ -1268,8 +1316,15 @@
   return !(have_ws && dpi_mfma_splitk(d, flip) > 1);
 }
 
+bool dpi_conv_mfma_bnred_ok(const dpi_conv_desc* d) {
+  if (d->k != 3 || d->kd != 3 || d->stride != 1 || dpi_io_in(d, true) || dpi_io_out(d, true)) return false;
+  const MfmaTiling t = mfma_tiling(d, true);
+  return !(t.nr == 8 && d->Cout > 8);
+}
+
 int dpi_conv_mfma_run(const dpi_conv_desc* d, const float* x, const float* chain, const float* w, const float* bias, float* y,
-                      double* partials, bool flip, int accumulate, float* ws, size_t ws_floats, hipStream_t st, const MfmaSecond* sec) {
+                      double* partials, bool flip, int accumulate, float* ws, size_t ws_floats, hipStream_t st, const MfmaSecond* sec,
+                      const BnRedArgs* bn) {
   const int taps = d->kd * 9;
   const int cin = flip ? d->Cout : d->Cin, cout = flip ? d->Cin : d->Cout;
   const long w_out = flip ? taps : (long)d->Cin * taps, w_in = flip ? (long)d->Cin * taps : taps;
@@ -1280,6 +1335,7 @@
   a.ntd = t.ntd; a.nth = t.nth; a.ntw = t.ntw;
   dim3 grid(ntiles, cdiv(cout, 16));
   if (sec) { a.x2 = sec->x2; a.w2 = sec->w2; a.C2 = sec->C2; a.w2_co_stride = sec->w2_co_stride; a.w2_c_stride = sec->w2_c_stride; }
+  if (bn) DPI_REQUIRE(flip && !sec && partials && dpi_conv_mfma_bnred_ok(d), "conv_mfma: this launch cannot take BatchNorm-backward partials");
   const int nsplit = (ws && !sec) ? dpi_mfma_splitk(d, flip) : 1;
   if (nsplit > 1) {
     int Do, Ho, Wo;
@@ -1293,9 +1349,16 @@
     if (d->kd == 3) { if (flip) launch_variant<3, true>(a, nr, nh, d->stride, grid, st); else launch_variant<3, false>(a, nr, nh, d->stride, grid, st); }
     else { if (flip) launch_variant<1, true>(a, nr, nh, d->stride, grid, st); else launch_variant<1, false>(a, nr, nh, d->stride, grid, st); }
     if (int e = dpi_check_launch("conv_mfma (split)")) return e;
-    splitk_reduce_kernel<<<dim3(ntiles, cdiv(cout, 4)), 256, 0, st>>>(ws, nz, bias, y, accumulate, partials, cout, Vo, cdivz(Vo, (size_t)ntiles),
-                                                                      dpi_io_out(d, flip));
-    return dpi_check_launch("splitk_reduce");
+    const dim3 rgrid(ntiles, cdiv(cout, 4));
+    const size_t per = cdivz(Vo, (size_t)ntiles);
+    if (bn) splitk_reduce_kernel<true><<<rgrid, 256, 0, st>>>(ws, nz, bias, y, accumulate, partials, cout, Vo, per, false, *bn);
+    else splitk_reduce_kernel<false><<<rgrid, 256, 0, st>>>(ws, nz, bias, y, accumulate, partials, cout, Vo, per, dpi_io_out(d, flip), BnRedArgs{});
+    return dpi_check_launch(bn ? "splitk_reduce (bn partials)" : "splitk_reduce");
+  }
+  if (bn) {
+    a.bn = *bn;
+    launch_variant_bnred(a, nr, nh, grid, st);
+    return dpi_check_launch("conv_mfma (bn partials)");
   }
   if (d->kd == 3) { if (flip) launch_variant<3, true>(a, nr, nh, d->stride, grid, st); else launch_variant<3, false>(a, nr, nh, d->stride, grid, st); }
   else { if (flip) launch_variant<1, true>(a, nr, nh, d->stride, grid, st); else launch_variant<1, false>(a, nr, nh, d->stride, grid, st); }
diff --git a/deep_prior_interpolation_amd/csrc/conv_q4_mfma.hip b/deep_prior_interpolation_amd/csrc/conv_q4_mfma.hip
--- a/deep_prior_interpolation_amd/csrc/conv_q4_mfma.hip
+++ b/deep_prior_interpolation_amd/csrc/conv_q4_mfma.hip
@@ -17,6 +17,7 @@
   long w_out_stride, w_in_stride;
   int accumulate;
   int dbg;
+  BnRedArgs bn;
 };
 
 template <int R>
@@ -34,8 +35,9 @@
   return (xcd < r ? xcd * (q + 1) : r * (q + 1) + (xcd - r) * q) + i;
 }
 
-template <int R, int NB, int CK, bool FLIP, bool AL>
+template <int R, int NB, int CK, bool FLIP, bool AL, bool BNR = false>
 __global__ __launch_bounds__(256, 2) void conv_q4_mfma_kernel(QArgs a) {
+  static_assert(!BNR || FLIP, "BatchNorm-backward partials: backward-data launches");
   using G = QGeo<R>;
   constexpr int TAPS = 27;
   constexpr int NWT = CK * TAPS * NB * 4;
@@ -203,6 +205,14 @@
       const float bv = (a.bias && cok) ? a.bias[co] : 0.f;
       float* __restrict__ yc = a.y + (size_t)(cok ? co : 0) * V + ((size_t)(od < Do ? od : 0) * Ho + oh0) * Wo + ow;
       double sm = 0.0, sq = 0.0;
+      float xf[BNR ? R : 1];
+      BnBwd bk;
+      if constexpr (BNR) {
+        bk = bn_bwd_consts(a.bn.mean_invstd, a.bn.gamma, a.bn.beta, a.bn.in_chain, a.bn.pre, a.bn.post, a.Cout, cok ? co : 0);
+        const float* __restrict__ xc = a.bn.x + (size_t)(cok ? co : 0) * V + ((size_t)(od < Do ? od : 0) * Ho + oh0) * Wo + ow;
+#pragma unroll
+        for (int hr = 0; hr < R; ++hr) xf[hr] = (cok && col_ok && oh0 + hr < Ho) ? xc[hr * Wo] : 0.f;
+      }
       float old[R];
       if (a.accumulate) {
 #pragma unroll
@@ -216,8 +226,15 @@
         if (cok && col_ok && oh0 + hr < Ho) {
           const float v = acc[hr][s][i] + bv + old[hr];
           if (!(a.dbg & 8)) yc[hr * Wo] = v;
-          sm += v;
-          sq += (double)v * v;
+          if constexpr (BNR) {
+            float xh, g;
+            bn_bwd_elem(bk, xf[hr], v, xh, g);
+            sm += (double)g;
+            sq += (double)(g * xh);
+          } else {
+            sm += v;
+            sq += (double)v * v;
+          }
         }
       }
       if (a.partials && cok) {
@@ -537,13 +554,31 @@
   else conv_q4_mfma_kernel<8, NB, 2, FLIP, false><<<ntiles, 256, extra, st>>>(a);
 }
 
+bool dpi_conv_q4_bnred_ok(const dpi_conv_desc* d) {
+  if (!dpi_conv_q4_usable(d, true)) return false;
+  return !(d->Cin <= 4 && (g_q4_ck == 4 || (g_q4_ck == 0 && d->Cout >= 16)));
+}
+
+template <int NB>
+static void q4_launch_bnred(const QArgs& a, int ntiles, bool aligned, hipStream_t st) {
+  const size_t extra = (size_t)((g_q4_dbg >> 8) & 255) * 1024;
+  if (aligned) conv_q4_mfma_kernel<8, NB, 2, true, true, true><<<ntiles, 256, extra, st>>>(a);
+  else conv_q4_mfma_kernel<8, NB, 2, true, false, true><<<ntiles, 256, extra, st>>>(a);
+}
+
 int dpi_conv_q4_run(const dpi_conv_desc* d, const float* x, const float* chain, const float* w, const float* bias, float* y,
-                    double* partials, bool flip, int accumulate, hipStream_t st) {
+                    double* partials, bool flip, int accumulate, hipStream_t st, const BnRedArgs* bn) {
   const int cin = flip ? d->Cout : d->Cin, cout = flip ? d->Cin : d->Cout;
   const long w_out = flip ? 27 : (long)d->Cin * 27, w_in = flip ? (long)d->Cin * 27 : 27;
   QArgs a{x, chain, w, bias, y, partials, cin, cout, d->D, d->H, d->W, 0, 0, 0, w_out, w_in, accumulate, g_q4_dbg};
   const int ntiles = q4_tiles(d, &a.ntd, &a.nth, &a.ntw);
   const bool aligned = ((uintptr_t)x & 15) == 0;
+  if (bn) {
+    DPI_REQUIRE(flip && partials && dpi_conv_q4_bnred_ok(d), "conv_q4: this launch cannot take BatchNorm-backward partials");
+    a.bn = *bn;
+    if (cout <= 4) q4_launch_bnred<1>(a, ntiles, aligned, st); else q4_launch_bnred<2>(a, ntiles, aligned, st);
+    return dpi_check_launch("conv_q4_mfma (bn partials)");
+  }
   if (cout <= 4) { if (flip) q4_launch<1, true>(a, ntiles, aligned, st); else q4_launch<1, false>(a, ntiles, aligned, st); }
   else { if (flip) q4_launch<2, true>(a, ntiles, aligned, st); else q4_launch<2, false>(a, ntiles, aligned, st); }
   return dpi_check_launch("conv_q4_mfma");
diff --git a/deep_prior_interpolation_amd/csrc/dpi_hip_internal.h b/deep_prior_interpolation_amd/csrc/dpi_hip_internal.h
--- a/deep_prior_interpolation_amd/csrc/dpi_hip_internal.h
+++ b/deep_prior_interpolation_amd/csrc/dpi_hip_internal.h
@@ -5,6 +5,7 @@
 DPI_INTERNAL void dpi_set_bf16_debug(int flags);
 DPI_INTERNAL void dpi_set_splitk(int on);
 DPI_INTERNAL void dpi_set_dual_bwd_data(int on);
+DPI_INTERNAL void dpi_set_bwd_data_bnred(int on);
 DPI_INTERNAL void dpi_set_bw_pair(int mode);
 DPI_INTERNAL void dpi_set_mfma_min_cout(int n);
 DPI_INTERNAL void dpi_set_bwd_weight_mfma_min_cout(int n);
diff --git a/deep_prior_interpolation_amd/csrc/elementwise.hip b/deep_prior_interpolation_amd/csrc/elementwise.hip
--- a/deep_prior_interpolation_amd/csrc/elementwise.hip
+++ b/deep_prior_interpolation_amd/csrc/elementwise.hip
@@ -1,4 +1,5 @@
 #include "common.h"
+#include "bn_bwd.h"
 #include <stdlib.h>
 
 namespace {
@@ -130,31 +131,6 @@
       for (int k = 0; k < 4 && i + k < V; ++k) dpi_st(yc, i + k, apply_chain(t, dpi_ld(xc, i + k, xb)), yb);
     }
   }
-}
-
-struct BnBwd {
-  float mean, invstd, a, pb, pre, post;
-  bool chained;
-  Chain in;
-};
-__device__ __forceinline__ BnBwd bn_bwd_consts(const float* __restrict__ mean_invstd, const float* __restrict__ gamma,
-                                               const float* __restrict__ beta, const float* __restrict__ in_chain, float pre,
-                                               float post, int C, int c) {
-  BnBwd k;
-  k.chained = in_chain != nullptr;
-  k.in = load_chain(in_chain, c);
-  k.mean = mean_invstd[c]; k.invstd = mean_invstd[C + c];
-  k.a = (gamma ? gamma[c] : 1.f) * k.invstd;
-  k.pb = (beta ? beta[c] : 0.f) - k.mean * k.a;
-  k.pre = pre; k.post = post;
-  return k;
-}
-__device__ __forceinline__ void bn_bwd_elem(const BnBwd& k, float x, float dy, float& xhat, float& g) {
-  if (k.chained) x = apply_chain(k.in, x);
-  const float u = x > 0.f ? x : x * k.pre;
-  xhat = (u - k.mean) * k.invstd;
-  const float yv = fmaf(k.a, u, k.pb);
-  g = (k.post == 1.f || yv > 0.f) ? dy : dy * k.post;
 }
 
 template <bool fb = false, bool gb = false>
@@ -1137,6 +1113,32 @@
   return dpi_check_launch("bn_bwd_apply");
 }
 
+namespace {
+constexpr int kFoldRows = 256;
+__global__ __launch_bounds__(256) void bn_bwd_fold_kernel(const double* __restrict__ in, int ntiles, int per, int n2, double* __restrict__ out) {
+  const int j = blockIdx.x;
+  const int lo = j * per, hi = lo + min(per, ntiles - lo);
+  for (int e = threadIdx.x; e < n2; e += 256) {
+    double s = 0.0;
+    for (int t = lo; t < hi; ++t) s += in[(size_t)t * n2 + e];
+    out[(size_t)j * n2 + e] = s;
+  }
+}
+}
+static int fold_per(int ntiles) { return (ntiles - 1) / kFoldRows + 1; }
+extern "C" int dpi_bn_bwd_fold_rows(int ntiles) {
+  if (ntiles <= 0) return 0;
+  return (ntiles - 1) / fold_per(ntiles) + 1;
+}
+extern "C" int dpi_bn_bwd_fold(const double* partials, int ntiles, int C, double* folded, void* stream) {
+  DPI_REQUIRE(partials && folded && ntiles > 0 && C > 0, "bn_bwd_fold: bad argument");
+  DPI_REQUIRE(partials != folded, "bn_bwd_fold: folds out of place");
+  DPI_REQUIRE(C <= (1 << 29), "bn_bwd_fold: %d channels", C);
+  const int per = fold_per(ntiles);
+  bn_bwd_fold_kernel<<<dpi_bn_bwd_fold_rows(ntiles), 256, 0, (hipStream_t)stream>>>(partials, ntiles, per, 2 * C, folded);
+  return dpi_check_launch("bn_bwd_fold");
+}
+
 extern "C" int dpi_bn_bwd_apply_fork(const float* dy, const float* x, const float* mean_invstd, const float* gamma, const float* beta,
                                      const float* in_chain, float pre_slope, float post_slope, const double* partials, int nblk, int C,
                                      size_t V, float* dx, float* dgamma, float* dbeta, const float* xa, const float* mi_a,
diff --git a/deep_prior_interpolation_amd/ops.py b/deep_prior_interpolation_amd/ops.py
--- a/deep_prior_interpolation_amd/ops.py
+++ b/deep_prior_interpolation_amd/ops.py
@@ -194,7 +194,8 @@
     n = _ws_cache.get(key)
     if n is None:
         L = _lib.load()
-        n = {"fwd": L.dpi_conv_fwd_ws_floats, "bwd_data": L.dpi_conv_bwd_data_ws_floats}[kind](C.byref(d))
+        n = {"fwd": L.dpi_conv_fwd_ws_floats, "bwd_data": L.dpi_conv_bwd_data_ws_floats,
+             "bnred": lambda p: L.dpi_conv_bwd_data_bnred_blocks(p) if L.dpi_conv_bwd_data_bnred_supported(p) else 0}[kind](C.byref(d))
         _ws_cache[key] = n
     return n
 
@@ -401,6 +402,27 @@
     check(L.dpi_bn_bwd_apply_io(ptr(dy), ptr(x), ptr(mi), ptr(gamma), ptr(beta), ptr(in_chain), pre_slope, post_slope, ptr(part), nblk,
                                 C_, V, ptr(dx), ptr(dgamma), ptr(dbeta), _io(x, dy), stream()), "dpi_bn_bwd_apply")
     return dx, dgamma, dbeta
+
+
+def _conv_bwd_data_bn_backward(d, dy, w, dcat, x, mi, gamma, beta, post_slope, dx):
+    nt = _ws_floats("bnred", d) if dcat.dtype == torch.float32 and x.dtype == torch.float32 else 0
+    if not nt:
+        raw_conv_bwd_data(d, dy, w, dcat, accumulate=True)
+        return _bn_backward(dcat, x, mi, gamma, beta, 1.0, post_slope, dx=dx)
+    L = _lib.load()
+    C_ = d.Cin
+    part = torch.empty(nt * C_ * 2, dtype=torch.float64, device=x.device)
+    n = _ws_floats("bwd_data", d)
+    ws = _conv_ws(n, dy)
+    _timed("conv_bwd_data", d, lambda: check(L.dpi_conv_bwd_data_bnred(C.byref(d), ptr(dy), ptr(w), ptr(dcat), 1, ptr(ws), n, ptr(x), ptr(mi), ptr(gamma),
+                                                                       ptr(beta), None, 1.0, post_slope, ptr(part), stream()),
+                                             "dpi_conv_bwd_data_bnred"))
+    nblk = L.dpi_bn_bwd_fold_rows(nt)
+    if nblk != nt:
+        folded = torch.empty(nblk * C_ * 2, dtype=torch.float64, device=x.device)
+        check(L.dpi_bn_bwd_fold(ptr(part), nt, C_, ptr(folded), stream()), "dpi_bn_bwd_fold")
+        part = folded
+    return _bn_backward_apply(dcat, x, mi, gamma, beta, 1.0, post_slope, (nblk, part), dx=dx)
 
 
 def _bn_backward_apply_dual(dy, side_a, side_b, fork=None):
@@ -691,12 +713,10 @@
         dws = torch.empty_like(ws)
         dw3 = torch.empty_like(w3)
         conv_bwd_weight_async(d3, R[:, s2], ch2, dR[:, s3], dw3)
-        raw_conv_bwd_data(d3, dR[:, s3], w3, dcat[:, s2], accumulate=True)
-        _, dg2, de2 = _bn_backward(dcat[:, s2], R[:, s2], mi2, g2, e2, 1.0, slope, dx=dR[:, s2])
+        _, dg2, de2 = _conv_bwd_data_bn_backward(d3, dR[:, s3], w3, dcat[:, s2], R[:, s2], mi2, g2, e2, slope, dR[:, s2])
         dw2 = torch.empty_like(w2)
         conv_bwd_weight_async(d2, R[:, s1], ch1, dR[:, s2], dw2)
-        raw_conv_bwd_data(d2, dR[:, s2], w2, dcat[:, s1], accumulate=True)
-        _, dg1, de1 = _bn_backward(dcat[:, s1], R[:, s1], mi1, g1, e1, 1.0, slope, dx=dR[:, s1])
+        _, dg1, de1 = _conv_bwd_data_bn_backward(d2, dR[:, s2], w2, dcat[:, s1], R[:, s1], mi1, g1, e1, slope, dR[:, s1])
         dw1 = torch.empty_like(w1)
         conv_bwd_weight_async(d1, x, None, dR[:, s1], dw1)
         conv_bwd_weight_async(dsc, x, None, dS, dws)
diff --git a/include/dpi_hip.h b/include/dpi_hip.h
--- a/include/dpi_hip.h
+++ b/include/dpi_hip.h
@@ -50,6 +50,11 @@
 int dpi_conv_bwd_data_dual(const dpi_conv_desc* d3, const float* dy3, const float* w3,
                            const dpi_conv_desc* d1, const float* dy1, const float* w1,
                            float* dx, int accumulate, float* ws, size_t ws_floats, void* stream);
+int dpi_conv_bwd_data_bnred_supported(const dpi_conv_desc* d);
+int dpi_conv_bwd_data_bnred_blocks(const dpi_conv_desc* d);
+int dpi_conv_bwd_data_bnred(const dpi_conv_desc* d, const float* dy, const float* w, float* dx, int accumulate, float* ws,
+                            size_t ws_floats, const float* x, const float* mean_invstd, const float* gamma, const float* beta, const float* in_chain,
+                            float pre_slope, float post_slope, double* partials, void* stream);
 size_t dpi_conv_bwd_weight_ws_floats(const dpi_conv_desc* d);
 int dpi_conv_bwd_weight(const dpi_conv_desc* d, const float* x, const float* x_chain, const float* dy,
                         float* dw, float* ws, size_t ws_floats, void* stream);
@@ -69,6 +74,8 @@
                      const float* beta, const float* in_chain, float pre_slope, float post_slope,
                      const double* partials, int nblk, int C, size_t V, float* dx, float* dgamma,
                      float* dbeta, void* stream);
+int dpi_bn_bwd_fold_rows(int ntiles);
+int dpi_bn_bwd_fold(const double* partials, int ntiles, int C, double* folded, void* stream);
 int dpi_bn_bwd_apply_fork(const float* dy, const float* x, const float* mean_invstd, const float* gamma,
                           const float* beta, const float* in_chain, float pre_slope, float post_slope,
                           const double* partials, int nblk, int C, size_t V, float* dx, float* dgamma,
```

New measurement: 34.27, median of 6. About the same (+0.6%).
